# ut-amrl/vision_slam_frontend

Hardware: AMD Instinct MI355X
Metric: stereo frames/s (640x480, 2000 kp/frame) (higher is better)
Workload: dtype u8

## Files before the change

### include/vsf.h

```cpp
#ifndef VSF_H_
#define VSF_H_

#include <stddef.h>
#include <stdint.h>

#ifdef __cplusplus
extern "C" {
#endif

#define VSF_VERSION 2
#define VSF_DESC_BYTES 32
#define VSF_MAX_LEVELS 64

typedef enum {
  VSF_OK = 0,
  VSF_ERR_INVALID_ARG = 1,
  VSF_ERR_CAPACITY = 2,
  VSF_ERR_HIP = 3,
  VSF_ERR_UNSUPPORTED = 4,
  VSF_ERR_NO_DEVICE = 5
} vsf_status;

typedef struct {
  float x, y;
  float size;
  float angle;
  float response;
  int32_t octave;
  int32_t class_id;
} vsf_keypoint;

typedef struct {
  int32_t queryIdx, trainIdx, imgIdx;
  float distance;
} vsf_dmatch;

typedef struct {
  int32_t nfeatures;
  float scale_factor;
  int32_t nlevels;
  int32_t edge_threshold;
  int32_t first_level;
  int32_t wta_k;
  int32_t score_type;
  int32_t patch_size;
  int32_t fast_threshold;
  int32_t blur_sse2;
  int32_t fast_detector_threshold;
  int32_t fast_detector_nms;
  uint32_t ratio_num;
  uint32_t ratio_shift;
  int32_t width, height;
  int32_t max_images;
  int32_t max_keypoints;
  int32_t residual_order;
} vsf_params;

typedef struct vsf_ctx vsf_ctx;

vsf_status vsf_params_default(vsf_params* p, int width, int height, int max_images);
vsf_status vsf_params_set_ratio(vsf_params* p, float nn_match_ratio);

vsf_status vsf_create(const vsf_params* p, int device, vsf_ctx** out);
void vsf_destroy(vsf_ctx* ctx);
const char* vsf_status_string(vsf_status s);
int vsf_last_hip_error(const vsf_ctx* ctx);
vsf_status vsf_get_params(const vsf_ctx* ctx, vsf_params* out);
vsf_status vsf_set_stream(vsf_ctx* ctx, void* hip_stream);
vsf_status vsf_set_lanes(vsf_ctx* ctx, int lanes);
vsf_status vsf_set_pipeline(vsf_ctx* ctx, int on);
vsf_status vsf_set_input_event(vsf_ctx* ctx, void* hip_event);
vsf_status vsf_set_blur_overlap(vsf_ctx* ctx, int on);
vsf_status vsf_set_fast_resident(vsf_ctx* ctx, int waves);
vsf_status vsf_get_fast_resident(const vsf_ctx* ctx, int* waves);
vsf_status vsf_tune_fast_resident(vsf_ctx* ctx, const uint8_t* d_imgs, int n_images, size_t image_stride,
                                  size_t row_stride, vsf_keypoint* d_kp, uint8_t* d_desc, int32_t* d_counts,
                                  int samples, float* ms_grid, float* ms_resident);
typedef enum {
  VSF_OPT_FAST_BOTH_MAX = 0,
  VSF_OPT_SELECT_WIDE = 1,
  VSF_OPT_PYRAMID_FEW = 2,
  VSF_OPT_PYRAMID_CHAIN = 3,
  VSF_OPT_PYRAMID_ROWS = 4,
  VSF_OPT_SELECT_BIG_CLASS = 5,
  VSF_OPT_PIPE_AFTER_FAST = 6,
  VSF_OPT_PIPE_PRIORITY = 7,
  VSF_OPT_OBSERVE_THREAD = 8,
  VSF_OPT_PYRAMID_TAIL_MIN = 9,
  VSF_OPT_OBSERVE_COPY_THREAD = 10,
  VSF_OPT_COUNT = 11
} vsf_option;
vsf_status vsf_set_option(vsf_ctx* ctx, int option, int value);
vsf_status vsf_get_option(const vsf_ctx* ctx, int option, int* value);
vsf_status vsf_sync(vsf_ctx* ctx);
vsf_status vsf_reserve(vsf_ctx* ctx, int n_frames, int n_pairs);

vsf_status vsf_level_info(const vsf_ctx* ctx, int level, int* w, int* h, float* scale, int* nfeatures);

#define VSF_COMM_ID_BYTES 128
typedef struct vsf_comm vsf_comm;
vsf_status vsf_comm_unique_id(uint8_t* id);
vsf_status vsf_comm_create(vsf_ctx* ctx, const uint8_t* id, int rank, int world, vsf_comm** out);
void vsf_comm_destroy(vsf_comm* comm);
vsf_status vsf_comm_info(const vsf_comm* comm, int* rank, int* world, int* rccl_version);
vsf_status vsf_allgather_dev(vsf_ctx* ctx, vsf_comm* comm, const void* d_send, void* d_recv, size_t bytes_per_rank);
vsf_status vsf_gather_payload_dev(vsf_ctx* ctx, vsf_comm* comm, const uint8_t* d_send, size_t bytes, uint8_t* d_recv,
                                  size_t recv_stride, int root);


vsf_status vsf_extract(vsf_ctx* ctx, const uint8_t* img, int w, int h, size_t stride, vsf_keypoint* kp_out,
                       uint8_t* desc_out, int cap, int* n_out);
vsf_status vsf_extract_pair(vsf_ctx* ctx, const uint8_t* img0, const uint8_t* img1, int w, int h, size_t stride,
                            vsf_keypoint* kp0, uint8_t* desc0, int* n0, vsf_keypoint* kp1, uint8_t* desc1, int* n1,
                            int cap);
vsf_status vsf_fast_detect(vsf_ctx* ctx, const uint8_t* img, int w, int h, size_t stride, int threshold, int nms,
                           vsf_keypoint* kp_out, int cap, int* n_out);
vsf_status vsf_knn2_hamming(vsf_ctx* ctx, const uint8_t* q, int nq, const uint8_t* t, int nt, int32_t* idx2,
                            int32_t* dist2);
vsf_status vsf_get_matches(vsf_ctx* ctx, const uint8_t* q, int nq, const uint8_t* t, int nt, vsf_dmatch* out,
                           int cap, int* n_out);

vsf_status vsf_get_matches_multi(vsf_ctx* ctx, const uint8_t* const* q, const int* nq, int n_sets, const uint8_t* t,
                                 int nt, vsf_dmatch* out, int cap_per_set, int* n_out);


vsf_status vsf_extract_batch_dev(vsf_ctx* ctx, const uint8_t* d_imgs, int n_images, size_t image_stride,
                                 size_t row_stride, vsf_keypoint* d_kp, uint8_t* d_desc, int32_t* d_counts);
vsf_status vsf_match_batch_dev(vsf_ctx* ctx, const uint8_t* d_desc, const int32_t* d_counts, size_t set_stride,
                               const int32_t* d_q_set, const int32_t* d_t_set, int n_pairs, int32_t* d_idx2,
                               int32_t* d_dist2, vsf_dmatch* d_matches, int32_t* d_nmatches);
vsf_status vsf_stereo_batch_dev(vsf_ctx* ctx, const uint8_t* d_imgs, int n_frames, size_t image_stride,
                                size_t row_stride, vsf_keypoint* d_kp, uint8_t* d_desc, int32_t* d_counts,
                                vsf_dmatch* d_matches, int32_t* d_nmatches);


vsf_status vsf_remove_ambig_stereo_batch_dev(vsf_ctx* ctx, const vsf_keypoint* d_kp, const uint8_t* d_desc,
                                             const vsf_dmatch* d_matches, const int32_t* d_nmatches, int n_frames,
                                             const float* F, float thr_in, const float* d_thr_override,
                                             float* d_means, float* d_thr, vsf_keypoint* d_kp_out,
                                             uint8_t* d_desc_out, int32_t* d_counts_out);
vsf_status vsf_feature_matches_batch_dev(vsf_ctx* ctx, const uint8_t* d_desc, const int32_t* d_counts,
                                         size_t set_stride, const int32_t* d_q_set, const int32_t* d_t_set,
                                         int n_pairs, float best_percent, uint64_t* d_pairs, int32_t* d_npairs);

vsf_status vsf_stereo_residuals_batch_dev(vsf_ctx* ctx, const vsf_keypoint* d_kp, const vsf_dmatch* d_matches,
                                          const int32_t* d_nmatches, int n_frames, const float* F, float* d_means);
vsf_status vsf_stereo_thresholds_dev(vsf_ctx* ctx, const float* d_means, int n, float* d_thr_state, float* d_thr);
vsf_status vsf_stereo_filter_batch_dev(vsf_ctx* ctx, const vsf_keypoint* d_kp, const uint8_t* d_desc,
                                       const vsf_dmatch* d_matches, const int32_t* d_nmatches, int n_frames,
                                       const float* d_thr, vsf_keypoint* d_kp_out, uint8_t* d_desc_out,
                                       int32_t* d_counts_out);


typedef struct {
  float projection_left[12];
  float projection_right[12];
  float camera_matrix_left[9];
  float distortion_left[5];
  float fundamental[9];
  int32_t triangulate_rows;
} vsf_calibration;

typedef struct {
  uint32_t feature_idx_lo, feature_idx_hi;
  float pixel[2];
  float point3d[3];
} vsf_vision_feature;
typedef struct {
  uint64_t feature_idx_initial, feature_idx_current;
} vsf_feature_match;

vsf_status vsf_vision_features_batch_dev(vsf_ctx* ctx, const vsf_calibration* calib, const vsf_keypoint* d_kp,
                                         const uint8_t* d_desc, const int32_t* d_counts, int n_frames,
                                         vsf_vision_feature* d_features, int32_t* d_nfeatures, int32_t* d_npoints);

size_t vsf_packed_outputs_capacity(const vsf_ctx* ctx, int n_frames, int n_pairs);
vsf_status vsf_pack_outputs_dev(vsf_ctx* ctx, const vsf_vision_feature* d_features, const int32_t* d_nfeatures,
                                int n_frames, const uint64_t* d_pairs, const int32_t* d_npairs, int n_pairs,
                                uint8_t* d_payload, size_t payload_cap);


size_t vsf_observe_capacity(const vsf_ctx* ctx, int frame_life);
vsf_status vsf_observe_configure(vsf_ctx* ctx, int depth, int min_batch, int in_flight);
vsf_status vsf_observe_stereo(vsf_ctx* ctx, const uint8_t* left, const uint8_t* right, int w, int h, size_t stride,
                              const vsf_calibration* calib, float best_percent, int frame_life, uint8_t* out,
                              size_t cap, size_t* out_bytes);
vsf_status vsf_observe_submit(vsf_ctx* ctx, const uint8_t* left, const uint8_t* right, int w, int h, size_t stride,
                              const vsf_calibration* calib, float best_percent, int frame_life, int64_t* ticket);
vsf_status vsf_observe_collect(vsf_ctx* ctx, int64_t ticket, uint8_t* out, size_t cap, size_t* out_bytes);
vsf_status vsf_observe_collect_view(vsf_ctx* ctx, int64_t ticket, const uint8_t** out, size_t* out_bytes);
vsf_status vsf_observe_submit_compressed(vsf_ctx* ctx, const uint8_t* left, size_t left_bytes, const uint8_t* right,
                                         size_t right_bytes, int bayer, const vsf_calibration* calib, float best_percent,
                                         int frame_life, int64_t* ticket);
vsf_status vsf_observe_stereo_compressed(vsf_ctx* ctx, const uint8_t* left, size_t left_bytes, const uint8_t* right,
                                         size_t right_bytes, int bayer, const vsf_calibration* calib, float best_percent,
                                         int frame_life, uint8_t* out, size_t cap, size_t* out_bytes);
vsf_status vsf_observe_set_compressed_cap(vsf_ctx* ctx, size_t cap_per_image);
size_t vsf_observe_default_compressed_cap(int width, int height);
vsf_status vsf_compressed_image_size(const uint8_t* file, size_t nbytes, int* width, int* height);
vsf_status vsf_observe_poll(vsf_ctx* ctx, int64_t ticket, int* ready);
vsf_status vsf_observe_reset(vsf_ctx* ctx);
#define VSF_OBSERVE_MAX_STREAMS 64
vsf_status vsf_observe_set_streams(vsf_ctx* ctx, int n_streams);
vsf_status vsf_observe_submit_stream(vsf_ctx* ctx, int stream, const uint8_t* left, const uint8_t* right, int w, int h,
                                     size_t stride, const vsf_calibration* calib, float best_percent, int frame_life,
                                     int64_t* ticket);
vsf_status vsf_observe_submit_compressed_stream(vsf_ctx* ctx, int stream, const uint8_t* left, size_t left_bytes,
                                                const uint8_t* right, size_t right_bytes, int bayer,
                                                const vsf_calibration* calib, float best_percent, int frame_life,
                                                int64_t* ticket);
vsf_status vsf_observe_reset_stream(vsf_ctx* ctx, int stream);
vsf_status vsf_observe_stats(const vsf_ctx* ctx, int64_t* out, int n);
vsf_status vsf_observe_set_debug_images(vsf_ctx* ctx, int on);
vsf_status vsf_observe_debug_view(vsf_ctx* ctx, int64_t ticket, const uint8_t** stereo, const uint8_t** match);
vsf_status vsf_observe_set_debug_jpeg(vsf_ctx* ctx, int quality);
vsf_status vsf_observe_debug_jpeg_view(vsf_ctx* ctx, int64_t ticket, const uint8_t** stereo, size_t* stereo_bytes,
                                       const uint8_t** match, size_t* match_bytes);
vsf_status vsf_observe_set_debug_png(vsf_ctx* ctx, int on);
vsf_status vsf_observe_debug_png_view(vsf_ctx* ctx, int64_t ticket, const uint8_t** stereo, size_t* stereo_bytes,
                                      const uint8_t** match, size_t* match_bytes);

size_t vsf_observe_compressed_slot_bytes(size_t cap_per_image);
size_t vsf_observe_compressed_ring_bytes(int depth, size_t cap_per_image);
vsf_status vsf_observe_probe_compressed(const uint8_t* file, size_t nbytes, int width, int height, size_t cap_per_image,
                                        int force_serial, int* kind);

enum { VSF_DRAW_CIRCLE = 0, VSF_DRAW_LINE = 1 };
typedef struct {
  int32_t kind;
  int32_t x0, y0, x1, y1;
  uint8_t bgr[4];
} vsf_draw_op;
typedef struct {
  const uint8_t* src0;
  const uint8_t* src1;
  int32_t width, height;
  int64_t src_pitch;
  uint8_t* out;
  int64_t out_pitch;
  int32_t op_begin, op_count;
} vsf_draw_canvas;
vsf_status vsf_draw_canvases_dev(vsf_ctx* ctx, const vsf_draw_canvas* canvases, int n, const vsf_draw_op* d_ops, int n_ops);
vsf_status vsf_draw_canvases(vsf_ctx* ctx, const vsf_draw_canvas* canvases, int n, const vsf_draw_op* ops, int n_ops);

vsf_status vsf_jpeg_decode_gray_batch(vsf_ctx* ctx, const uint8_t* const* jpeg, const size_t* nbytes, int n_images,
                                      int width, int height, uint8_t* d_dst, size_t dst_image_stride,
                                      size_t dst_row_stride);

vsf_status vsf_png_decode_gray_batch(vsf_ctx* ctx, const uint8_t* const* png, const size_t* nbytes, int n_images,
                                     int width, int height, uint8_t* d_dst, size_t dst_image_stride,
                                     size_t dst_row_stride);

vsf_status vsf_imdecode_gray_batch(vsf_ctx* ctx, const uint8_t* const* files, const size_t* nbytes, int n_images,
                                   int width, int height, uint8_t* d_dst, size_t dst_image_stride,
                                   size_t dst_row_stride);

vsf_status vsf_bayer_bg_to_gray_batch_dev(vsf_ctx* ctx, const uint8_t* d_src, int n_images, int width, int height,
                                          size_t src_image_stride, size_t src_row_stride, uint8_t* d_dst,
                                          size_t dst_image_stride, size_t dst_row_stride);

size_t vsf_jpeg_encode_capacity(int width, int height, int channels);
vsf_status vsf_jpeg_encode_batch_dev(vsf_ctx* ctx, const uint8_t* d_src, int n_images, int width, int height, int channels,
                                     size_t src_image_stride, size_t src_row_stride, int quality, uint8_t* d_out,
                                     size_t out_stride, int32_t* d_out_bytes);
vsf_status vsf_jpeg_encode(vsf_ctx* ctx, const uint8_t* src, int n_images, int width, int height, int channels,
                           size_t src_image_stride, size_t src_row_stride, int quality, uint8_t* out, size_t out_stride,
                           int32_t* out_bytes);

size_t vsf_png_encode_capacity(int width, int height, int channels);
vsf_status vsf_png_encode_batch_dev(vsf_ctx* ctx, const uint8_t* d_src, int n_images, int width, int height, int channels,
                                    size_t src_image_stride, size_t src_row_stride, uint8_t* d_out, size_t out_stride,
                                    int32_t* d_out_bytes);
vsf_status vsf_png_encode(vsf_ctx* ctx, const uint8_t* src, int n_images, int width, int height, int channels,
                          size_t src_image_stride, size_t src_row_stride, uint8_t* out, size_t out_stride, int32_t* out_bytes);


vsf_status vsf_debug_png_encode_header(int width, int height, int channels, uint8_t* out, size_t cap, size_t* n_bytes);
vsf_status vsf_debug_png_encode_cpu(const uint8_t* src, int width, int height, int channels, size_t src_row_stride, uint8_t* out,
                                    size_t cap, size_t* n_bytes);

vsf_status vsf_debug_jpeg_encode_header(int width, int height, int channels, int quality, uint8_t* out, size_t cap,
                                        size_t* n_bytes);

vsf_status vsf_debug_inject_hip_error(vsf_ctx* ctx, int code);
vsf_status vsf_debug_level_image(vsf_ctx* ctx, int image, int level, int blurred, uint8_t* out, size_t ostride);
vsf_status vsf_debug_fast_candidates(vsf_ctx* ctx, int image, int level, vsf_keypoint* kp_out, int cap,
                                     int* n_out);
vsf_status vsf_debug_fast_work(const vsf_params* p, int orb, int nms, uint32_t* words, int cap, int* n_words, int* n_full,
                               int32_t* levels_out, int level_cap);
vsf_status vsf_debug_level_keypoints(vsf_ctx* ctx, int image, int level, vsf_keypoint* kp_out, int cap,
                                     int* n_out);
vsf_status vsf_debug_retain_best(vsf_ctx* ctx, uint32_t* key_bits, uint32_t* ids, int n, int n_points, int use_lds,
                                 int mode, int* n_out);
vsf_status vsf_debug_sort_trim(vsf_ctx* ctx, const vsf_dmatch* matches, int n_lists, int n, float best_percent,
                               int serial, uint64_t* pairs_out, int32_t* counts_out);

vsf_status vsf_debug_jpeg_serial(vsf_ctx* ctx, int on);

#define VSF_STAGE_COUNT 8
enum { VSF_STAGE_PYRAMID = 0, VSF_STAGE_FAST, VSF_STAGE_SELECT, VSF_STAGE_BLUR, VSF_STAGE_DESCRIBE, VSF_STAGE_KNN2,
       VSF_STAGE_RATIO, VSF_STAGE_TAIL  };
vsf_status vsf_profile_enable(vsf_ctx* ctx, int on);
vsf_status vsf_profile_read(vsf_ctx* ctx, double* ms_total, int64_t* launches, int reset);
const char* vsf_stage_name(int stage);

uint64_t vsf_algorithmic_bytes_per_image(const vsf_ctx* ctx);
uint64_t vsf_pyramid_pixels(const vsf_ctx* ctx);

#ifdef __cplusplus
}
#endif
#endif
```

### vision_slam_frontend_amd/capi.py

```python
from __future__ import annotations

import ctypes as C
from pathlib import Path

import numpy as np

_PKG = Path(__file__).resolve().parent
LIB_PATH = _PKG / "libvsf_hip.so"

KEYPOINT_DTYPE = np.dtype([("x", "<f4"), ("y", "<f4"), ("size", "<f4"), ("angle", "<f4"), ("response", "<f4"),
                           ("octave", "<i4"), ("class_id", "<i4")])
DMATCH_DTYPE = np.dtype([("queryIdx", "<i4"), ("trainIdx", "<i4"), ("imgIdx", "<i4"), ("distance", "<f4")])
VISION_FEATURE_DTYPE = np.dtype([("feature_idx", "<u8"), ("pixel", "<f4", (2,)), ("point3d", "<f4", (3,))])
FEATURE_MATCH_DTYPE = np.dtype([("feature_idx_initial", "<u8"), ("feature_idx_current", "<u8")])
assert VISION_FEATURE_DTYPE.itemsize == 28 and FEATURE_MATCH_DTYPE.itemsize == 16
DESC_BYTES = 32
PAYLOAD_MAGIC = 0x31465356

VSF_OK, VSF_ERR_INVALID_ARG, VSF_ERR_CAPACITY, VSF_ERR_HIP, VSF_ERR_UNSUPPORTED, VSF_ERR_NO_DEVICE = range(6)

EXPORTS = [
    "vsf_params_default", "vsf_params_set_ratio", "vsf_create", "vsf_destroy", "vsf_status_string",
    "vsf_last_hip_error", "vsf_get_params", "vsf_set_stream", "vsf_sync", "vsf_level_info", "vsf_extract",
    "vsf_fast_detect", "vsf_knn2_hamming", "vsf_get_matches", "vsf_extract_pair", "vsf_get_matches_multi", "vsf_extract_batch_dev", "vsf_match_batch_dev",
    "vsf_stereo_batch_dev", "vsf_set_lanes", "vsf_set_pipeline", "vsf_set_blur_overlap", "vsf_set_fast_resident", "vsf_get_fast_resident", "vsf_remove_ambig_stereo_batch_dev", "vsf_feature_matches_batch_dev", "vsf_bayer_bg_to_gray_batch_dev", "vsf_debug_level_image", "vsf_debug_fast_candidates", "vsf_debug_fast_work", "vsf_debug_level_keypoints",
    "vsf_algorithmic_bytes_per_image", "vsf_pyramid_pixels", "vsf_profile_enable", "vsf_profile_read",
    "vsf_stage_name", "vsf_debug_retain_best", "vsf_debug_sort_trim", "vsf_stereo_residuals_batch_dev", "vsf_stereo_thresholds_dev",
    "vsf_stereo_filter_batch_dev", "vsf_vision_features_batch_dev", "vsf_packed_outputs_capacity",
    "vsf_pack_outputs_dev", "vsf_observe_capacity", "vsf_observe_stereo", "vsf_observe_submit", "vsf_observe_collect", "vsf_observe_reset",
    "vsf_observe_configure", "vsf_observe_collect_view", "vsf_observe_stats", "vsf_observe_poll", "vsf_debug_jpeg_serial",
    "vsf_jpeg_decode_gray_batch", "vsf_png_decode_gray_batch", "vsf_imdecode_gray_batch", "vsf_tune_fast_resident", "vsf_set_option", "vsf_get_option", "vsf_debug_inject_hip_error", "vsf_comm_unique_id", "vsf_comm_create", "vsf_comm_destroy", "vsf_comm_info",
    "vsf_allgather_dev", "vsf_gather_payload_dev", "vsf_reserve", "vsf_set_input_event",
    "vsf_observe_set_debug_images", "vsf_observe_debug_view", "vsf_draw_canvases_dev", "vsf_draw_canvases",
    "vsf_observe_submit_compressed", "vsf_observe_stereo_compressed", "vsf_observe_set_compressed_cap",
    "vsf_observe_default_compressed_cap", "vsf_observe_compressed_slot_bytes", "vsf_observe_compressed_ring_bytes",
    "vsf_compressed_image_size", "vsf_observe_probe_compressed",
    "vsf_observe_set_debug_jpeg", "vsf_observe_debug_jpeg_view", "vsf_jpeg_encode_capacity", "vsf_jpeg_encode_batch_dev", "vsf_jpeg_encode", "vsf_debug_jpeg_encode_header",
    "vsf_png_encode_capacity", "vsf_png_encode_batch_dev", "vsf_png_encode", "vsf_debug_png_encode_header", "vsf_debug_png_encode_cpu", "vsf_observe_set_debug_png", "vsf_observe_debug_png_view",
    "vsf_observe_set_streams", "vsf_observe_submit_stream", "vsf_observe_submit_compressed_stream", "vsf_observe_reset_stream",
]
(OPT_FAST_BOTH_MAX, OPT_SELECT_WIDE, OPT_PYRAMID_FEW, OPT_PYRAMID_CHAIN, OPT_PYRAMID_ROWS, OPT_SELECT_BIG_CLASS,
 OPT_PIPE_AFTER_FAST, OPT_PIPE_PRIORITY, OPT_OBSERVE_THREAD, OPT_PYRAMID_TAIL_MIN, OPT_OBSERVE_COPY_THREAD) = range(11)
STAGE_COUNT = 8
OBSERVE_STATS = ("frames", "batches", "max_batch", "solo", "forced", "slot_waits", "depth", "bmax", "copy_ns", "launch_ns",
                 "wait_ns", "compressed", "ingest_commands", "compressed_bytes", "debug_jpeg_commands", "streams",
                 "multi_stream_batches")


class VsfParams(C.Structure):
    _fields_ = [("nfeatures", C.c_int32), ("scale_factor", C.c_float), ("nlevels", C.c_int32),
                ("edge_threshold", C.c_int32), ("first_level", C.c_int32), ("wta_k", C.c_int32),
                ("score_type", C.c_int32), ("patch_size", C.c_int32), ("fast_threshold", C.c_int32),
                ("blur_sse2", C.c_int32), ("fast_detector_threshold", C.c_int32), ("fast_detector_nms", C.c_int32),
                ("ratio_num", C.c_uint32), ("ratio_shift", C.c_uint32), ("width", C.c_int32), ("height", C.c_int32),
                ("max_images", C.c_int32), ("max_keypoints", C.c_int32), ("residual_order", C.c_int32)]


class VsfCalibration(C.Structure):
    _fields_ = [("projection_left", C.c_float * 12), ("projection_right", C.c_float * 12),
                ("camera_matrix_left", C.c_float * 9), ("distortion_left", C.c_float * 5),
                ("fundamental", C.c_float * 9), ("triangulate_rows", C.c_int32)]

    def set(self, name: str, values) -> "VsfCalibration":
        arr = getattr(self, name)
        v = np.ascontiguousarray(values, np.float32).reshape(-1)
        assert len(v) == len(arr), name
        for i, x in enumerate(v):
            arr[i] = float(x)
        return self

    def get(self, name: str) -> np.ndarray:
        return np.array(list(getattr(self, name)), np.float32)


DRAW_CIRCLE, DRAW_LINE = 0, 1
DRAW_OP_DTYPE = np.dtype([("kind", "<i4"), ("x0", "<i4"), ("y0", "<i4"), ("x1", "<i4"), ("y1", "<i4"), ("bgr", "u1", (4,))])
assert DRAW_OP_DTYPE.itemsize == 24


class VsfDrawCanvas(C.Structure):
    _fields_ = [("src0", C.c_void_p), ("src1", C.c_void_p), ("width", C.c_int32), ("height", C.c_int32),
                ("src_pitch", C.c_int64), ("out", C.c_void_p), ("out_pitch", C.c_int64), ("op_begin", C.c_int32),
                ("op_count", C.c_int32)]


class VsfError(RuntimeError):
    def __init__(self, status: int, where: str, hip: int = 0):
        self.status = status
        msg = "%s: %s" % (where, lib().vsf_status_string(status).decode())
        if status == VSF_ERR_HIP:
            msg += " (hipError %d)" % hip
        super().__init__(msg)


_lib = None


def jpeg_encode_capacity(width: int, height: int, channels: int) -> int:
    return int(lib().vsf_jpeg_encode_capacity(width, height, channels))


def jpeg_encode_header(width: int, height: int, channels: int, quality: int = 0) -> bytes:
    buf = np.zeros(640, np.uint8)
    n = C.c_size_t()
    st = lib().vsf_debug_jpeg_encode_header(width, height, channels, quality, buf.ctypes.data_as(C.c_void_p), 640, C.byref(n))
    if st != VSF_OK:
        raise VsfError(st, "vsf_debug_jpeg_encode_header")
    return buf[:n.value].tobytes()


def png_encode_capacity(width: int, height: int, channels: int) -> int:
    return int(lib().vsf_png_encode_capacity(width, height, channels))


def png_encode_header(width: int, height: int, channels: int) -> bytes:
    buf = np.zeros(64, np.uint8)
    n = C.c_size_t()
    st = lib().vsf_debug_png_encode_header(width, height, channels, buf.ctypes.data_as(C.c_void_p), 64, C.byref(n))
    if st != VSF_OK:
        raise VsfError(st, "vsf_debug_png_encode_header")
    return buf[:n.value].tobytes()


def png_encode_cpu(img) -> bytes:
    img = np.ascontiguousarray(img, dtype=np.uint8)
    h, w = img.shape[:2]
    ch = 1 if img.ndim == 2 else img.shape[2]
    cap = png_encode_capacity(w, h, ch)
    out = np.zeros(cap, np.uint8)
    n = C.c_size_t()
    st = lib().vsf_debug_png_encode_cpu(_p(img), w, h, ch, w * ch, _p(out), cap, C.byref(n))
    if st != VSF_OK:
        raise VsfError(st, "vsf_debug_png_encode_cpu")
    return out[:n.value].tobytes()


def lib() -> C.CDLL:
    global _lib
    if _lib is None:
        if not LIB_PATH.exists():
            raise ImportError("%s is missing: run `python -c 'import __graft_entry__ as g; g.build()'` "
                              "(hipcc --offload-arch=gfx950). The product has no CPU fallback." % LIB_PATH)
        L = C.CDLL(str(LIB_PATH))
        vp, i32, sz, pp = C.c_void_p, C.c_int, C.c_size_t, C.POINTER(VsfParams)
        ip = C.POINTER(C.c_int)
        L.vsf_params_default.argtypes = [pp, i32, i32, i32]
        L.vsf_params_set_ratio.argtypes = [pp, C.c_float]
        L.vsf_create.argtypes = [pp, i32, C.POINTER(vp)]
        L.vsf_destroy.argtypes = [vp]
        L.vsf_destroy.restype = None
        L.vsf_status_string.argtypes = [i32]
        L.vsf_status_string.restype = C.c_char_p
        L.vsf_last_hip_error.argtypes = [vp]
        L.vsf_get_params.argtypes = [vp, pp]
        L.vsf_set_stream.argtypes = [vp, vp]
        L.vsf_sync.argtypes = [vp]
        L.vsf_level_info.argtypes = [vp, i32, ip, ip, C.POINTER(C.c_float), ip]
        L.vsf_extract.argtypes = [vp, vp, i32, i32, sz, vp, vp, i32, ip]
        L.vsf_fast_detect.argtypes = [vp, vp, i32, i32, sz, i32, i32, vp, i32, ip]
        L.vsf_extract_pair.argtypes = [vp, vp, vp, i32, i32, sz, vp, vp, ip, vp, vp, ip, i32]
        L.vsf_get_matches_multi.argtypes = [vp, vp, vp, i32, vp, i32, vp, i32, vp]
        L.vsf_knn2_hamming.argtypes = [vp, vp, i32, vp, i32, vp, vp]
        L.vsf_get_matches.argtypes = [vp, vp, i32, vp, i32, vp, i32, ip]
        L.vsf_extract_batch_dev.argtypes = [vp, vp, i32, sz, sz, vp, vp, vp]
        L.vsf_match_batch_dev.argtypes = [vp, vp, vp, sz, vp, vp, i32, vp, vp, vp, vp]
        L.vsf_stereo_batch_dev.argtypes = [vp, vp, i32, sz, sz, vp, vp, vp, vp, vp]
        L.vsf_set_lanes.argtypes = [vp, i32]
        L.vsf_set_pipeline.argtypes = [vp, i32]
        L.vsf_set_input_event.argtypes = [vp, vp]
        L.vsf_reserve.argtypes = [vp, i32, i32]
        L.vsf_set_blur_overlap.argtypes = [vp, i32]
        L.vsf_set_fast_resident.argtypes = [vp, i32]
        L.vsf_get_fast_resident.argtypes = [vp, C.POINTER(C.c_int)]
        L.vsf_tune_fast_resident.argtypes = [vp, vp, i32, sz, sz, vp, vp, vp, i32, C.POINTER(C.c_float), C.POINTER(C.c_float)]
        L.vsf_set_option.argtypes = [vp, i32, i32]
        L.vsf_get_option.argtypes = [vp, i32, ip]
        L.vsf_debug_inject_hip_error.argtypes = [vp, i32]
        L.vsf_comm_unique_id.argtypes = [vp]
        L.vsf_comm_create.argtypes = [vp, vp, i32, i32, C.POINTER(vp)]
        L.vsf_comm_destroy.argtypes = [vp]
        L.vsf_comm_destroy.restype = None
        L.vsf_comm_info.argtypes = [vp, ip, ip, ip]
        L.vsf_allgather_dev.argtypes = [vp, vp, vp, vp, sz]
        L.vsf_gather_payload_dev.argtypes = [vp, vp, vp, sz, vp, sz, i32]
        L.vsf_remove_ambig_stereo_batch_dev.argtypes = [vp, vp, vp, vp, vp, i32, vp, C.c_float, vp, vp, vp, vp, vp, vp]
        L.vsf_feature_matches_batch_dev.argtypes = [vp, vp, vp, sz, vp, vp, i32, C.c_float, vp, vp]
        L.vsf_bayer_bg_to_gray_batch_dev.argtypes = [vp, vp, i32, i32, i32, sz, sz, vp, sz, sz]
        L.vsf_jpeg_encode_capacity.argtypes = [i32, i32, i32]
        L.vsf_jpeg_encode_capacity.restype = sz
        L.vsf_jpeg_encode_batch_dev.argtypes = [vp, vp, i32, i32, i32, i32, sz, sz, i32, vp, sz, vp]
        L.vsf_jpeg_encode.argtypes = [vp, vp, i32, i32, i32, i32, sz, sz, i32, vp, sz, vp]
        L.vsf_debug_jpeg_encode_header.argtypes = [i32, i32, i32, i32, vp, sz, C.POINTER(sz)]
        L.vsf_png_encode_capacity.argtypes = [i32, i32, i32]
        L.vsf_png_encode_capacity.restype = sz
        L.vsf_png_encode_batch_dev.argtypes = [vp, vp, i32, i32, i32, i32, sz, sz, vp, sz, vp]
        L.vsf_png_encode.argtypes = [vp, vp, i32, i32, i32, i32, sz, sz, vp, sz, vp]
        L.vsf_debug_png_encode_header.argtypes = [i32, i32, i32, vp, sz, C.POINTER(sz)]
        L.vsf_debug_png_encode_cpu.argtypes = [vp, i32, i32, i32, sz, vp, sz, C.POINTER(sz)]
        L.vsf_stereo_residuals_batch_dev.argtypes = [vp, vp, vp, vp, i32, vp, vp]
        L.vsf_stereo_thresholds_dev.argtypes = [vp, vp, i32, vp, vp]
        L.vsf_stereo_filter_batch_dev.argtypes = [vp, vp, vp, vp, vp, i32, vp, vp, vp, vp]
        L.vsf_vision_features_batch_dev.argtypes = [vp, C.POINTER(VsfCalibration), vp, vp, vp, i32, vp, vp, vp]
        L.vsf_packed_outputs_capacity.argtypes = [vp, i32, i32]
        L.vsf_packed_outputs_capacity.restype = sz
        L.vsf_pack_outputs_dev.argtypes = [vp, vp, vp, i32, vp, vp, i32, vp, sz]
        L.vsf_debug_sort_trim.argtypes = [vp, vp, i32, i32, C.c_float, i32, vp, vp]
        L.vsf_observe_capacity.argtypes = [vp, i32]
        L.vsf_observe_capacity.restype = sz
        L.vsf_observe_submit.argtypes = [vp, vp, vp, i32, i32, sz, C.POINTER(VsfCalibration), C.c_float, i32,
                                         C.POINTER(C.c_int64)]
        L.vsf_observe_collect.argtypes = [vp, C.c_int64, vp, sz, C.POINTER(sz)]
        L.vsf_observe_collect_view.argtypes = [vp, C.c_int64, C.POINTER(vp), C.POINTER(sz)]
        L.vsf_observe_configure.argtypes = [vp, i32, i32, i32]
        L.vsf_observe_stats.argtypes = [vp, vp, i32]
        L.vsf_observe_poll.argtypes = [vp, C.c_int64, C.POINTER(i32)]
        L.vsf_observe_stereo.argtypes = [vp, vp, vp, i32, i32, sz, C.POINTER(VsfCalibration), C.c_float, i32, vp, sz,
                                         C.POINTER(sz)]
        L.vsf_observe_reset.argtypes = [vp]
        L.vsf_observe_set_streams.argtypes = [vp, i32]
        L.vsf_observe_reset_stream.argtypes = [vp, i32]
        L.vsf_observe_submit_stream.argtypes = [vp, i32, vp, vp, i32, i32, sz, C.POINTER(VsfCalibration), C.c_float, i32,
                                                C.POINTER(C.c_int64)]
        L.vsf_observe_submit_compressed_stream.argtypes = [vp, i32, vp, sz, vp, sz, i32, C.POINTER(VsfCalibration), C.c_float,
                                                           i32, C.POINTER(C.c_int64)]
        L.vsf_observe_submit_compressed.argtypes = [vp, vp, sz, vp, sz, i32, C.POINTER(VsfCalibration), C.c_float, i32,
                                                    C.POINTER(C.c_int64)]
        L.vsf_observe_stereo_compressed.argtypes = [vp, vp, sz, vp, sz, i32, C.POINTER(VsfCalibration), C.c_float, i32, vp,
                                                    sz, C.POINTER(sz)]
        L.vsf_observe_set_compressed_cap.argtypes = [vp, sz]
        L.vsf_observe_default_compressed_cap.argtypes = [i32, i32]
        L.vsf_observe_default_compressed_cap.restype = sz
        L.vsf_observe_compressed_slot_bytes.argtypes = [sz]
        L.vsf_observe_compressed_slot_bytes.restype = sz
        L.vsf_observe_compressed_ring_bytes.argtypes = [i32, sz]
        L.vsf_observe_compressed_ring_bytes.restype = sz
        L.vsf_compressed_image_size.argtypes = [vp, sz, ip, ip]
        L.vsf_observe_probe_compressed.argtypes = [vp, sz, i32, i32, sz, i32, ip]
        L.vsf_observe_set_debug_images.argtypes = [vp, i32]
        L.vsf_observe_debug_view.argtypes = [vp, C.c_int64, C.POINTER(vp), C.POINTER(vp)]
        L.vsf_observe_set_debug_jpeg.argtypes = [vp, i32]
        L.vsf_observe_debug_jpeg_view.argtypes = [vp, C.c_int64, C.POINTER(vp), C.POINTER(sz), C.POINTER(vp), C.POINTER(sz)]
        L.vsf_observe_set_debug_png.argtypes = [vp, i32]
        L.vsf_observe_debug_png_view.argtypes = [vp, C.c_int64, C.POINTER(vp), C.POINTER(sz), C.POINTER(vp), C.POINTER(sz)]
        L.vsf_draw_canvases_dev.argtypes = [vp, C.POINTER(VsfDrawCanvas), i32, vp, i32]
        L.vsf_draw_canvases.argtypes = [vp, C.POINTER(VsfDrawCanvas), i32, vp, i32]
        L.vsf_jpeg_decode_gray_batch.argtypes = [vp, vp, vp, i32, i32, i32, vp, sz, sz]
        L.vsf_png_decode_gray_batch.argtypes = [vp, vp, vp, i32, i32, i32, vp, sz, sz]
        L.vsf_imdecode_gray_batch.argtypes = [vp, vp, vp, i32, i32, i32, vp, sz, sz]
        L.vsf_debug_level_image.argtypes = [vp, i32, i32, i32, vp, sz]
        L.vsf_debug_fast_candidates.argtypes = [vp, i32, i32, vp, i32, ip]
        L.vsf_debug_fast_work.argtypes = [vp, i32, i32, vp, i32, ip, ip, vp, i32]
        L.vsf_debug_level_keypoints.argtypes = [vp, i32, i32, vp, i32, ip]
        L.vsf_algorithmic_bytes_per_image.argtypes = [vp]
        L.vsf_algorithmic_bytes_per_image.restype = C.c_uint64
        L.vsf_pyramid_pixels.argtypes = [vp]
        L.vsf_pyramid_pixels.restype = C.c_uint64
        L.vsf_debug_retain_best.argtypes = [vp, vp, vp, i32, i32, i32, i32, ip]
        L.vsf_profile_enable.argtypes = [vp, i32]
        L.vsf_profile_read.argtypes = [vp, C.POINTER(C.c_double), C.POINTER(C.c_int64), i32]
        L.vsf_stage_name.argtypes = [i32]
        L.vsf_stage_name.restype = C.c_char_p
        _lib = L
    return _lib


def _p(a):
    return a.ctypes.data_as(C.c_void_p) if isinstance(a, np.ndarray) else C.c_void_p(int(a) if a else 0)


def default_params(width: int, height: int, max_images: int = 2, nfeatures: int = 10000, **over) -> VsfParams:
    p = VsfParams()
    st = lib().vsf_params_default(C.byref(p), width, height, max_images)
    if st != VSF_OK:
        raise VsfError(st, "vsf_params_default")
    p.nfeatures = nfeatures
    ratio = over.pop("nn_match_ratio", None)
    if ratio is not None:
        st = lib().vsf_params_set_ratio(C.byref(p), ratio)
        if st != VSF_OK:
            raise VsfError(st, "vsf_params_set_ratio")
    for k, v in over.items():
        if not hasattr(p, k):
            raise AttributeError(k)
        setattr(p, k, v)
    return p


class Context:

    def __init__(self, params: VsfParams, device: int = 0):
        self._h = C.c_void_p()
        st = lib().vsf_create(C.byref(params), device, C.byref(self._h))
        if st != VSF_OK:
            self._h = None
            raise VsfError(st, "vsf_create")
        self.params = VsfParams()
        lib().vsf_get_params(self._h, C.byref(self.params))
        self.device = device

    def close(self):
        if getattr(self, "_h", None):
            lib().vsf_destroy(self._h)
            self._h = None

    def __del__(self):
        try:
            self.close()
        except TypeError:
            pass

    def __enter__(self):
        return self

    def __exit__(self, *a):
        self.close()

    def _check(self, st: int, where: str, allow_capacity: bool = False):
        if st == VSF_OK or (allow_capacity and st == VSF_ERR_CAPACITY):
            return st
        raise VsfError(st, where, lib().vsf_last_hip_error(self._h))

    @property
    def nlevels(self) -> int:
        return self.params.nlevels

    def level_info(self, level: int):
        w, h, n, s = C.c_int(), C.c_int(), C.c_int(), C.c_float()
        self._check(lib().vsf_level_info(self._h, level, C.byref(w), C.byref(h), C.byref(s), C.byref(n)),
                    "vsf_level_info")
        return w.value, h.value, s.value, n.value

    def algorithmic_bytes_per_image(self) -> int:
        return int(lib().vsf_algorithmic_bytes_per_image(self._h))

    def pyramid_pixels(self) -> int:
        return int(lib().vsf_pyramid_pixels(self._h))

    def set_stream(self, hip_stream: int | None):
        self._check(lib().vsf_set_stream(self._h, C.c_void_p(hip_stream or 0)), "vsf_set_stream")

    def set_lanes(self, lanes: int):
        self._check(lib().vsf_set_lanes(self._h, lanes), "vsf_set_lanes")

    def set_blur_overlap(self, on: bool):
        self._check(lib().vsf_set_blur_overlap(self._h, int(on)), "vsf_set_blur_overlap")
# ... 470 lines not shown
```

### vision_slam_frontend_amd/csrc/k_fast.hip

```cpp
#include "vsf_gather.h"
#include <cstdlib>

#include "vsf_internal.h"

namespace {

typedef short v2s __attribute__((ext_vector_type(2)));
constexpr int SR = VSF_FAST_STRIP_ROWS;

struct FastArgs {
  const VsfLevel* levels;
  const uint32_t* units;
  int nwork_full;
  int nunits;
  const uint8_t* img0;
  size_t img0_stride;
  int img0_pitch;
  const uint8_t* pyr;
  uint32_t pyr_bytes;
  uint32_t* cand;
  uint32_t cand_entries;
  uint16_t* rowstart;
  int threshold;
  int nms;
};

__device__ __forceinline__ uint32_t wave_shr1(uint32_t v) {
  return (uint32_t)__builtin_amdgcn_update_dpp(0, (int)v, 0x138, 0xF, 0xF, true);
}
__device__ __forceinline__ uint32_t wave_shl1(uint32_t v) {
  return (uint32_t)__builtin_amdgcn_update_dpp(0, (int)v, 0x130, 0xF, 0xF, true);
}

template <class T>
__device__ __forceinline__ T uniform_copy(const T* p) {
  static_assert(sizeof(T) % 4 == 0, "dwords");
  T out;
  const uint32_t* src = reinterpret_cast<const uint32_t*>(p);
  uint32_t* dst = reinterpret_cast<uint32_t*>(&out);
#pragma unroll
  for (size_t i = 0; i < sizeof(T) / 4; i++) dst[i] = (uint32_t)__builtin_amdgcn_readfirstlane((int)src[i]);
  return out;
}

struct RowP {
  uint32_t d;
  v2s b1, b2, b3, b4, b5, b6, b7, b8;
};

__device__ __forceinline__ v2s as_v2s(uint32_t v) { return __builtin_bit_cast(v2s, v); }
__device__ __forceinline__ uint32_t as_u32(v2s v) { return __builtin_bit_cast(uint32_t, v); }

__device__ __forceinline__ void prep_row(RowP& r) {
  const uint32_t e = r.d & 0x00FF00FFu, o = (r.d >> 8) & 0x00FF00FFu;
  const uint32_t ep = wave_shr1(e), op = wave_shr1(o);
  const uint32_t en = wave_shl1(e), on = wave_shl1(o);
  r.b1 = as_v2s(op);
  r.b2 = as_v2s(__builtin_amdgcn_alignbit(e, ep, 16));
  r.b3 = as_v2s(__builtin_amdgcn_alignbit(o, op, 16));
  r.b4 = as_v2s(e);
  r.b5 = as_v2s(o);
  r.b6 = as_v2s(__builtin_amdgcn_alignbit(en, e, 16));
  r.b7 = as_v2s(__builtin_amdgcn_alignbit(on, o, 16));
  r.b8 = as_v2s(en);
}

__device__ __forceinline__ v2s vmin(v2s a, v2s b) { return __builtin_elementwise_min(a, b); }
__device__ __forceinline__ v2s vmax(v2s a, v2s b) { return __builtin_elementwise_max(a, b); }
__device__ __forceinline__ v2s vmin3(v2s a, v2s b, v2s c) {
  v2s r;
  asm("v_pk_minimum3_f16 %0, %1, %2, %3" : "=v"(r) : "v"(a), "v"(b), "v"(c));
  return r;
}
__device__ __forceinline__ v2s vmax3(v2s a, v2s b, v2s c) {
  v2s r;
  asm("v_pk_maximum3_f16 %0, %1, %2, %3" : "=v"(r) : "v"(a), "v"(b), "v"(c));
  return r;
}
__device__ __forceinline__ v2s vsubsat(v2s a, v2s b) {
  typedef unsigned short v2us __attribute__((ext_vector_type(2)));
  return __builtin_bit_cast(v2s, __builtin_elementwise_sub_sat(__builtin_bit_cast(v2us, a), __builtin_bit_cast(v2us, b)));
}

template <bool NMS>
__device__ __forceinline__ v2s score_from_circle(const v2s (&d)[16], v2s v, v2s toff) {
  v2s E[8], G[8], F[8], H[8];
#pragma unroll
  for (int j = 0; j < 8; j++) {
    E[j] = vmin(d[2 * j + 1], d[(2 * j + 2) & 15]);
    G[j] = vmax(d[2 * j + 1], d[(2 * j + 2) & 15]);
  }
#pragma unroll
  for (int j = 0; j < 8; j++) {
    F[j] = vmin(E[j], E[(j + 1) & 7]);
    H[j] = vmax(G[j], G[(j + 1) & 7]);
  }
  v2s ta[8], tb[8];
#pragma unroll
  for (int j = 0; j < 8; j++) {
    ta[j] = vmin3(F[j], F[(j + 2) & 7], vmax(d[2 * j], d[(2 * j + 9) & 15]));
    tb[j] = vmax3(H[j], H[(j + 2) & 7], vmin(d[2 * j], d[(2 * j + 9) & 15]));
  }
  const v2s A = vmax(vmax3(vmax3(ta[0], ta[1], ta[2]), vmax3(ta[3], ta[4], ta[5]), ta[6]), ta[7]);
  const v2s Bm = vmin(vmin3(vmin3(tb[0], tb[1], tb[2]), vmin3(tb[3], tb[4], tb[5]), tb[6]), tb[7]);
  const v2s sc = vsubsat(vmax(vsubsat(A, v), vsubsat(v, Bm)), toff);
  const v2s one = {1, 1};
  return NMS ? sc : vmin(sc, one);
}

template <bool NMS>
__device__ __forceinline__ v2s score_pair0(const RowP& R0, const RowP& R1, const RowP& R2, const RowP& R3, const RowP& R4,
                                           const RowP& R5, const RowP& R6, v2s toff) {
  const v2s d[16] = {R6.b4, R6.b5, R5.b6, R4.b7, R3.b7, R2.b7, R1.b6, R0.b5, R0.b4, R0.b3, R1.b2, R2.b1, R3.b1, R4.b1, R5.b2, R6.b3};
  return score_from_circle<NMS>(d, R3.b4, toff);
}
template <bool NMS>
__device__ __forceinline__ v2s score_pair1(const RowP& R0, const RowP& R1, const RowP& R2, const RowP& R3, const RowP& R4,
                                           const RowP& R5, const RowP& R6, v2s toff) {
  const v2s d[16] = {R6.b5, R6.b6, R5.b7, R4.b8, R3.b8, R2.b8, R1.b7, R0.b6, R0.b5, R0.b4, R1.b3, R2.b2, R3.b2, R4.b2, R5.b3, R6.b4};
  return score_from_circle<NMS>(d, R3.b5, toff);
}

struct ScoreRow {
  v2s s02, s13;
  v2s h3a, h3b;
  v2s h2a, h2b;
};

__device__ __forceinline__ ScoreRow make_score_row(v2s s02, v2s s13) {
  ScoreRow o;
  o.s02 = s02;
  o.s13 = s13;
  const v2s x = as_v2s(__builtin_amdgcn_alignbit(as_u32(s13), wave_shr1(as_u32(s13)), 16));
  const v2s y = as_v2s(__builtin_amdgcn_alignbit(wave_shl1(as_u32(s02)), as_u32(s02), 16));
  o.h2a = vmax(x, s13);
  o.h2b = vmax(s02, y);
  o.h3a = vmax3(x, s13, s02);
  o.h3b = vmax3(s02, y, s13);
  return o;
}

template <bool PACK, bool NMS>
__device__ __forceinline__ void fast_march_body(const FastArgs& a, int work, int image) {
  const int lane = threadIdx.x & 63;
  int level, band, strip, hl, nl, nrows0 = 0;
  bool valid = true, mixed = false, rim = false;
  VsfLevel L;
  if constexpr (PACK) {
    struct Item {
      uint32_t w[VSF_FAST_PACK_WORDS];
    };
    const Item P = uniform_copy(reinterpret_cast<const Item*>(a.units + a.nwork_full) + work);
    uint32_t w0 = P.w[4], w1 = P.w[5];
#pragma unroll
    for (int k = 1; k < VSF_FAST_PACK_SEGS; k++)
      if (k < (int)P.w[0] && lane >= (int)(P.w[5 + 2 * k] & 0xFFu)) w0 = P.w[4 + 2 * k], w1 = P.w[5 + 2 * k];
    nrows0 = (int)P.w[1];
    mixed = P.w[2] != 0u;
    rim = P.w[3] != 0u;
    level = (int)(w0 >> 24), band = (int)((w0 >> 16) & 0xFF), strip = (int)(w0 & 0x7FFF);
    hl = lane - (int)(w1 & 0xFFu);
    nl = (int)((w1 >> 8) & 0xFFu);
    valid = hl < nl;
    L = a.levels[level];
  } else {
    const uint32_t ud = uniform_copy(a.units + work);
    level = (int)(ud >> 24), band = (int)((ud >> 16) & 0xFF), strip = (int)(ud & 0x7FFF);
    L = uniform_copy(a.levels + level);
    hl = lane, nl = 64;
  }
  const int pitch = level == 0 ? a.img0_pitch : L.pitch, hrow = L.h;
  const uint8_t* src;
  uint32_t src_bytes;
  if constexpr (PACK) {
    const bool lvl0 = __builtin_amdgcn_readfirstlane(level) == 0;
    src = lvl0 ? a.img0 + (size_t)image * a.img0_stride : a.pyr + (size_t)image * a.pyr_bytes;
    src_bytes = lvl0 ? (uint32_t)(a.img0_pitch * __builtin_amdgcn_readfirstlane(hrow)) : a.pyr_bytes;
  } else {
    src = level == 0 ? a.img0 + (size_t)image * a.img0_stride : a.pyr + (size_t)image * a.pyr_bytes + L.offset;
    src_bytes = (uint32_t)(pitch * hrow);
  }
  const int t = a.threshold;
  const int offs = NMS ? max(t, 1) : t;
  const v2s toff = {(short)offs, (short)offs};
  const int bx0 = L.fast_a0 + VSF_FAST_BAND_COLS * band;
  const int c0 = bx0 - 4 + 4 * hl;
  const bool loadable = valid && c0 >= 0 && c0 + 3 < pitch;
  const int ys = L.y_lo + strip * SR;
  const int nrows = valid ? min(SR, L.y_hi - ys) : 0;
  if constexpr (!PACK) nrows0 = nrows;
  const int sx_lo = max(L.x_lo - 1, 3), sx_hi = min(L.x_hi + 1, L.w - 3);
  uint32_t sm02 = 0, sm13 = 0, em02 = 0, em13 = 0;
#pragma unroll
  for (int j = 0; j < 4; j++) {
    const int x = c0 + j;
    const uint32_t bit = 0xFFFFu << (16 * (j >> 1));
    const bool sc_ok = valid && ((hl >= 1 && hl <= nl - 2) || (hl == 0 && j == 3) || (hl == nl - 1 && j == 0)) &&
                       x >= sx_lo && x < sx_hi;
    const bool em_ok = valid && hl >= 1 && hl <= nl - 2 && x >= L.x_lo && x < L.x_hi && x < bx0 + VSF_FAST_BAND_COLS;
    if (j & 1) {
      if (sc_ok) sm13 |= bit;
      if (em_ok) em13 |= bit;
    } else {
      if (sc_ok) sm02 |= bit;
      if (em_ok) em02 |= bit;
    }
  }
  const int unit_local = strip * L.nbands + band;
  uint16_t* rs = a.rowstart + ((size_t)image * a.nunits + L.unit0 + unit_local) * VSF_FAST_RS_STRIDE;
  const int seg_cap = L.seg_cap;
  const __amdgpu_buffer_rsrc_t seg_rsrc =
      PACK ? __builtin_amdgcn_make_buffer_rsrc(a.cand + (size_t)image * a.cand_entries, 0, a.cand_entries * 4, 0x00020000)
           : __builtin_amdgcn_make_buffer_rsrc(a.cand + (size_t)image * a.cand_entries + L.cand_offset +
                                                   (size_t)unit_local * seg_cap,
                                               0, seg_cap * 4, 0x00020000);
  const uint32_t seg_off = PACK ? 4u * (L.cand_offset + (uint32_t)(unit_local * seg_cap)) : 0u;
  const __amdgpu_buffer_rsrc_t rs_rsrc = __builtin_amdgcn_make_buffer_rsrc(
      a.rowstart + (size_t)image * a.nunits * VSF_FAST_RS_STRIDE, 0, a.nunits * VSF_FAST_RS_STRIDE * 2, 0x00020000);
  const uint32_t rs_off = 2u * (uint32_t)((L.unit0 + unit_local) * VSF_FAST_RS_STRIDE);
  const bool rs_lane = PACK && valid && hl == 0;
  const int cfirst = lane - hl, cend = min(cfirst + nl, 64);
  const unsigned long long from_m = ~0ull << cfirst, cell_m = from_m & (cend >= 64 ? ~0ull : (1ull << cend) - 1ull);
  const uint32_t from_lo = (uint32_t)from_m, from_hi = (uint32_t)(from_m >> 32);
  const uint32_t cell_lo = (uint32_t)cell_m, cell_hi = (uint32_t)(cell_m >> 32);

  const __amdgpu_buffer_rsrc_t src_rsrc = __builtin_amdgcn_make_buffer_rsrc(const_cast<uint8_t*>(src), 0, src_bytes, 0x00020000);
  const uint32_t col_off = loadable ? (uint32_t)c0 : 0xFFFFFFF0u;
  const int qlo = 1 - ys, qhi = hrow - ys;
  const uint32_t rbase = loadable ? (level == 0 ? 0u : L.offset) + (uint32_t)(c0 + (ys - 1) * pitch) : 0x40000000u;
  auto load_row = [&](int q) -> uint32_t {
    if (PACK)
      return __builtin_amdgcn_raw_buffer_load_b32(src_rsrc, rbase + (uint32_t)__mul24(min(max(q, qlo), qhi), pitch), 0u,
                                                  0);
    const int yc = min(max(ys - 1 + q, 0), hrow - 1);
    return __builtin_amdgcn_raw_buffer_load_b32(src_rsrc, col_off, (uint32_t)(yc * pitch), 0);
  };

  const unsigned long long scorable = __builtin_amdgcn_ballot_w64((sm02 | sm13) != 0u);
  const v2s zero2 = {0, 0};
  ScoreRow S0 = make_score_row(zero2, zero2), S1 = S0, S2 = S0;
  int count = 0;
  uint32_t my_rs = 0;
  const uint32_t yx0 = ((uint32_t)ys << 12) + (uint32_t)c0 + ((uint32_t)(NMS ? offs - 1 : 0) << 24);
  auto below = [&](unsigned long long b, int acc) -> int {
    if (PACK)
      return (int)__builtin_amdgcn_mbcnt_hi((uint32_t)(b >> 32) & from_hi,
                                            __builtin_amdgcn_mbcnt_lo((uint32_t)b & from_lo, (uint32_t)acc));
    return (int)__builtin_amdgcn_mbcnt_hi((uint32_t)(b >> 32), __builtin_amdgcn_mbcnt_lo((uint32_t)b, (uint32_t)acc));
  };
  auto in_cell = [&](unsigned long long b) -> int {
    if (PACK) return __popc((uint32_t)b & cell_lo) + __popc((uint32_t)(b >> 32) & cell_hi);
    return __popcll(b);
  };

  auto step = [&](int q, const RowP& R0, const RowP& R1, const RowP& R2, const RowP& R3, const RowP& R4,
                  const RowP& R5, RowP& R6, const ScoreRow& S_up, const ScoreRow& S_mid, ScoreRow& S_dn) {
    prep_row(R6);
    v2s s02 = zero2, s13 = zero2;
    const int sy = ys - 1 + q;
    const bool row_ok = sy >= 3 && sy < hrow - 3;
    const uint32_t far = max(__builtin_amdgcn_sad_u8(R0.d, R3.d, 0u), __builtin_amdgcn_sad_u8(R6.d, R3.d, 0u));
    unsigned long long want = __builtin_amdgcn_ballot_w64(far > (uint32_t)t) & scorable;
    if (PACK) {
      if (rim) want &= __builtin_amdgcn_ballot_w64(row_ok);
    } else {
      want &= row_ok ? ~0ull : 0ull;
    }
    if (want != 0ull) {
      s02 = score_pair0<NMS>(R0, R1, R2, R3, R4, R5, R6, toff);
      s13 = score_pair1<NMS>(R0, R1, R2, R3, R4, R5, R6, toff);
      if (PACK && rim) {
        s02 = as_v2s(as_u32(s02) & (row_ok ? sm02 : 0u));
        s13 = as_v2s(as_u32(s13) & (row_ok ? sm13 : 0u));
      } else {
        s02 = as_v2s(as_u32(s02) & sm02);
        s13 = as_v2s(as_u32(s13) & sm13);
      }
    }
    S_dn = make_score_row(s02, s13);
    const int r = q - 2;
    if (r >= 0 && r < nrows0) {
      if (__any((as_u32(S_mid.s02) | as_u32(S_mid.s13)) != 0)) {
        uint32_t k02, k13;
        if (NMS) {
          const v2s nb02 = vmax3(S_up.h3a, S_dn.h3a, S_mid.h2a), nb13 = vmax3(S_up.h3b, S_dn.h3b, S_mid.h2b);
          k02 = as_u32((nb02 - S_mid.s02) >> 15) & as_u32(S_mid.s02) & em02;
          k13 = as_u32((nb13 - S_mid.s13) >> 15) & as_u32(S_mid.s13) & em13;
        } else {
          k02 = as_u32(S_mid.s02) & em02;
          k13 = as_u32(S_mid.s13) & em13;
        }
        if (PACK && mixed && r >= nrows) k02 = k13 = 0;
        const uint32_t yx = yx0 + ((uint32_t)r << 12);
        if (NMS) {
          const uint32_t kk = k02 | k13;
          const bool hasA = (kk & 0xFFFFu) != 0u, hasB = (kk >> 16) != 0u;
          const unsigned long long bA = __ballot(hasA), bB = __ballot(hasB);
          if ((bA | bB) != 0ull) {
            const int pos = below(bB, below(bA, count));
            const uint32_t eA = (kk << 24) + yx + ((k13 & 0xFFFFu) != 0u ? 1u : 0u);
            const uint32_t eB = ((kk & 0xFFFF0000u) << 8) + yx + 2u + ((k13 >> 16) != 0u ? 1u : 0u);
            const int posB = pos + (hasA ? 1 : 0);
            if (hasA && (!PACK || pos < seg_cap)) __builtin_amdgcn_raw_buffer_store_b32(eA, seg_rsrc, seg_off + 4u * (uint32_t)pos, 0, 0);
            if (hasB && (!PACK || posB < seg_cap)) __builtin_amdgcn_raw_buffer_store_b32(eB, seg_rsrc, seg_off + 4u * (uint32_t)posB, 0, 0);
            count += in_cell(bA) + in_cell(bB);
          }
        } else {
          const bool k0 = (k02 & 0xFFFFu) != 0, k1 = (k13 & 0xFFFFu) != 0, k2 = (k02 >> 16) != 0, k3 = (k13 >> 16) != 0;
          const unsigned long long b0 = __ballot(k0), b1 = __ballot(k1), b2 = __ballot(k2), b3 = __ballot(k3);
          if ((b0 | b1 | b2 | b3) != 0ull) {
            int pos = below(b3, below(b2, below(b1, below(b0, count))));
            if (k0) {
              if (!PACK || pos < seg_cap) __builtin_amdgcn_raw_buffer_store_b32(yx, seg_rsrc, seg_off + 4u * (uint32_t)pos, 0, 0);
              ++pos;
            }
            if (k1) {
              if (!PACK || pos < seg_cap) __builtin_amdgcn_raw_buffer_store_b32(yx + 1, seg_rsrc, seg_off + 4u * (uint32_t)pos, 0, 0);
              ++pos;
            }
            if (k2) {
              if (!PACK || pos < seg_cap) __builtin_amdgcn_raw_buffer_store_b32(yx + 2, seg_rsrc, seg_off + 4u * (uint32_t)pos, 0, 0);
              ++pos;
            }
            if (k3) {
              if (!PACK || pos < seg_cap) __builtin_amdgcn_raw_buffer_store_b32(yx + 3, seg_rsrc, seg_off + 4u * (uint32_t)pos, 0, 0);
            }
            count += in_cell(b0) + in_cell(b1) + in_cell(b2) + in_cell(b3);
          }
        }
      }
      if (r + 1 < SR) {
        if (PACK) {
          if (rs_lane)
            __builtin_amdgcn_raw_buffer_store_b16((unsigned short)min(count, seg_cap), rs_rsrc, rs_off, 2u * (uint32_t)(r + 1), 0);
        } else {
          asm("s_mov_b32 m0, %2\n\ts_nop 0\n\tv_writelane_b32 %0, %1, m0" : "+v"(my_rs) : "s"(min(count, seg_cap)), "s"(r + 1));
        }
      }
    }
  };

  RowP A0, A1, A2, A3, A4, A5, A6, A7, A8;
  A0.d = load_row(-3), A1.d = load_row(-2), A2.d = load_row(-1), A3.d = load_row(0), A4.d = load_row(1), A5.d = load_row(2),
  A6.d = load_row(3), A7.d = load_row(4);
  prep_row(A0), prep_row(A1), prep_row(A2), prep_row(A3), prep_row(A4), prep_row(A5);
  const int qe = nrows0 + 1;
#define VSF_FAST_STEP(j, r0, r1, r2, r3, r4, r5, r6, ld, su, sm, sd) \
  if (q + (j) > qe) break;                                             \
  ld.d = load_row(q + (j) + 5);                                        \
  step(q + (j), r0, r1, r2, r3, r4, r5, r6, su, sm, sd);
  for (int q = 0;; q += 9) {
    VSF_FAST_STEP(0, A0, A1, A2, A3, A4, A5, A6, A8, S0, S1, S2)
    VSF_FAST_STEP(1, A1, A2, A3, A4, A5, A6, A7, A0, S1, S2, S0)
    VSF_FAST_STEP(2, A2, A3, A4, A5, A6, A7, A8, A1, S2, S0, S1)
    VSF_FAST_STEP(3, A3, A4, A5, A6, A7, A8, A0, A2, S0, S1, S2)
    VSF_FAST_STEP(4, A4, A5, A6, A7, A8, A0, A1, A3, S1, S2, S0)
    VSF_FAST_STEP(5, A5, A6, A7, A8, A0, A1, A2, A4, S2, S0, S1)
    VSF_FAST_STEP(6, A6, A7, A8, A0, A1, A2, A3, A5, S0, S1, S2)
    VSF_FAST_STEP(7, A7, A8, A0, A1, A2, A3, A4, A6, S1, S2, S0)
    VSF_FAST_STEP(8, A8, A0, A1, A2, A3, A4, A5, A7, S2, S0, S1)
  }
#undef VSF_FAST_STEP
  if (PACK) {
    if (rs_lane) {
      rs[0] = 0;
      rs[SR] = (uint16_t)min(count, seg_cap);
    }
  } else {
    if (hl < SR) rs[hl] = (uint16_t)my_rs;
    if (hl == 0) rs[SR] = (uint16_t)min(count, seg_cap);
  }
}

template <bool PACK, bool NMS>
__global__ __launch_bounds__(256) void fast_march_kernel(FastArgs a, int nwork) {
  const int item = __builtin_amdgcn_readfirstlane(blockIdx.x * 4 + (threadIdx.x >> 6));
  if (item >= nwork) return;
  fast_march_body<PACK, NMS>(a, item, blockIdx.y);
}

template <bool NMS>
__global__ __launch_bounds__(256) void fast_march_both_kernel(FastArgs a, int nfull, int npack) {
  const int item = __builtin_amdgcn_readfirstlane(blockIdx.x * 4 + (threadIdx.x >> 6));
  if (item >= nfull + npack) return;
  if (item < nfull)
    fast_march_body<false, NMS>(a, item, blockIdx.y);
  else
    fast_march_body<true, NMS>(a, item - nfull, blockIdx.y);
}

template <bool PACK, bool NMS>
__global__ __launch_bounds__(1024) void fast_march_resident_kernel(FastArgs a, int nwork, int nimages, uint32_t* next_cell) {
  const int total = nwork * nimages;
  while (true) {
    uint32_t r;
    asm volatile(
        "s_mov_b64 s[34:35], exec\n\t"
        "s_mov_b64 exec, 1\n\t"
        "global_atomic_add %0, %1, %2, %3 sc0\n\t"
        "s_waitcnt vmcnt(0)\n\t"
        "s_mov_b64 exec, s[34:35]"
        : "=&v"(r)
        : "v"(0u), "v"(1u), "s"(next_cell)
        : "memory", "s34", "s35");
    const uint32_t u = (uint32_t)__builtin_amdgcn_readfirstlane((int)r);
    if (u >= (uint32_t)total) break;
    const int image = (int)u / nwork, cell = (int)u - image * nwork;
    fast_march_body<PACK, NMS>(a, cell, image);
  }
}

__global__ __launch_bounds__(256) void fast_emit_kernel(const VsfLevel* __restrict__ levels,
                                                        const uint32_t* __restrict__ cand, uint32_t cand_entries,
                                                        const uint16_t* __restrict__ rowstart, int nunits,
                                                        int max_keypoints, vsf_keypoint* __restrict__ out,
                                                        int32_t* __restrict__ counts, int32_t* __restrict__ status) {
  __shared__ int cellpre[2048 + 8];
  __shared__ __attribute__((aligned(4))) uint16_t rs_lds[64 * VSF_FAST_RS_STRIDE];
  __shared__ int lds4[4];
  const int image = blockIdx.x;
  const VsfLevel L = levels[0];
  const uint16_t* rs_img = rowstart + (size_t)image * nunits * VSF_FAST_RS_STRIDE;
  const uint32_t* cand_img = cand + (size_t)image * cand_entries;
  vsf_keypoint* o = out + (size_t)image * max_keypoints;
  const int n = vsf_gather_level<256>(L, cand_img, rs_img, cellpre, 2048, rs_lds, 64, lds4, [](int) {}, [&](int dst, uint32_t cd) {
    if (dst < max_keypoints) {
      vsf_keypoint kp;
      kp.x = (float)VSF_CAND_X(cd);
      kp.y = (float)VSF_CAND_Y(cd);
      kp.size = 7.f;
      kp.angle = -1.f;
      kp.response = (float)VSF_CAND_SCORE(cd);
      kp.octave = 0;
      kp.class_id = -1;
      o[dst] = kp;
    }
  });
  if (threadIdx.x == 0) {
    counts[image] = n;
    if (n > max_keypoints) atomicOr(status, 1);
  }
}

}

void vsf_launch_fast(const VsfDev& d, const VsfGeom& g, const VsfImages& im, int threshold, int nms, hipStream_t s,
                     int resident_waves_per_simd, int n_cus, uint32_t* d_cell_counters) {
  FastArgs a;
  a.levels = d.levels;
  a.units = d.units;
  a.nwork_full = g.nwork_full;
  a.nunits = g.nunits;
  a.img0 = im.base;
  a.img0_stride = im.image_stride;
  a.img0_pitch = (int)im.row_stride;
  a.pyr = d.pyr;
  a.pyr_bytes = g.pyr_bytes;
  a.cand = d.cand;
  a.cand_entries = g.cand_entries;
  a.rowstart = d.rowstart;
  a.threshold = threshold;
  a.nms = nms;
  if (resident_waves_per_simd > 0 && resident_waves_per_simd <= 4 && nms && d_cell_counters) {
    vsf_note(hipMemsetAsync(d_cell_counters, 0, 2 * sizeof(uint32_t), s));
    const dim3 block(256 * resident_waves_per_simd);
    if (g.nwork_full > 0)
      hipLaunchKernelGGL((fast_march_resident_kernel<false, true>), dim3(n_cus), block, 0, s, a, g.nwork_full, im.n,
                         d_cell_counters);
    if (g.nwork_pack > 0)
      hipLaunchKernelGGL((fast_march_resident_kernel<true, true>), dim3(n_cus), block, 0, s, a, g.nwork_pack, im.n,
                         d_cell_counters + 1);
    return;
  }
  const dim3 gf((g.nwork_full + 3) / 4, im.n), gp((g.nwork_pack + 3) / 4, im.n);
  const int both_max = d.tune ? d.tune->fast_both_max : 16;
  if (im.n <= both_max && g.nwork_full > 0 && g.nwork_pack > 0) {
    const dim3 gb((g.nwork_full + g.nwork_pack + 3) / 4, im.n);
    if (nms)
      hipLaunchKernelGGL((fast_march_both_kernel<true>), gb, dim3(256), 0, s, a, g.nwork_full, g.nwork_pack);
    else
      hipLaunchKernelGGL((fast_march_both_kernel<false>), gb, dim3(256), 0, s, a, g.nwork_full, g.nwork_pack);
    return;
  }
  if (nms) {
    if (g.nwork_full > 0) hipLaunchKernelGGL((fast_march_kernel<false, true>), gf, dim3(256), 0, s, a, g.nwork_full);
    if (g.nwork_pack > 0) hipLaunchKernelGGL((fast_march_kernel<true, true>), gp, dim3(256), 0, s, a, g.nwork_pack);
  } else {
    if (g.nwork_full > 0) hipLaunchKernelGGL((fast_march_kernel<false, false>), gf, dim3(256), 0, s, a, g.nwork_full);
    if (g.nwork_pack > 0) hipLaunchKernelGGL((fast_march_kernel<true, false>), gp, dim3(256), 0, s, a, g.nwork_pack);
  }
}

void vsf_launch_fast_emit(const VsfDev& d, const VsfGeom& g, int n_images, int max_keypoints, vsf_keypoint* d_kp,
                          int32_t* d_counts, hipStream_t s) {
  hipLaunchKernelGGL(fast_emit_kernel, dim3(n_images), dim3(256), 0, s, d.levels, d.cand, g.cand_entries, d.rowstart,
                     g.nunits, max_keypoints, d_kp, d_counts, d.status);
}
```

### vision_slam_frontend_amd/csrc/k_pyramid.hip

```cpp
#pragma clang fp contract(off)
#include <algorithm>
#include <cmath>
#include <cstdlib>
#include <type_traits>

#include "vsf_internal.h"

namespace {


typedef unsigned short v2u16 __attribute__((ext_vector_type(2)));
struct __attribute__((packed, aligned(1))) U8B {
  uint32_t lo, hi;
};

struct ResizeArgs {
  const uint8_t* src;
  size_t src_img_stride;
  int src_pitch, sw, sh;
  uint8_t* dst;
  size_t dst_img_stride;
  int dst_pitch, dw, dh;
  double scale_x, scale_y;
  int nstrips;
// ... 213 lines not shown
  }
  uint8_t* D = a.dst + (size_t)image * a.dst_img_stride;
  const int rlast = a.dh - last * R;
  const uint32_t d0 = (uint32_t)(sc * R) * (uint32_t)a.dst_pitch + (uint32_t)c.x4;
#pragma unroll
  for (int r = 0; r < R; r++) {
    const uint32_t wmr = (uint32_t)__builtin_amdgcn_ds_bpermute(slot + 4 * r, (int)wm);
    const uint32_t wor = (uint32_t)__builtin_amdgcn_ds_bpermute(slot + 4 * r, (int)wo);
    const bool step = (int)wor < 0;
    const H4 other = {step ? H[r + 2].a : H[r].a, step ? H[r + 2].b : H[r].b, step ? H[r + 2].c : H[r].c,
                      step ? H[r + 2].d : H[r].d};
    const uint32_t out = vblend(H[r + 1], other, wmr, wor);
    const uint32_t doff = d0 + (uint32_t)r * (uint32_t)a.dst_pitch;
    if (live && (r < rlast || strip < last)) {
      *reinterpret_cast<uint32_t*>(D + doff) = out;
      if (to_lds) st32(lcopy + doff, out);
    }
  }
}

template <int R>
__device__ __forceinline__ void resize_packed_unit(const ResizeArgs& a, int image, int j) {
  const VsfPackedLane at = packed_lane(a.pk, (uint32_t)j * 64u + (threadIdx.x & 63));
  const StripX c = strip_setup_at(a, a.pk.x0 + at.lane * 4);
  strip_packed<R>(a, c, image, at.strip, __builtin_amdgcn_readfirstlane(at.strip), a.src + (size_t)image * a.src_img_stride);
}

template <int R>
__global__ __launch_bounds__(256) __attribute__((amdgpu_waves_per_eu(8, 8))) void resize_strip_kernel(ResizeArgs a) {
  const int unit = __builtin_amdgcn_readfirstlane(blockIdx.x * 4 + (threadIdx.x >> 6));
  if (a.pk.waves > 0 && blockIdx.z == gridDim.z - 1) {
    if (unit < a.pk.waves) resize_packed_unit<R>(a, blockIdx.y, unit);
    return;
  }
  if (unit >= a.nstrips) return;
  resize_strip_unit<R>(a, blockIdx.y, unit, blockIdx.z);
}

struct PyramidArgs {
  const VsfLevel* levels;
  const uint8_t* img0;
  size_t img0_stride;
  int img0_pitch;
  uint8_t* pyr;
  uint32_t pyr_bytes;
  int l_begin, nlevels;
};

__host__ __device__ __forceinline__ ResizeArgs level_args(const VsfLevel& L, const VsfLevel& P, const PyramidArgs& p, int l) {
  ResizeArgs a;
  if (l >= 2) {
    a.src = p.pyr + P.offset;
    a.src_img_stride = (size_t)p.pyr_bytes;
    a.src_pitch = P.pitch;
  } else {
    a.src = p.img0;
    a.src_img_stride = p.img0_stride;
    a.src_pitch = p.img0_pitch;
  }
  a.sw = P.w;
  a.sh = P.h;
  a.dst = p.pyr + L.offset;
  a.dst_img_stride = (size_t)p.pyr_bytes;
  a.dst_pitch = L.pitch;
  a.dw = L.w;
  a.dh = L.h;
  a.scale_x = __builtin_bit_cast(double, ((unsigned long long)L.rscale_x[1] << 32) | L.rscale_x[0]);
  a.scale_y = __builtin_bit_cast(double, ((unsigned long long)L.rscale_y[1] << 32) | L.rscale_y[0]);
  a.nstrips = (L.h + 7) / 8;
  a.pk = VsfPackPlan{0, 0, 0, 0};
  return a;
}

constexpr int kTailLdsBytes = 61440;

__global__ __launch_bounds__(1024) void pyramid_image_kernel(PyramidArgs p) {
  __shared__ __attribute__((aligned(16))) uint8_t lvl[2][kTailLdsBytes];
  __shared__ uint32_t xs[2][kStripXWords][64];
  const int image = blockIdx.x;
  const int lane = threadIdx.x & 63;
  const int wave = __builtin_amdgcn_readfirstlane(threadIdx.x >> 6);
  auto level = [&](int l) {
    __builtin_assume(l >= 2);
    return level_args(p.levels[l], p.levels[l - 1], p, l);
  };
  auto publish = [&](int l) { stripx_store(xs[l & 1], lane, strip_setup(level(l), 0)); };
  if (wave == 0) publish(p.l_begin);
  __syncthreads();
  for (int l = p.l_begin; l < p.nlevels; l++) {
    const ResizeArgs a = level(l);
    const StripX c = stripx_load(xs[l & 1], lane, lane * 4, a.dw);
    const bool from_lds = l > p.l_begin;
    uint8_t* lcopy = (l + 1 < p.nlevels) ? lvl[(l - p.l_begin) & 1] : nullptr;
    const uint8_t* lsrc = lvl[(l - p.l_begin + 1) & 1];
    const uint8_t* gsrc = a.src + (size_t)image * a.src_img_stride;
    const VsfPackPlan pk = pack_plan(8, 0, a.dw, a.nstrips);
    if (pk.waves > 0) {
      for (int j = wave; j < pk.waves; j += 16) {
        const uint32_t g = (uint32_t)j * 64u + lane;
        VsfPackedLane at;
        at.strip = (int)__umulhi(g, pk.magic);
        at.lane = (int)g - at.strip * pk.lanes;
        const StripX cp = stripx_load(xs[l & 1], at.lane, at.lane * 4, a.dw);
        const int s_lo = __builtin_amdgcn_readfirstlane(at.strip);
        if (from_lds)
          strip_packed<8, true>(a, cp, image, at.strip, s_lo, lsrc, lcopy, lcopy != nullptr);
        else
          strip_packed<8>(a, cp, image, at.strip, s_lo, gsrc, lcopy, lcopy != nullptr);
      }
    } else {
      for (int strip = wave; strip < a.nstrips; strip += 16) {
        StripRows<8> rows;
        if (from_lds)
          strip_issue_from<8, true>(a, c, lsrc, strip * 8, rows);
        else
          strip_issue_from<8>(a, c, gsrc, strip * 8, rows);
        strip_finish<8>(a, c, image, strip * 8, a.dh, rows, lcopy, lcopy != nullptr);
      }
    }
    if (wave == 0 && l + 1 < p.nlevels) publish(l + 1);
    __syncthreads();
  }
}

constexpr int kSlabMaxLevels = 32;
constexpr int kSlabBands = 3;
constexpr size_t kSlabTapBytes = sizeof(uint32_t) * 2 * kSlabBands * kStripXWords * 64;
constexpr size_t kSlabFixedBytes = kSlabTapBytes + 2 * kSlabMaxLevels * sizeof(int) + (kSlabMaxLevels + 1) * sizeof(VsfLevel);

struct SlabArgs {
  PyramidArgs p;
  int la, lb;
  int nslabs;
  uint32_t cap;
  int32_t* status;
};

__global__ __launch_bounds__(1024) void pyramid_slab_kernel(SlabArgs q) {
  extern __shared__ __attribute__((aligned(16))) uint8_t smem[];
  const lds_u8p buf0 = (lds_u8p)smem, buf1 = buf0 + q.cap;
  uint32_t(*xs)[kSlabBands][kStripXWords][64] =
      reinterpret_cast<uint32_t(*)[kSlabBands][kStripXWords][64]>(smem + 2 * (size_t)q.cap);
  int* s_lo = reinterpret_cast<int*>(smem + 2 * (size_t)q.cap + kSlabTapBytes);
  int* s_hi = s_lo + kSlabMaxLevels;
  VsfLevel* s_lev = reinterpret_cast<VsfLevel*>(s_hi + kSlabMaxLevels);
  const int image = blockIdx.y, slab = blockIdx.x;
  const int lane = threadIdx.x & 63;
  const int wave = __builtin_amdgcn_readfirstlane(threadIdx.x >> 6);
  const int nl = q.lb - q.la;
  {
    const uint32_t* src = reinterpret_cast<const uint32_t*>(q.p.levels + (q.la - 1));
    uint32_t* dst = reinterpret_cast<uint32_t*>(s_lev);
    for (int i = threadIdx.x; i < (nl + 1) * (int)(sizeof(VsfLevel) / 4); i += 1024) dst[i] = src[i];
  }
  __syncthreads();
  auto level = [&](int l) { return level_args(s_lev[l - q.la + 1], s_lev[l - q.la], q.p, l); };
  if (threadIdx.x == 0) {
    const int hz = s_lev[nl].h;
    int lo = (int)((long)hz * slab / q.nslabs), hi = (int)((long)hz * (slab + 1) / q.nslabs);
    bool fits = true;
    s_lo[nl - 1] = lo;
    s_hi[nl - 1] = hi;
    for (int l = q.lb - 1; l > q.la; l--) {
      const ResizeArgs a = level(l);
      if (hi > lo) {
        const int f = resize_ytap32(min(lo, a.dh - 1), a.scale_y, a.sh).i0, g = resize_ytap32(min(hi - 1, a.dh - 1), a.scale_y, a.sh).i0;
        lo = f;
        hi = min(g + 1, a.sh - 1) + 1;
        fits = fits && (size_t)(hi - lo) * (size_t)a.src_pitch <= (size_t)q.cap;
      }
      s_lo[l - 1 - q.la] = lo;
      s_hi[l - 1 - q.la] = hi;
    }
    if (!fits) {
      atomicOr(q.status, 1);
      s_hi[nl - 1] = s_lo[nl - 1];
    }
  }
  auto publish = [&](int l) {
    const ResizeArgs a = level(l);
    const int band = 15 - wave;
    if (band < ((a.dw + 255) >> 8)) stripx_store(xs[l & 1][band], lane, strip_setup(a, band));
  };
  if (wave >= 16 - kSlabBands) publish(q.la);
  __syncthreads();
  if (s_hi[nl - 1] <= s_lo[nl - 1]) return;
  for (int l = q.la; l < q.lb; l++) {
    const ResizeArgs a = level(l);
    const int j = l - q.la;
    if (wave >= 16 - kSlabBands && l + 1 < q.lb) publish(l + 1);
    const int ylo = s_lo[j], yhi = s_hi[j];
    const int nb = (a.dw + 255) >> 8;
    const bool from_lds = j > 0;
    const bool to_lds = l + 1 < q.lb;
    const lds_u8p lcopy = ((j & 1) ? buf1 : buf0) - (uint32_t)ylo * (uint32_t)a.dst_pitch;
    const lds_cu8p lsrc = ((j & 1) ? buf0 : buf1) - (uint32_t)(from_lds ? s_lo[j - 1] : 0) * (uint32_t)a.src_pitch;
    const uint8_t* gsrc = a.src + (size_t)image * a.src_img_stride;
    auto run = [&](auto rows_tag) {
      constexpr int R = decltype(rows_tag)::value;
      const int nunits = ((yhi - ylo + R - 1) / R) * nb;
      for (int u = wave; u < nunits; u += 16) {
        const int st = u / nb, band = u - st * nb;
        const StripX c = stripx_load(xs[l & 1][band], lane, band * 256 + lane * 4, a.dw);
        const int ys = ylo + st * R;
        StripRows<R> rows;
        if (from_lds)
          strip_issue_from<R, true, lds_cu8p>(a, c, lsrc, ys, rows);
        else
          strip_issue_from<R>(a, c, gsrc, ys, rows);
        strip_finish<R, lds_u8p>(a, c, image, ys, yhi, rows, lcopy, to_lds);
      }
    };
    if (((yhi - ylo + 1) >> 1) * nb <= 16 - kSlabBands)
      run(std::integral_constant<int, 2>{});
    else if (((yhi - ylo + 3) >> 2) * nb <= 16 - kSlabBands)
      run(std::integral_constant<int, 4>{});
    else
      run(std::integral_constant<int, 8>{});
    __syncthreads();
  }
}

size_t slab_chain_bytes(const VsfLevel* lv, int la, int lb, int nslabs) {
  long rows = (lv[lb - 1].h + nslabs - 1) / nslabs + 1;
  size_t need = 0;
  for (int l = lb - 1; l > la; l--) {
    const double sy = 1. / ((double)lv[l].h / lv[l - 1].h);
    rows = std::min<long>((long)std::floor((double)rows * sy) + 4, lv[l - 1].h);
    need = std::max(need, (size_t)rows * (size_t)lv[l - 1].pitch);
  }
  return need;
}

PyramidArgs pyramid_args(const VsfDev& d, const VsfGeom& g, const VsfImages& im, int l_begin, int nlevels) {
  PyramidArgs p;
  p.levels = d.levels;
  p.img0 = im.base;
  p.img0_stride = im.image_stride;
  p.img0_pitch = (int)im.row_stride;
  p.pyr = d.pyr;
  p.pyr_bytes = g.pyr_bytes;
  p.l_begin = l_begin;
  p.nlevels = nlevels;
  return p;
}

bool launch_slab_chains(const VsfDev& d, const VsfGeom& g, const VsfLevel* h_levels, const VsfImages& im, hipStream_t s) {
  bool ok = true;
  for (int l = 1; l < g.nlevels; l++) ok = ok && h_levels[l].resize_any8 && h_levels[l].w <= 256 * kSlabBands;
  const int chain_env = d.tune ? d.tune->pyramid_chain : 8;
  const int lds_limit = d.tune ? d.tune->lds_limit : 160 * 1024;
  if (!(ok && chain_env > 0 && lds_limit >= 160 * 1024 - 2048)) return false;
  const size_t fixed = kSlabFixedBytes;
  const size_t budget = 144 * 1024;
  for (int la = 1; la < g.nlevels;) {
    int lb = std::min({la + chain_env, la + kSlabMaxLevels, g.nlevels});
    const int rows_env = d.tune ? std::max(1, d.tune->pyramid_rows) : 6;
    int nslabs = std::max(1, std::min(64, h_levels[lb - 1].h / rows_env));
    size_t need = slab_chain_bytes(h_levels, la, lb, nslabs);
    while (2 * need + fixed > budget && (nslabs < 64 || lb > la + 1)) {
      if (nslabs < 64)
        nslabs = std::min(64, nslabs * 2);
      else
        --lb;
      need = slab_chain_bytes(h_levels, la, lb, nslabs);
    }
    SlabArgs q;
    q.p = pyramid_args(d, g, im, la, lb);
    q.la = la;
    q.lb = lb;
    q.nslabs = nslabs;
    q.cap = (uint32_t)((need + 255) & ~(size_t)255);
    q.status = d.status;
    hipLaunchKernelGGL(pyramid_slab_kernel, dim3(nslabs, im.n), dim3(1024), 2 * (size_t)q.cap + fixed, s, q);
    la = lb;
  }
  return true;
}

int choose_l_tail(const VsfDev& d, const VsfGeom& g, const VsfLevel* h_levels, const VsfImages& im, const VsfSideStream* side,
                  bool few) {
  int l_tail = g.nlevels;
  if (side && (im.n >= 64 || few || (d.tune && d.tune->pyramid_tail_min > 0 && im.n >= d.tune->pyramid_tail_min))) {
    static int ncu = 0;
    if (ncu == 0) {
      int dev = 0;
      hipDeviceProp_t prop;
      if (hipGetDevice(&dev) == hipSuccess && hipGetDeviceProperties(&prop, dev) == hipSuccess) ncu = prop.multiProcessorCount;
      if (ncu <= 0) ncu = 256;
    }
    const int rounds = (im.n + ncu - 1) / ncu;
    const int tail_min = d.tune ? d.tune->pyramid_tail_min : 0;
    if (few || 4 * im.n >= 3 * rounds * ncu || (tail_min > 0 && im.n >= tail_min)) {
      while (l_tail > 2 && h_levels[l_tail - 1].w <= 256 && h_levels[l_tail - 1].resize_rows >= 8 &&
             h_levels[l_tail - 1].pitch * h_levels[l_tail - 1].h + 16 <= kTailLdsBytes)
        --l_tail;
      if (g.nlevels - l_tail < 4) l_tail = g.nlevels;
    }
  }
  return l_tail;
}

void launch_level_chains(const VsfDev& d, const VsfGeom& g, const VsfLevel* h_levels, const VsfImages& im, hipStream_t s,
                         const VsfSideStream* side, int l_tail) {
  const PyramidArgs p = pyramid_args(d, g, im, 1, l_tail);
  const int nchains = (side && side->n > 0 && im.n >= 2) ? 2 : 1;
  hipStream_t st[VSF_SIDE_STREAMS + 1] = {s};
  for (int c = 1; c < nchains; c++) st[c] = side->stream[c - 1];
  if (nchains > 1) {
    vsf_note(hipEventRecord(side->fork, s));
    for (int c = 1; c < nchains; c++) vsf_note(hipStreamWaitEvent(st[c], side->fork, 0));
  }
  for (int l = 1; l < l_tail; l++) {
    const VsfLevel& L = h_levels[l];
    for (int c = 0; c < nchains; c++) {
      const int i0 = (int)((long)im.n * c / nchains), n = (int)((long)im.n * (c + 1) / nchains) - i0;
      ResizeArgs a = level_args(L, h_levels[l - 1], p, l);
      a.src += (size_t)i0 * a.src_img_stride;
      a.dst += (size_t)i0 * a.dst_img_stride;
      const int nbands = (L.w + 255) / 256;
      const bool large = (long)L.w * L.h * n >= 4000000;
      if (L.resize_rows >= 8) {
        const int R = (large && L.resize_rows >= 16) ? 16 : 8;
        a.nstrips = (L.h + R - 1) / R;
        const int x0 = (L.w / 256) * 256;
        if (x0 < L.w) a.pk = pack_plan(R, x0, L.w, a.nstrips);
        const dim3 grid((a.nstrips + 3) / 4, n, nbands);
        if (R == 16)
          hipLaunchKernelGGL(resize_strip_kernel<16>, grid, dim3(256), 0, st[c], a);
        else
          hipLaunchKernelGGL(resize_strip_kernel<8>, grid, dim3(256), 0, st[c], a);
        continue;
      }
      const int rows = large ? 8 : 4;
      a.nstrips = (L.h + rows - 1) / rows;
      const dim3 grid((a.nstrips + 3) / 4, n, nbands);
      if (large)
        hipLaunchKernelGGL(resize_march_kernel<8>, grid, dim3(256), 0, st[c], a);
      else
        hipLaunchKernelGGL(resize_march_kernel<4>, grid, dim3(256), 0, st[c], a);
    }
  }
  for (int c = 1; c < nchains; c++) {
    vsf_note(hipEventRecord(side->join[c - 1], st[c]));
    vsf_note(hipStreamWaitEvent(s, side->join[c - 1], 0));
  }
}

}

hipError_t vsf_prepare_pyramid_kernels(int lds_limit) {
  if (lds_limit < 160 * 1024 - 2048) return hipSuccess;
  return hipFuncSetAttribute(reinterpret_cast<const void*>(pyramid_slab_kernel), hipFuncAttributeMaxDynamicSharedMemorySize,
                             160 * 1024 - 2048);
}

void vsf_launch_pyramid(const VsfDev& d, const VsfGeom& g, const VsfLevel* h_levels, const VsfImages& im,
                        hipStream_t s, const VsfSideStream* side) {
  const int few_max = d.tune ? d.tune->pyramid_few : 16;
  const bool few = side && im.n <= few_max;
  if (few && g.nlevels > 1 && launch_slab_chains(d, g, h_levels, im, s)) return;
  const int l_tail = choose_l_tail(d, g, h_levels, im, side, few);
  launch_level_chains(d, g, h_levels, im, s, side, l_tail);
  if (l_tail < g.nlevels)
    hipLaunchKernelGGL(pyramid_image_kernel, dim3(im.n), dim3(1024), 0, s, pyramid_args(d, g, im, l_tail, g.nlevels));
}
```

### vision_slam_frontend_amd/csrc/vsf_api.hip

```cpp
#include <algorithm>
#include <cfloat>
#include <climits>
#include <cmath>
#include <cstdio>
#include <cstring>
#include <new>
#include <vector>

#include "vsf_ctx.h"

using namespace vsfi;

thread_local int vsf_tls_hip_error = 0;

namespace vsfi {

vsf_status alloc_devset(vsf_ctx* ctx, const Geometry& G, DevSet* ds, bool orb, int n_images) {
  VSF_HIP(upload(ds->levels, G.levels));
  VSF_HIP(upload(ds->units, G.units));
  VSF_HIP(upload(ds->blur_mma_units, G.blur_mma_units));
  VSF_HIP(upload(ds->blur_mma_units_small, G.blur_mma_units_small));
  VSF_HIP(upload(ds->blur_tcol, G.blur_tcol));
  VSF_HIP(upload(ds->blur_tv, G.blur_tv));
  VSF_HIP(upload(ds->ic_table, build_ic_table()));
  const size_t n = (size_t)n_images;
  if (orb) {
    VSF_HIP(ds->pyr.alloc(n * G.g.pyr_bytes));
    VSF_HIP(ds->blur.alloc(n * G.g.pyr_bytes));
    VSF_HIP(ds->scratch.alloc(n * 6 * G.g.cand_entries * sizeof(uint32_t)));
    VSF_HIP(ds->lvlkp.alloc(n * G.g.lvlkp_entries * sizeof(VsfLevelKp)));
    VSF_HIP(ds->lvl_count.alloc(n * G.g.nlevels * sizeof(int32_t)));
    VSF_HIP(hipMemset(ds->lvl_count, 0, n * G.g.nlevels * sizeof(int32_t)));
  }
  VSF_HIP(ds->cand.alloc(n * G.g.cand_entries * sizeof(uint32_t)));
  const size_t rs_bytes = n * (size_t)std::max(G.g.nunits, 1) * VSF_FAST_RS_STRIDE * sizeof(uint16_t);
  VSF_HIP(ds->rowstart.alloc(rs_bytes));
  VSF_HIP(hipMemset(ds->rowstart, 0, rs_bytes));
  ds->d = VsfDev{ds->levels, ds->units,     ds->pyr,       ds->blur,        ds->cand, ds->rowstart, ds->scratch,
                 ds->lvlkp,  ds->ic_table,  ds->lvl_count, ctx->d_status,   0,        &ctx->tuning};
  ds->ready = true;
  return VSF_OK;
}

void free_retired(vsf_ctx* ctx) {
  ctx->retired.clear();
  ctx->retired_host.clear();
}

vsf_status ensure_match_buffers(vsf_ctx* ctx, int pairs, int rows) {
  if (pairs <= ctx->m_pairs && rows <= ctx->m_rows) return VSF_OK;
  pairs = std::max(pairs, ctx->m_pairs);
  rows = std::max(rows, ctx->m_rows);
  vsf_status st = grow_scratch(ctx, ctx->m_idx2, (size_t)pairs * rows * 2 * sizeof(int32_t));
  if (st == VSF_OK) st = grow_scratch(ctx, ctx->m_dist2, (size_t)pairs * rows * 2 * sizeof(int32_t));
  if (st != VSF_OK) return st;
  ctx->m_pairs = pairs;
  ctx->m_rows = rows;
  return VSF_OK;
}

vsf_status ensure_match_host_staging(vsf_ctx* ctx, int rows) {
  if (rows <= ctx->mh_rows) return VSF_OK;
  vsf_status st = grow_scratch(ctx, ctx->mh_desc, (size_t)2 * rows * VSF_DESC_BYTES);
  if (st == VSF_OK) st = grow_scratch(ctx, ctx->mh_matches, (size_t)rows * sizeof(vsf_dmatch));
  if (st != VSF_OK) return st;
  if (!ctx->mh_counts) VSF_HIP(ctx->mh_counts.alloc(2 * sizeof(int32_t)));
  if (!ctx->mh_nmatches) VSF_HIP(ctx->mh_nmatches.alloc(sizeof(int32_t)));
  ctx->mh_rows = rows;
  return VSF_OK;
}

vsf_status ensure_residual_buffers(vsf_ctx* ctx, int n_frames) {
  const size_t K = (size_t)ctx->p.max_keypoints;
  if (n_frames > ctx->f_frames) {
    vsf_status st = grow_scratch(ctx, ctx->f_residual, (size_t)n_frames * K * sizeof(float));
    if (st != VSF_OK) return st;
    ctx->f_frames = n_frames;
  }
  return VSF_OK;
}

vsf_status ensure_temporal_buffers(vsf_ctx* ctx, int n_pairs) {
  const size_t K = (size_t)ctx->p.max_keypoints;
  if (n_pairs <= ctx->t_pairs) return VSF_OK;
  vsf_status st = grow_scratch(ctx, ctx->t_matches, (size_t)n_pairs * K * sizeof(vsf_dmatch));
  if (st == VSF_OK) st = grow_scratch(ctx, ctx->t_nmatches, (size_t)n_pairs * sizeof(int32_t));
  if (st == VSF_OK) st = grow_scratch(ctx, ctx->t_sortkeys, (size_t)n_pairs * K * 8);
  if (st != VSF_OK) return st;
  ctx->t_pairs = n_pairs;
  return VSF_OK;
}

vsf_status ensure_vision_buffers(vsf_ctx* ctx, int n_frames) {
  const size_t K = (size_t)ctx->p.max_keypoints;
  if (n_frames <= ctx->v_frames) return VSF_OK;
  vsf_status st = grow_scratch(ctx, ctx->v_pairs, (size_t)n_frames * K * 2 * sizeof(uint64_t));
  if (st == VSF_OK) st = grow_scratch(ctx, ctx->v_npairs, (size_t)n_frames * sizeof(int32_t));
  if (st == VSF_OK) st = grow_scratch(ctx, ctx->v_sets, (size_t)2 * n_frames * sizeof(int32_t));
  if (st != VSF_OK) return st;
  vsf_launch_fill_stereo_sets(ctx->v_sets, n_frames, ctx->stream);
  ctx->v_frames = n_frames;
  return VSF_OK;
}

vsf_status ensure_pack_buffers(vsf_ctx* ctx, int n) {
  if (n <= ctx->pk_entries) return VSF_OK;
  vsf_status st = grow_scratch(ctx, ctx->pk_offsets, (size_t)n * sizeof(uint32_t));
  if (st != VSF_OK) return st;
  ctx->pk_entries = n;
  return VSF_OK;
}

vsf_status reserve_scratch(vsf_ctx* ctx, int n_frames, int n_pairs) {
  const int pairs = std::max(n_frames, n_pairs);
  vsf_status st = ensure_match_buffers(ctx, pairs, ctx->p.max_keypoints);
  if (st == VSF_OK) st = ensure_residual_buffers(ctx, n_frames);
  if (st == VSF_OK) st = ensure_temporal_buffers(ctx, pairs);
  if (st == VSF_OK) st = ensure_vision_buffers(ctx, n_frames);
  if (st == VSF_OK) st = ensure_pack_buffers(ctx, n_frames + n_pairs);
  return st;
}

vsf_status check_status_word(vsf_ctx* ctx) {
  VSF_HIP(hipMemcpyAsync(ctx->h_status, ctx->d_status, sizeof(int32_t), hipMemcpyDeviceToHost, ctx->stream));
  VSF_HIP(hipMemsetAsync(ctx->d_status, 0, sizeof(int32_t), ctx->stream));
  VSF_HIP(hipStreamSynchronize(ctx->stream));
  VSF_STICKY();
  if (*ctx->h_status & 2) return VSF_ERR_INVALID_ARG;
  return (*ctx->h_status & 1) ? VSF_ERR_CAPACITY : VSF_OK;
}

vsf_status validate_images(const vsf_ctx* ctx, const uint8_t* d_imgs, int n, size_t image_stride, size_t row_stride) {
  if (!d_imgs || n < 1 || n > ctx->p.max_images) return VSF_ERR_INVALID_ARG;
  if (((uintptr_t)d_imgs & 15) || (image_stride & 15) || (row_stride & 15)) return VSF_ERR_INVALID_ARG;
  if (row_stride < (size_t)ctx->p.width || image_stride < row_stride * (size_t)ctx->p.height) return VSF_ERR_INVALID_ARG;
  return VSF_OK;
}

void prof_fold(vsf_ctx* ctx) {
  for (size_t i = 0; i < ctx->ev_used; i++) {
    float ms = 0.f;
    if (hipEventElapsedTime(&ms, ctx->ev_pool[2 * i], ctx->ev_pool[2 * i + 1]) == hipSuccess) {
      ctx->prof_ms[ctx->ev_stage[i]] += ms;
      ctx->prof_launches[ctx->ev_stage[i]] += ctx->ev_launches[i];
    }
  }
  ctx->ev_used = 0;
}

void sync_all_streams(vsf_ctx* ctx) {
  if (ctx->stream) vsf_note(hipStreamSynchronize(ctx->stream));
  if (ctx->own_stream && ctx->own_stream != ctx->stream) vsf_note(hipStreamSynchronize(ctx->own_stream));
  if (ctx->aux_stream) vsf_note(hipStreamSynchronize(ctx->aux_stream));
  if (ctx->pipe_stream) vsf_note(hipStreamSynchronize(ctx->pipe_stream));
  if (ctx->blur_stream) vsf_note(hipStreamSynchronize(ctx->blur_stream));
  for (int i = 1; i < ctx->side.n; i++)
    if (ctx->side.stream[i]) vsf_note(hipStreamSynchronize(ctx->side.stream[i]));
  if (ctx->ob.copy_stream) vsf_note(hipStreamSynchronize(ctx->ob.copy_stream));
  if (ctx->ob.tail_stream) vsf_note(hipStreamSynchronize(ctx->ob.tail_stream));
}

VsfDev shifted(const VsfDev& d, const VsfGeom& g, int i0) {
  VsfDev o = d;
  const size_t i = (size_t)i0;
  if (o.pyr) o.pyr += i * g.pyr_bytes;
  if (o.blur) o.blur += i * g.pyr_bytes;
  o.cand += i * g.cand_entries;
  o.rowstart += i * (size_t)g.nunits * VSF_FAST_RS_STRIDE;
  if (o.scratch) o.scratch += i * 6 * g.cand_entries;
  if (o.lvlkp) o.lvlkp += i * g.lvlkp_entries;
  if (o.lvl_count) o.lvl_count += i * g.nlevels;
  return o;
}

void extract_on(vsf_ctx* ctx, hipStream_t st, const VsfImages& im_all, int i0, int n, vsf_keypoint* d_kp,
                uint8_t* d_desc, int32_t* d_counts, bool inputs_complete, const VsfSideStream* own_side, int32_t* status,
                int status_stride) {
  const VsfGeom& g = ctx->orb.g;
  VsfDev d = shifted(ctx->dorb.d, g, i0);
  if (status) {
    d.status = status;
    d.status_stride = status_stride;
  }
  VsfImages im = im_all;
  im.base += (size_t)i0 * im.image_stride;
  im.n = n;
  const size_t K = (size_t)ctx->p.max_keypoints;
  const bool pipe = ctx->pipeline && inputs_complete && ctx->lanes == 1 && st == ctx->stream && i0 == 0;
  if (pipe) {
    const int buf = ctx->pyr_flip;
    d.pyr = buf ? ctx->pyr_alt : ctx->dorb.d.pyr;
    hipStream_t ps = ctx->pipe_stream ? ctx->pipe_stream : ctx->aux_stream;
    if (ctx->pyr_free_valid[buf]) vsf_note(hipStreamWaitEvent(ps, ctx->ev_pyr_free[buf], 0));
    if (ctx->fast_done_valid && ctx->tuning.pipe_after_fast) vsf_note(hipStreamWaitEvent(ps, ctx->ev_fast_done, 0));
    if (ctx->ingest_done_valid) vsf_note(hipStreamWaitEvent(ps, ctx->ev_ingest_done, 0));
    if (ctx->input_event) vsf_note(hipStreamWaitEvent(ps, ctx->input_event, 0));
    {
      StageTimer t(ctx, ps, VSF_STAGE_PYRAMID, g.nlevels - 1);
      vsf_launch_pyramid(d, g, ctx->orb.levels.data(), im, ps, nullptr);
    }
    vsf_note(hipEventRecord(ctx->ev_pyr_done, ps));
    vsf_note(hipStreamWaitEvent(st, ctx->ev_pyr_done, 0));
  } else {
    StageTimer t(ctx, st, VSF_STAGE_PYRAMID, g.nlevels - 1);
    vsf_launch_pyramid(d, g, ctx->orb.levels.data(), im, st, own_side ? own_side : (ctx->lanes == 1 ? &ctx->side : nullptr));
  }
  ctx->last_pyr = d.pyr - (size_t)i0 * g.pyr_bytes;
  const bool beside_ok = ctx->blur_overlap && im.n >= 32 && ctx->blur_stream;
  int resident = 0;
  if (beside_ok && ctx->lanes == 1 && st == ctx->stream && i0 == 0 && !own_side) {
    if (ctx->fast_force >= 0)
      resident = ctx->fast_force;
    else if (ctx->fast_resident >= 0)
      resident = ctx->fast_resident;
    else if (ctx->fast_tune.n == im.n && ctx->fast_tune.choice > 0)
      resident = ctx->fast_tune.choice;
  }
  const bool blur_beside = beside_ok;
  auto launch_blur = [&](hipStream_t bs) {
    StageTimer t(ctx, bs, VSF_STAGE_BLUR, 1);
    if (im.n >= 32)
      vsf_launch_blur_mma(d, g, im, ctx->dorb.blur_mma_units, (int)ctx->orb.blur_mma_units.size(), ctx->dorb.blur_tcol,
                          ctx->dorb.blur_tv, ctx->orb.blur_bias, bs);
    else
      vsf_launch_blur_mma(d, g, im, ctx->dorb.blur_mma_units_small, (int)ctx->orb.blur_mma_units_small.size(),
                          ctx->dorb.blur_tcol, ctx->dorb.blur_tv, ctx->orb.blur_bias, bs);
  };
  auto fork_blur = [&]() {
    vsf_note(hipEventRecord(ctx->ev_blur_fork, st));
    vsf_note(hipStreamWaitEvent(ctx->blur_stream, ctx->ev_blur_fork, 0));
    launch_blur(ctx->blur_stream);
    vsf_note(hipEventRecord(ctx->ev_blur_done, ctx->blur_stream));
  };
  if (blur_beside) fork_blur();
  {
    StageTimer t(ctx, st, VSF_STAGE_FAST, 1);
    vsf_launch_fast(d, g, im, ctx->p.fast_threshold, 1, st, blur_beside ? resident : 0, ctx->n_cus, ctx->fast_cells);
  }
  if (pipe) {
    vsf_note(hipEventRecord(ctx->ev_fast_done, st));
    ctx->fast_done_valid = true;
  }
  {
    StageTimer t(ctx, st, VSF_STAGE_SELECT, 1);
    vsf_launch_select(d, g, ctx->orb.levels.data(), im, st);
  }
  if (blur_beside)
    vsf_note(hipStreamWaitEvent(st, ctx->ev_blur_done, 0));
  else
    launch_blur(st);
  {
    StageTimer t(ctx, st, VSF_STAGE_DESCRIBE, 1);
    vsf_launch_describe(d, g, im, ctx->p.max_keypoints, d_kp + i0 * K, d_desc + i0 * K * VSF_DESC_BYTES, d_counts + i0,
                        st);
  }
  if (pipe) {
    const int buf = ctx->pyr_flip;
    vsf_note(hipEventRecord(ctx->ev_pyr_free[buf], st));
    ctx->pyr_free_valid[buf] = true;
    ctx->pyr_flip ^= 1;
  }
}

void match_on(vsf_ctx* ctx, hipStream_t st, const uint8_t* d_desc, const int32_t* d_counts, size_t set_stride,
              const int32_t* d_q_set, const int32_t* d_t_set, int p0, int n, int32_t* d_idx2, int32_t* d_dist2,
              vsf_dmatch* d_matches, int32_t* d_nmatches, int32_t* status) {
  const int rows = ctx->p.max_keypoints;
  const size_t R = (size_t)rows;
  const uint8_t* desc = d_desc;
  const int32_t* counts = d_counts;
  if (!d_q_set) {
    desc += (size_t)(2 * p0) * set_stride;
    counts += 2 * p0;
  }
  int32_t* idx2 = d_idx2 + (size_t)p0 * R * 2;
  int32_t* dist2 = d_dist2 + (size_t)p0 * R * 2;
  {
    StageTimer t(ctx, st, VSF_STAGE_KNN2, 1);
    vsf_launch_knn2(desc, counts, set_stride, d_q_set ? d_q_set + p0 : nullptr, d_t_set ? d_t_set + p0 : nullptr, n,
                    rows, idx2, dist2, st);
  }
  {
    StageTimer t(ctx, st, VSF_STAGE_RATIO, 1);
    vsf_launch_ratio_compact(counts, d_q_set ? d_q_set + p0 : nullptr, d_t_set ? d_t_set + p0 : nullptr, n, rows, idx2,
                             dist2, ctx->p.ratio_num, ctx->p.ratio_shift, d_matches + (size_t)p0 * R, d_nmatches + p0,
                             status ? status : ctx->d_status, st);
  }
}

vsf_status fork_lane(vsf_ctx* ctx) {
  VSF_HIP(hipEventRecord(ctx->ev_fork, ctx->stream));
  VSF_HIP(hipStreamWaitEvent(ctx->aux_stream, ctx->ev_fork, 0));
  return VSF_OK;
}
vsf_status join_lane(vsf_ctx* ctx) {
  VSF_HIP(hipEventRecord(ctx->ev_join, ctx->aux_stream));
  VSF_HIP(hipStreamWaitEvent(ctx->stream, ctx->ev_join, 0));
  return VSF_OK;
}

vsf_status extract_async(vsf_ctx* ctx, const VsfImages& im, vsf_keypoint* d_kp, uint8_t* d_desc, int32_t* d_counts,
                         bool inputs_complete) {
  vsf_status st = run_chunked(ctx, im.n, [&](hipStream_t s, int i0, int n) {
    extract_on(ctx, s, im, i0, n, d_kp, d_desc, d_counts, inputs_complete);
  });
  if (st != VSF_OK) return st;
  ctx->last_images = im;
  ctx->last_valid = true;
  VSF_STICKY();
  return VSF_OK;
}

vsf_status ensure_pipeline_buffers(vsf_ctx* ctx) {
  if (ctx->pyr_alt) return VSF_OK;
  VSF_HIP(ctx->pyr_alt.alloc((size_t)ctx->p.max_images * ctx->orb.g.pyr_bytes));
  VSF_HIP(ctx->ev_pyr_done.alloc(hipEventDisableTiming));
  VSF_HIP(ctx->ev_fast_done.alloc(hipEventDisableTiming));
  for (Event& e : ctx->ev_pyr_free) VSF_HIP(e.alloc(hipEventDisableTiming));
  return VSF_OK;
}

}

hipStream_t vsf_ctx_stream(const vsf_ctx* ctx) { return ctx->stream; }
int vsf_ctx_device(const vsf_ctx* ctx) { return ctx->device; }
void vsf_ctx_set_last_error(vsf_ctx* ctx, int code) { ctx->last_hip = code; }
void vsf_ctx_absorb_noted_error(vsf_ctx* ctx) {
  if (ctx->pending_hip == 0) ctx->pending_hip = vsf_tls_hip_error;
  vsf_tls_hip_error = 0;
}

extern "C" {

vsf_status vsf_params_default(vsf_params* p, int width, int height, int max_images) {
  if (!p) return VSF_ERR_INVALID_ARG;
  std::memset(p, 0, sizeof(*p));
  p->nfeatures = 10000;
  p->scale_factor = 1.04f;
  p->nlevels = 50;
  p->edge_threshold = 31;
  p->first_level = 0;
  p->wta_k = 2;
  p->score_type = 0;
  p->patch_size = 31;
  p->fast_threshold = 20;
  p->blur_sse2 = 1;
  p->residual_order = 0;
  p->fast_detector_threshold = 10;
  p->fast_detector_nms = 1;
  p->width = width;
  p->height = height;
  p->max_images = max_images;
  p->max_keypoints = 0;
  return vsf_params_set_ratio(p, 0.6f);
}

vsf_status vsf_params_set_ratio(vsf_params* p, float nn_match_ratio) {
  if (!p || !(nn_match_ratio > 0.f) || !(nn_match_ratio < 256.f)) return VSF_ERR_INVALID_ARG;
  double r = (double)nn_match_ratio;
  uint32_t shift = 0;
  while (r != std::floor(r) && shift < 31) {
    r *= 2.0;
    ++shift;
  }
  if (r != std::floor(r) || r >= 4294967296.0) return VSF_ERR_INVALID_ARG;
  p->ratio_num = (uint32_t)r;
  p->ratio_shift = shift;
  return VSF_OK;
}

const char* vsf_status_string(vsf_status s) {
  switch (s) {
    case VSF_OK: return "ok";
    case VSF_ERR_INVALID_ARG: return "invalid argument";
    case VSF_ERR_CAPACITY: return "capacity exceeded (results truncated)";
    case VSF_ERR_HIP: return "HIP runtime error";
    case VSF_ERR_UNSUPPORTED: return "unsupported parameter combination";
    case VSF_ERR_NO_DEVICE: return "no usable GPU";
  }
  return "unknown";
}

vsf_status vsf_create(const vsf_params* p, int device, vsf_ctx** out) {
  if (!p || !out) return VSF_ERR_INVALID_ARG;
  *out = nullptr;
  if (p->first_level != 0 || p->wta_k != 2 || p->score_type != 0 || p->patch_size != 31) return VSF_ERR_UNSUPPORTED;
  if (p->nlevels < 1 || p->nlevels > VSF_MAX_LEVELS || p->width < 16 || p->height < 16 || p->max_images < 1 ||
      p->nfeatures < 0 || p->edge_threshold < 0 || !(p->scale_factor > 1.0f))
    return VSF_ERR_INVALID_ARG;
  if (p->edge_threshold < 22) return VSF_ERR_UNSUPPORTED;
  {
    const std::vector<int> um = orb_umax(31);
    static const int expect[16] = {15, 15, 15, 15, 14, 14, 14, 13, 13, 12, 11, 10, 9, 8, 6, 3};
    for (int i = 0; i < 16; i++)
      if (um[i] != expect[i]) return VSF_ERR_UNSUPPORTED;
  }
  int ndev = 0;
  if (hipGetDeviceCount(&ndev) != hipSuccess || ndev < 1 || device < 0 || device >= ndev) return VSF_ERR_NO_DEVICE;
  vsf_ctx* ctx = new (std::nothrow) vsf_ctx();
  if (!ctx) return VSF_ERR_INVALID_ARG;
  ctx->p = *p;
  if (ctx->p.max_keypoints <= 0) ctx->p.max_keypoints = ctx->p.nfeatures + 256;
  ctx->device = device;
  auto fail = [&](vsf_status s) {
    vsf_destroy(ctx);
    return s;
  };
  if (hipSetDevice(device) != hipSuccess) return fail(VSF_ERR_NO_DEVICE);
  {
    int cus = 0;
    if (hipDeviceGetAttribute(&cus, hipDeviceAttributeMultiprocessorCount, device) == hipSuccess && cus > 0) ctx->n_cus = cus;
  }
  if (!build_geometry(ctx->p, true, true, &ctx->orb)) return fail(VSF_ERR_INVALID_ARG);
  if (ctx->own_stream.alloc(hipStreamNonBlocking) != hipSuccess) return fail(VSF_ERR_HIP);
  ctx->stream = ctx->own_stream;
  vsf_ctx::SideOwner& so = ctx->side_own;
  if (ctx->aux_stream.alloc(hipStreamNonBlocking) != hipSuccess ||
      ctx->ev_fork.alloc(hipEventDisableTiming) != hipSuccess ||
      ctx->ev_join.alloc(hipEventDisableTiming) != hipSuccess ||
      so.fork.alloc(hipEventDisableTiming) != hipSuccess)
    return fail(VSF_ERR_HIP);
  ctx->side.fork = so.fork;
  if (ctx->blur_stream.alloc(hipStreamNonBlocking) != hipSuccess ||
      ctx->ev_blur_fork.alloc(hipEventDisableTiming) != hipSuccess ||
      ctx->ev_blur_done.alloc(hipEventDisableTiming) != hipSuccess)
    return fail(VSF_ERR_HIP);
  for (int i = 0; i < VSF_SIDE_STREAMS; i++) {
    if (i > 0 && so.stream[i].alloc(hipStreamNonBlocking) != hipSuccess) return fail(VSF_ERR_HIP);
    if (so.join[i].alloc(hipEventDisableTiming) != hipSuccess) return fail(VSF_ERR_HIP);
    ctx->side.stream[i] = i > 0 ? so.stream[i].get() : ctx->aux_stream.get();
    ctx->side.join[i] = so.join[i];
    ctx->side.n = i + 1;
  }
  if (ctx->d_status.alloc(4 * sizeof(int32_t)) != hipSuccess) return fail(VSF_ERR_HIP);
  if (hipMemset(ctx->d_status, 0, 4 * sizeof(int32_t)) != hipSuccess) return fail(VSF_ERR_HIP);
  {
    int per_block = 0, per_cu = 0;
    if (hipDeviceGetAttribute(&per_block, hipDeviceAttributeMaxSharedMemoryPerBlock, device) != hipSuccess) per_block = 0;
    if (hipDeviceGetAttribute(&per_cu, hipDeviceAttributeMaxSharedMemoryPerMultiprocessor, device) != hipSuccess) per_cu = 0;
    int limit = std::min(std::max(std::max(per_block, per_cu), 64 * 1024), 160 * 1024);
    if (vsf_prepare_sort_kernels(limit) != hipSuccess) {
      (void)hipGetLastError();
      limit = 64 * 1024;
    }
    ctx->tuning.lds_limit = limit;
    if (vsf_prepare_pyramid_kernels(limit) != hipSuccess) {
      (void)hipGetLastError();
      ctx->tuning.pyramid_chain = 0;
    }
    if (vsf_prepare_jpeg_kernels(limit) != hipSuccess) {
      (void)hipGetLastError();
      ctx->tuning.jpeg_serial = 1;
    }
  }
  if (ctx->fast_cells.alloc(2 * sizeof(uint32_t)) != hipSuccess) return fail(VSF_ERR_HIP);
  if (ctx->h_status.alloc(sizeof(int32_t), hipHostMallocDefault) != hipSuccess) return fail(VSF_ERR_HIP);
  vsf_status st = alloc_devset(ctx, ctx->orb, &ctx->dorb, true, ctx->p.max_images);
  if (st != VSF_OK) return fail(st);
  ctx->st_img_pitch = (size_t)align_up(ctx->p.width, 64);
  ctx->st_img_stride = ctx->st_img_pitch * (size_t)ctx->p.height;
  const size_t n = (size_t)ctx->p.max_images, K = (size_t)ctx->p.max_keypoints;
  if (ctx->st_img.alloc(n * ctx->st_img_stride) != hipSuccess ||
      ctx->st_kp.alloc(n * K * sizeof(vsf_keypoint)) != hipSuccess ||
      ctx->st_desc.alloc(n * K * VSF_DESC_BYTES) != hipSuccess ||
      ctx->st_counts.alloc(n * sizeof(int32_t)) != hipSuccess)
    return fail(VSF_ERR_HIP);
  if (reserve_scratch(ctx, std::max(1, ctx->p.max_images / 2), std::max(1, ctx->p.max_images / 2)) != VSF_OK)
    return fail(VSF_ERR_HIP);
  if (hipDeviceSynchronize() != hipSuccess) return fail(VSF_ERR_HIP);
  *out = ctx;
  return VSF_OK;
}

void vsf_destroy(vsf_ctx* ctx) {
  if (!ctx) return;
  hipSetDevice(ctx->device);
  stop_observe_threads(ctx);
  sync_all_streams(ctx);
  vsf_tls_hip_error = 0;
  delete ctx;
}

int vsf_last_hip_error(const vsf_ctx* ctx) { return ctx ? ctx->last_hip : 0; }

vsf_status vsf_get_params(const vsf_ctx* ctx, vsf_params* out) {
  if (!ctx || !out) return VSF_ERR_INVALID_ARG;
  *out = ctx->p;
  return VSF_OK;
}

vsf_status vsf_set_stream(vsf_ctx* ctx, void* hip_stream) {
  VsfErrorScope scope_(ctx);
  if (!ctx) return VSF_ERR_INVALID_ARG;
  VSF_HIP(hipStreamSynchronize(ctx->stream));
  prof_fold(ctx);
  ctx->stream = hip_stream ? (hipStream_t)hip_stream : ctx->own_stream;
  return VSF_OK;
}

vsf_status vsf_set_lanes(vsf_ctx* ctx, int lanes) {
  VsfErrorScope scope_(ctx);
  if (!ctx || lanes < 1 || lanes > 2) return VSF_ERR_INVALID_ARG;
  VSF_HIP(hipStreamSynchronize(ctx->stream));
  ctx->lanes = lanes;
  return VSF_OK;
}

vsf_status vsf_set_blur_overlap(vsf_ctx* ctx, int on) {
  VsfErrorScope scope_(ctx);
  if (!ctx) return VSF_ERR_INVALID_ARG;
  VSF_HIP(hipStreamSynchronize(ctx->stream));
  ctx->blur_overlap = on ? 1 : 0;
  return VSF_OK;
}

vsf_status vsf_set_fast_resident(vsf_ctx* ctx, int waves) {
  VsfErrorScope scope_(ctx);
  if (!ctx || waves < -1 || waves == 1 || waves > 4) return VSF_ERR_INVALID_ARG;
  VSF_HIP(hipStreamSynchronize(ctx->stream));
  ctx->fast_resident = waves;
  return VSF_OK;
}

vsf_status vsf_get_fast_resident(const vsf_ctx* ctx, int* waves) {
  if (!ctx || !waves) return VSF_ERR_INVALID_ARG;
  *waves = ctx->fast_resident >= 0 ? ctx->fast_resident : std::max(ctx->fast_tune.choice, 0);
  return VSF_OK;
}

vsf_status vsf_set_option(vsf_ctx* ctx, int option, int value) {
  VsfErrorScope scope_(ctx);
  if (!ctx || option < 0 || option >= VSF_OPT_COUNT) return VSF_ERR_INVALID_ARG;
  VSF_HIP(hipStreamSynchronize(ctx->stream));
  VsfTuning& t = ctx->tuning;
  switch (option) {
    case VSF_OPT_FAST_BOTH_MAX:
      if (value < 0) return VSF_ERR_INVALID_ARG;
      t.fast_both_max = value;
      break;
    case VSF_OPT_SELECT_WIDE: t.select_wide = value != 0; break;
    case VSF_OPT_SELECT_BIG_CLASS: t.select_big_class = value != 0; break;
    case VSF_OPT_PIPE_AFTER_FAST: t.pipe_after_fast = value != 0; break;
    case VSF_OPT_OBSERVE_THREAD: t.observe_thread = value != 0; break;
    case VSF_OPT_OBSERVE_COPY_THREAD: t.observe_copy_thread = value != 0; break;
    case VSF_OPT_PIPE_PRIORITY:
      if (value < -1 || value > 1) return VSF_ERR_INVALID_ARG;
      t.pipe_priority = value;
      break;
    case VSF_OPT_PYRAMID_FEW:
      if (value < 0) return VSF_ERR_INVALID_ARG;
      t.pyramid_few = value;
      break;
    case VSF_OPT_PYRAMID_CHAIN:
      if (value < 0 || value > 64) return VSF_ERR_INVALID_ARG;
      if (value > 0 && t.lds_limit < 160 * 1024 - 2048) return VSF_ERR_UNSUPPORTED;
      t.pyramid_chain = value;
      break;
    case VSF_OPT_PYRAMID_ROWS:
      if (value < 1) return VSF_ERR_INVALID_ARG;
      t.pyramid_rows = value;
      break;
    case VSF_OPT_PYRAMID_TAIL_MIN:
      if (value < 0) return VSF_ERR_INVALID_ARG;
      t.pyramid_tail_min = value;
      break;
    default: return VSF_ERR_INVALID_ARG;
  }
  return VSF_OK;
}

vsf_status vsf_get_option(const vsf_ctx* ctx, int option, int* value) {
  if (!ctx || !value) return VSF_ERR_INVALID_ARG;
  const VsfTuning& t = ctx->tuning;
  switch (option) {
    case VSF_OPT_FAST_BOTH_MAX: *value = t.fast_both_max; break;
    case VSF_OPT_SELECT_WIDE: *value = t.select_wide; break;
    case VSF_OPT_SELECT_BIG_CLASS: *value = t.select_big_class; break;
    case VSF_OPT_PIPE_AFTER_FAST: *value = t.pipe_after_fast; break;
    case VSF_OPT_OBSERVE_THREAD: *value = t.observe_thread; break;
    case VSF_OPT_OBSERVE_COPY_THREAD: *value = t.observe_copy_thread; break;
    case VSF_OPT_PIPE_PRIORITY: *value = t.pipe_priority; break;
    case VSF_OPT_PYRAMID_FEW: *value = t.pyramid_few; break;
    case VSF_OPT_PYRAMID_CHAIN: *value = t.pyramid_chain; break;
    case VSF_OPT_PYRAMID_ROWS: *value = t.pyramid_rows; break;
    case VSF_OPT_PYRAMID_TAIL_MIN: *value = t.pyramid_tail_min; break;
    default: return VSF_ERR_INVALID_ARG;
  }
  return VSF_OK;
}

vsf_status vsf_set_pipeline(vsf_ctx* ctx, int on) {
  VsfErrorScope scope_(ctx);
  if (!ctx) return VSF_ERR_INVALID_ARG;
  VSF_HIP(hipSetDevice(ctx->device));
  VSF_HIP(hipStreamSynchronize(ctx->stream));
  VSF_HIP(hipStreamSynchronize(ctx->aux_stream));
  if (ctx->pipe_stream) VSF_HIP(hipStreamSynchronize(ctx->pipe_stream));
  if (on && ctx->tuning.pipe_priority != ctx->pipe_stream_priority) {
    ctx->pipe_stream.reset();
    ctx->pipe_stream_priority = 0;
    if (ctx->tuning.pipe_priority != 0) {
      int least = 0, greatest = 0;
      VSF_HIP(hipDeviceGetStreamPriorityRange(&least, &greatest));
      VSF_HIP(ctx->pipe_stream.alloc(hipStreamNonBlocking, ctx->tuning.pipe_priority > 0 ? least : greatest));
      ctx->pipe_stream_priority = ctx->tuning.pipe_priority;
    }
  }
  if (on) {
    const vsf_status st = ensure_pipeline_buffers(ctx);
    if (st != VSF_OK) return st;
  }
  ctx->pipeline = on != 0;
  ctx->pyr_free_valid[0] = ctx->pyr_free_valid[1] = false;
  ctx->fast_done_valid = false;
  return VSF_OK;
}

vsf_status vsf_sync(vsf_ctx* ctx) {
  VsfErrorScope scope_(ctx);
  if (!ctx) return VSF_ERR_INVALID_ARG;
  const vsf_status st = check_status_word(ctx);
  if (!ctx->retired.empty() || !ctx->retired_host.empty()) {
    VSF_HIP(hipSetDevice(ctx->device));
    sync_all_streams(ctx);
    free_retired(ctx);
  }
  return st;
}

vsf_status vsf_set_input_event(vsf_ctx* ctx, void* hip_event) {
  VsfErrorScope scope_(ctx);
  if (!ctx) return VSF_ERR_INVALID_ARG;
  ctx->input_event = static_cast<hipEvent_t>(hip_event);
  return VSF_OK;
}

vsf_status vsf_reserve(vsf_ctx* ctx, int n_frames, int n_pairs) {
  VsfErrorScope scope_(ctx);
  if (!ctx || n_frames < 1 || n_pairs < 0) return VSF_ERR_INVALID_ARG;
  VSF_HIP(hipSetDevice(ctx->device));
  sync_all_streams(ctx);
  free_retired(ctx);
  vsf_status st = reserve_scratch(ctx, n_frames, n_pairs);
  if (st != VSF_OK) return st;
  sync_all_streams(ctx);
  free_retired(ctx);
  VSF_STICKY();
  return VSF_OK;
}

vsf_status vsf_level_info(const vsf_ctx* ctx, int level, int* w, int* h, float* scale, int* nfeatures) {
  if (!ctx || level < 0 || level >= ctx->orb.g.nlevels) return VSF_ERR_INVALID_ARG;
  const VsfLevel& L = ctx->orb.levels[level];
  if (w) *w = L.w;
  if (h) *h = L.h;
  if (scale) *scale = L.scale;
  if (nfeatures) *nfeatures = L.nfeatures;
  return VSF_OK;
}

uint64_t vsf_pyramid_pixels(const vsf_ctx* ctx) { return ctx ? ctx->orb.g.pyramid_pixels : 0; }

uint64_t vsf_algorithmic_bytes_per_image(const vsf_ctx* ctx) {
  if (!ctx) return 0;
  const auto& Ls = ctx->orb.levels;
  uint64_t P = 0, rd = 0, wr = 0;
  for (size_t l = 0; l < Ls.size(); l++) {
    const uint64_t px = (uint64_t)Ls[l].w * Ls[l].h;
    P += px;
    if (l + 1 < Ls.size()) rd += px;
    if (l >= 1) wr += px;
  }
  return rd + wr + P + 2 * P + (uint64_t)ctx->p.nfeatures * (sizeof(vsf_keypoint) + VSF_DESC_BYTES);
}

}
```

### vision_slam_frontend_amd/csrc/vsf_ctx.h

```cpp
#ifndef VSF_CTX_H_
#define VSF_CTX_H_

#include <cstddef>
#include <cstdint>
#include <memory>
#include <vector>

#include "vsf_internal.h"
#include "vsf_observe_plan.h"
#include "vsf_observe_queue.h"

namespace vsfi {

inline int align_up(int v, int a) { return (v + a - 1) / a * a; }

struct Geometry {
  VsfGeom g{};
  std::vector<VsfLevel> levels;
  std::vector<uint32_t> units;
  std::vector<VsfTap> xt, yt;
  std::vector<uint32_t> blur_mma_units, blur_mma_units_small;
  std::vector<uint4> blur_tcol, blur_tv;
  int blur_bias = 0;
};

struct DevSet {
  VsfDev d{};
  vsfi::DevBuf<VsfLevel> levels;
  vsfi::DevBuf<uint32_t> units;
  vsfi::DevBuf<uint32_t> blur_mma_units;
  vsfi::DevBuf<uint32_t> blur_mma_units_small;
  vsfi::DevBuf<uint4> blur_tcol;
  vsfi::DevBuf<uint4> blur_tv;
  vsfi::DevBuf<uint2> ic_table;
  vsfi::DevBuf<uint8_t> pyr, blur;
  vsfi::DevBuf<uint32_t> scratch, cand;
  vsfi::DevBuf<VsfLevelKp> lvlkp;
  vsfi::DevBuf<int32_t> lvl_count;
  vsfi::DevBuf<uint16_t> rowstart;
  bool ready = false;
};

bool build_geometry(const vsf_params& p, bool orb, bool nms, Geometry* out);
void gaussian_taps(int k[4]);
std::vector<uint2> build_ic_table();
std::vector<int> orb_umax(int patch_size);

}

struct vsf_ctx {
  vsf_params p{};
  int device = 0;
  int n_cus = 256;
  vsfi::Stream own_stream;
  hipStream_t stream = nullptr;
  vsfi::Stream aux_stream;
  vsfi::Event ev_fork, ev_join;
  vsfi::Stream blur_stream;
  vsfi::Event ev_blur_fork, ev_blur_done;
  struct SideOwner {
    vsfi::Stream stream[VSF_SIDE_STREAMS];
    vsfi::Event fork, join[VSF_SIDE_STREAMS];
  } side_own;
  VsfSideStream side{};
  bool pipeline = false;
  vsfi::Stream pipe_stream;
  int pipe_stream_priority = 0;
  int pyr_flip = 0;
  vsfi::Event ev_pyr_done, ev_pyr_free[2], ev_fast_done;
  bool pyr_free_valid[2] = {false, false}, fast_done_valid = false;
  vsfi::Event ev_ingest_done;
  bool ingest_done_valid = false;
  hipEvent_t input_event = nullptr;
  const uint8_t* last_pyr = nullptr;
  int lanes = 1;
  int blur_overlap = 1;
  int fast_resident = -1;
  int fast_force = -1;
  VsfTuning tuning;
  int last_hip = 0;
  int pending_hip = 0;
  static constexpr int kObserveBatchSlots = 4;
  struct ObserveBatchMeta;
  struct ObserveBatch {
    vsfi::DevBuf<uint8_t> d_img;
    vsfi::DevBuf<vsf_keypoint> kp_raw;
    vsfi::DevBuf<uint8_t> desc_raw;
    vsfi::DevBuf<int32_t> counts_raw;
    vsfi::DevBuf<vsf_dmatch> matches;
    vsfi::DevBuf<int32_t> nmatches;
    vsfi::DevBuf<int32_t> status;
    vsfi::PinnedBuf<ObserveBatchMeta> h_meta;
    VsfStaging blob;
    vsfi::Event ev_uploaded, ev_extracted, ev_done;
    bool used = false;
    hipStream_t done_stream = nullptr;
  };
  struct ObserveFrame {
    vsf_calibration calib;
    float best_percent = 0.f;
    int batch = -1;
    uint8_t kind[2] = {0, 0};
    uint32_t nbytes[2] = {0, 0};
    bool bayer = false;
    int stream = 0;
    int64_t k = 0;
  };
  struct ObserveStream {
    int64_t frames = 0;
    int64_t last_ticket = -1;
    int uncollected = 0;
  };
  struct DebugForm {
    int kind = VSF_FILE_NONE;
    int quality = 0;
    bool operator==(const DebugForm& o) const { return kind == o.kind && quality == o.quality; }
  };
  struct Observe {
    vsfi::Stream copy_stream, tail_stream;
    std::unique_ptr<vsfi::ObserveQueue> queue;
    std::unique_ptr<vsfi::ObserveCopyHelper> copy_helper;
    bool ready = false;
    int frame_life = 0;
    bool debug = false;
    vsfi::DevBuf<uint8_t> dbg_canvas;
    vsfi::DevBuf<uint64_t> dbg_win;
    vsfi::DevBuf<vsf_draw_op> dbg_ops;
    vsfi::DevBuf<void> dbg_table;
    vsfi::DevBuf<vsf_keypoint> dbg_prev_kp;
    vsfi::DevBuf<int64_t> dbg_ints;
    size_t dbg_stride = 0;
    vsfi::PinnedBuf<uint8_t> h_dbg;
    vsfi::PinnedBuf<uint32_t> h_col;
    int64_t col_ring = 0, col_generated = 0, col_retired = 0;
    struct DebugFiles {
      DebugForm form;
      size_t off[2] = {0, 0}, cap[2] = {0, 0}, slot = 0;
      vsfi::DevBuf<uint8_t> d_slots;
      vsfi::DevBuf<int32_t> d_bytes;
      vsfi::DevBuf<uint8_t> d_scratch;
      vsfi::PinnedBuf<uint8_t> h_ring;
    } files;
    int depth = 0;
    int bmax = 0;
    int n_streams = 1;
    int ring = 0;
    int max_pairs = 0;
    vsfi::DevBuf<uint8_t> sets;
    vsfi::DevBuf<int32_t> set_counts;
    vsfi::DevBuf<float> residual;
    vsfi::DevBuf<float> floats;
    vsfi::DevBuf<vsf_keypoint> kpf;
    vsfi::DevBuf<int32_t> ints;
    vsfi::DevBuf<int32_t> ex_idx2, ex_dist2;
    vsfi::DevBuf<int32_t> t_idx2, t_dist2;
    vsfi::DevBuf<vsf_dmatch> t_matches;
    vsfi::DevBuf<int32_t> t_nmatches;
    vsfi::DevBuf<void> t_sortkeys;
    vsfi::DevBuf<uint64_t> pairs;
    vsfi::DevBuf<int32_t> npairs;
    vsfi::DevBuf<vsf_vision_feature> features;
    vsfi::PinnedBuf<uint8_t> h_img;
    vsfi::PinnedBuf<uint8_t> h_out;
    vsfi::PinnedBuf<uint8_t> h_cmp;
    size_t cmp_cap = 0, cmp_slot = 0;
    vsfi::DevBuf<uint8_t> d_bayer;
    VsfDecodeScratch ing_scratch;
    size_t out_cap = 0, out_stride = 0;
    ObserveBatch batch[kObserveBatchSlots];
    std::vector<ObserveFrame> frames;
    std::vector<ObserveStream> streams;
    std::vector<vsfi::ObservePlanIn> plan_in;
    vsfi::ObservePlan plan;
    int last_batch = -1;
    int64_t stat_copy_ns = 0, stat_wait_ns = 0;
  } ob;
  int ob_depth = 0, ob_min_batch = 0, ob_in_flight = 2;
  int ob_streams = 1;
  bool ob_debug = false;
  DebugForm ob_debug_form;
  size_t ob_cmp_cap = 0;
  vsfi::DevBuf<uint8_t> pyr_alt;
  vsfi::Geometry orb, fast;
  vsfi::DevSet dorb, dfast;
  vsfi::DevBuf<int32_t> d_status;
  vsfi::DevBuf<uint32_t> fast_cells;
  struct FastTune {
    int n = 0, choice = -1;
    vsfi::Event ev[2];
  } fast_tune;
  vsfi::PinnedBuf<int32_t> h_status;
  vsfi::DevBuf<uint8_t> st_img;
  size_t st_img_pitch = 0, st_img_stride = 0;
  vsfi::DevBuf<vsf_keypoint> st_kp;
  vsfi::DevBuf<uint8_t> st_desc;
  vsfi::DevBuf<int32_t> st_counts;
  vsfi::DevBuf<int32_t> m_idx2;
  vsfi::DevBuf<int32_t> m_dist2;
  int m_pairs = 0, m_rows = 0;
  vsfi::DevBuf<float> f_residual;
  int f_frames = 0;
  vsfi::DevBuf<vsf_dmatch> t_matches;
  vsfi::DevBuf<int32_t> t_nmatches;
  vsfi::DevBuf<void> t_sortkeys;
  int t_pairs = 0;
  vsfi::DevBuf<uint64_t> v_pairs;
  vsfi::DevBuf<int32_t> v_npairs;
  vsfi::DevBuf<int32_t> v_sets;
  int v_frames = 0;
  vsfi::DevBuf<uint32_t> pk_offsets;
  int pk_entries = 0;
  std::vector<vsfi::DevBuf<void>> retired;
  std::vector<vsfi::PinnedBuf<void>> retired_host;
  vsfi::DevBuf<uint64_t> dr_win;
  size_t dr_win_cap = 0;
  vsfi::DevBuf<void> dr_canv;
  int dr_canv_cap = 0;
  std::vector<uint8_t> dr_canv_host;
  vsfi::Event dr_uploaded;
  vsfi::DevBuf<uint8_t> dr_buf;
  size_t dr_buf_cap = 0;
  VsfStaging ingest_stage[2];
  int ingest_flip = 0;
  VsfDecodeScratch ingest_scratch;
  VsfEncodeScratch encode;
  vsfi::DevBuf<uint8_t> mh_desc;
  vsfi::DevBuf<int32_t> mh_counts;
  vsfi::DevBuf<vsf_dmatch> mh_matches;
  vsfi::DevBuf<int32_t> mh_nmatches;
  int mh_rows = 0;
  vsfi::DevBuf<uint8_t> mm_desc;
  vsfi::DevBuf<int32_t> mm_counts;
  vsfi::DevBuf<vsf_dmatch> mm_matches;
  vsfi::DevBuf<int32_t> mm_nmatches;
  int mm_sets = 0, mm_rows = 0;
  VsfImages last_images{};
  bool last_valid = false;
  bool fast_nms = true;
  bool prof_on = false;
  std::vector<vsfi::Event> ev_pool;
  std::vector<int> ev_stage;
  std::vector<int> ev_launches;
  size_t ev_used = 0;
  double prof_ms[VSF_STAGE_COUNT] = {0};
  int64_t prof_launches[VSF_STAGE_COUNT] = {0};
};

#define VSF_HIP(call)                     \
  do {                                    \
    hipError_t e_ = (call);               \
    if (e_ != hipSuccess) {               \
      ctx->last_hip = (int)e_;            \
      return VSF_ERR_HIP;                 \
    }                                     \
  } while (0)
#define VSF_STICKY()                                               \
  do {                                                             \
    hipError_t e_ = hipGetLastError();                             \
    if (e_ == hipSuccess) e_ = (hipError_t)vsf_tls_hip_error;      \
    if (e_ == hipSuccess) e_ = (hipError_t)ctx->pending_hip;       \
    vsf_tls_hip_error = 0;                                         \
    ctx->pending_hip = 0;                                          \
    if (e_ != hipSuccess) {                                        \
      ctx->last_hip = (int)e_;                                     \
      return VSF_ERR_HIP;                                          \
    }                                                              \
  } while (0)

namespace vsfi {

template <class T>
hipError_t upload(DevBuf<T>& dst, const std::vector<T>& v) {
  hipError_t e = dst.alloc(v.size() * sizeof(T));
  if (e != hipSuccess) return e;
  return hipMemcpy(dst, v.data(), v.size() * sizeof(T), hipMemcpyHostToDevice);
}

vsf_status alloc_devset(vsf_ctx* ctx, const Geometry& G, DevSet* ds, bool orb, int n_images);

template <class T>
vsf_status grow_scratch(vsf_ctx* ctx, DevBuf<T>& buf, size_t bytes) {
  DevBuf<T> fresh;
  VSF_HIP(fresh.alloc(std::max<size_t>(bytes, 16)));
  if (buf) ctx->retired.emplace_back(buf.release());
  buf = std::move(fresh);
  return VSF_OK;
}
void free_retired(vsf_ctx* ctx);
vsf_status decode_runs(vsf_ctx* ctx, const uint8_t* const* files, const size_t* nbytes, const uint8_t* kinds, int n, int width,
                       int height, VsfStaging& stage, VsfDecodeScratch& scratch, uint8_t* d_dst, size_t dst_image_stride,
                       int dst_pitch, int32_t* d_status, int status_stride, hipStream_t s, int* n_runs = nullptr);
vsf_status ensure_match_buffers(vsf_ctx* ctx, int pairs, int rows);
vsf_status ensure_match_host_staging(vsf_ctx* ctx, int rows);
vsf_status ensure_residual_buffers(vsf_ctx* ctx, int n_frames);
vsf_status ensure_temporal_buffers(vsf_ctx* ctx, int n_pairs);
vsf_status ensure_vision_buffers(vsf_ctx* ctx, int n_frames);
vsf_status ensure_pack_buffers(vsf_ctx* ctx, int n);
vsf_status reserve_scratch(vsf_ctx* ctx, int n_frames, int n_pairs);
vsf_status ensure_pipeline_buffers(vsf_ctx* ctx);
void free_observe(vsf_ctx* ctx);
void stop_observe_threads(vsf_ctx* ctx);

vsf_status check_status_word(vsf_ctx* ctx);
vsf_status validate_images(const vsf_ctx* ctx, const uint8_t* d_imgs, int n, size_t image_stride, size_t row_stride);
void prof_fold(vsf_ctx* ctx);
void sync_all_streams(vsf_ctx* ctx);

struct StageTimer {
  vsf_ctx* ctx;
  size_t slot = 0;
  bool on;
  hipStream_t st;
  StageTimer(vsf_ctx* c, hipStream_t stream, int stage, int launches) : ctx(c), on(c->prof_on), st(stream) {
    if (!on) return;
    if (ctx->ev_used >= 2048) {
      sync_all_streams(ctx);
      prof_fold(ctx);
    }
    slot = ctx->ev_used++;
    while (ctx->ev_pool.size() < 2 * (slot + 1)) {
      ctx->ev_pool.emplace_back();
      vsf_note(ctx->ev_pool.back().alloc(hipEventDefault));
    }
    if (ctx->ev_stage.size() <= slot) {
      ctx->ev_stage.resize(slot + 1);
      ctx->ev_launches.resize(slot + 1);
    }
    ctx->ev_stage[slot] = stage;
    ctx->ev_launches[slot] = launches;
    vsf_note(hipEventRecord(ctx->ev_pool[2 * slot], st));
  }
  ~StageTimer() {
    if (on) vsf_note(hipEventRecord(ctx->ev_pool[2 * slot + 1], st));
  }
};

VsfDev shifted(const VsfDev& d, const VsfGeom& g, int i0);

struct InputEventScope {
  vsf_ctx* ctx;
  explicit InputEventScope(vsf_ctx* c) : ctx(c) {}
  void wait() {
    if (ctx->input_event) vsf_note(hipStreamWaitEvent(ctx->stream, ctx->input_event, 0));
  }
  ~InputEventScope() { ctx->input_event = nullptr; }
};

void extract_on(vsf_ctx* ctx, hipStream_t st, const VsfImages& im_all, int i0, int n, vsf_keypoint* d_kp, uint8_t* d_desc,
                int32_t* d_counts, bool inputs_complete = false, const VsfSideStream* own_side = nullptr,
                int32_t* status = nullptr, int status_stride = 0);
void match_on(vsf_ctx* ctx, hipStream_t st, const uint8_t* d_desc, const int32_t* d_counts, size_t set_stride,
              const int32_t* d_q_set, const int32_t* d_t_set, int p0, int n, int32_t* d_idx2, int32_t* d_dist2,
              vsf_dmatch* d_matches, int32_t* d_nmatches, int32_t* status = nullptr);
vsf_status fork_lane(vsf_ctx* ctx);
vsf_status join_lane(vsf_ctx* ctx);

template <class Body>
vsf_status run_chunked(vsf_ctx* ctx, int units, Body body) {
  if (ctx->lanes < 2 || units < 2) {
    body(ctx->stream, 0, units);
    return VSF_OK;
  }
  vsf_status st = fork_lane(ctx);
  if (st != VSF_OK) return st;
  const int n0 = (units + 1) / 2;
  body(ctx->stream, 0, n0);
  body(ctx->aux_stream, n0, units - n0);
  return join_lane(ctx);
}

vsf_status extract_async(vsf_ctx* ctx, const VsfImages& im, vsf_keypoint* d_kp, uint8_t* d_desc, int32_t* d_counts,
                         bool inputs_complete = false);

}

#endif
```

### vision_slam_frontend_amd/csrc/vsf_geometry.hip

```cpp
#include <algorithm>
#include <cfloat>
#include <climits>
#include <cmath>
#include <cstdio>
#include <cstring>
#include <new>
#include <vector>

#include "vsf_ctx.h"

using namespace vsfi;

namespace {

inline int cvRoundD(double v) { return (int)std::nearbyint(v); }
inline int cvRoundF(float v) { return (int)std::nearbyintf(v); }
inline int cvFloorD(double v) {
  const int i = cvRoundD(v);
  return i - ((float)(v - i) < 0);
}
inline int cvCeilD(double v) {
  const int i = cvRoundD(v);
  return i + ((float)(i - v) < 0);
}

}

namespace vsfi {

void build_taps(int sw, int sh, int dw, int dh, std::vector<VsfTap>* xt, std::vector<VsfTap>* yt) {
  const double scale_x = 1. / ((double)dw / sw), scale_y = 1. / ((double)dh / sh);
  for (int dx = 0; dx < dw; dx++) xt->push_back(resize_xtap(dx, scale_x, sw));
  while (xt->size() % 4) xt->push_back(VsfTap{0, 0, 0, 0});
  for (int dy = 0; dy < dh; dy++) yt->push_back(resize_ytap(dy, scale_y, sh));
}

std::vector<int> orb_umax(int patch_size) {
  const int half = patch_size / 2;
  std::vector<int> umax(half + 2, 0);
  int v, v0;
  const int vmax = cvFloorD(half * std::sqrt(2.f) / 2 + 1);
  const int vmin = cvCeilD(half * std::sqrt(2.f) / 2);
  for (v = 0; v <= vmax; ++v) umax[v] = cvRoundD(std::sqrt((double)half * half - v * v));
  for (v = half, v0 = 0; v >= vmin; --v) {
    while (umax[v0] == umax[v0 + 1]) ++v0;
    umax[v] = v0;
    ++v0;
  }
  return umax;
}

inline int reflect101_host(int p, int len) {
  if (p < 0) p = -p;
  if (p >= len) p = 2 * len - 2 - p;
  return p < 0 ? 0 : (p >= len ? len - 1 : p);
}

uint16_t f16_bits_of_small_int(int v) {
  if (v == 0) return 0;
  int e = 0;
  while ((v >> (e + 1)) != 0) e++;
  const int mant = e <= 10 ? (v << (10 - e)) & 0x3FF : (v >> (e - 10)) & 0x3FF;
  return (uint16_t)(((e + 15) << 10) | mant);
}

void build_blur_mma_tables(Geometry* G) {
  int k4[4];
  gaussian_taps(k4);
  const int k[7] = {k4[0], k4[1], k4[2], k4[3], k4[2], k4[1], k4[0]};
  G->blur_bias = 128 * (k[0] + k[1] + k[2] + k[3] + k[4] + k[5] + k[6]);
  G->blur_tcol.clear();
  G->blur_mma_units.clear();
  G->blur_mma_units_small.clear();
  for (size_t l = 0; l < G->levels.size(); l++) {
    VsfLevel& L = G->levels[l];
    L.blur_tcol = (uint32_t)(G->blur_tcol.size() / 64);
    const int nbands = (L.w + 63) / 64, npairs = (nbands + 1) / 2;
    for (int b = 0; b < 2 * npairs; b++)
      for (int op = 0; op < 4; op++) {
        const int tile = 2 * b + (op >> 1);
        const int first = 32 * tile - 16 + 32 * (op & 1);
        for (int lane = 0; lane < 64; lane++) {
          const int n = lane & 31, h = lane >> 5, x = 32 * tile + n;
          int8_t wgt[16] = {0};
          if (x < L.w)
            for (int j = 0; j < 7; j++) {
              const int c = reflect101_host(x + j - 3, L.w) - (first + 16 * h);
              if (c >= 0 && c < 16) wgt[c] = (int8_t)(wgt[c] + k[j]);
            }
          uint4 v;
          memcpy(&v, wgt, 16);
          G->blur_tcol.push_back(v);
        }
      }
    const int nsteps = (L.h + VSF_BLUR_MMA_ROWS - 1) / VSF_BLUR_MMA_ROWS, ndsteps = (nsteps + 1) / 2;
    for (int pass = 0; pass < 2; pass++) {
      const int per_unit = pass == 0 ? VSF_BLUR_MMA_STEPS : VSF_BLUR_MMA_STEPS_SMALL;
      std::vector<uint32_t>& units = pass == 0 ? G->blur_mma_units : G->blur_mma_units_small;
      const int nstrips = (ndsteps + per_unit - 1) / per_unit;
      for (int st = 0; st < nstrips; st++) {
        const int s0 = (int)((long long)ndsteps * st / nstrips), s1 = (int)((long long)ndsteps * (st + 1) / nstrips);
        for (int b = 0; b < npairs; b++)
          units.push_back(((uint32_t)l << 24) | ((uint32_t)b << 16) | ((uint32_t)s0 << 8) | (uint32_t)(s1 - s0));
      }
    }
  }
  G->blur_tv.clear();
  for (int op = 0; op < 4; op++)
    for (int lane = 0; lane < 64; lane++) {
      const int n = lane & 31, h = lane >> 5, s = op & 1;
      uint16_t e[8];
      for (int j = 0; j < 8; j++) {
        const int row = 16 * s + 8 * (j >> 2) + 4 * h + (j & 3), d = row - n;
        const int tap = (n < VSF_BLUR_MMA_ROWS && d >= 0 && d < 7) ? k[d] : 0;
        e[j] = f16_bits_of_small_int(op >= 2 ? tap * 256 : tap);
      }
      uint4 v;
      memcpy(&v, e, 16);
      G->blur_tv.push_back(v);
    }
}

bool build_geometry(const vsf_params& p, bool orb, bool nms, Geometry* out) {
  Geometry& G = *out;
  const int nlevels = orb ? p.nlevels : 1;
  const int border = orb ? std::max(p.edge_threshold, 3) : 3;
  G.levels.assign(nlevels, VsfLevel{});
  G.g.nlevels = nlevels;
  G.g.width = p.width;
  G.g.height = p.height;
  const double scale_factor = (double)p.scale_factor;
  std::vector<int> nfeat(nlevels, 0);
  if (orb) {
    const float factor = (float)(1.0 / scale_factor);
    float nd = p.nfeatures * (1 - factor) / (1 - (float)std::pow((double)factor, (double)nlevels));
    int sum = 0;
    for (int l = 0; l < nlevels - 1; l++) {
      nfeat[l] = cvRoundF(nd);
      sum += nfeat[l];
      nd *= factor;
    }
    nfeat[nlevels - 1] = std::max(p.nfeatures - sum, 0);
  }
  uint32_t offset = 0;
  uint64_t pixels = 0;
  int max_w = 0;
  for (int l = 0; l < nlevels; l++) {
    VsfLevel& L = G.levels[l];
    L.scale = orb ? (float)std::pow(scale_factor, (double)(l - p.first_level)) : 1.f;
    L.w = cvRoundF(p.width / L.scale);
    L.h = cvRoundF(p.height / L.scale);
    if (L.w < 8 || L.h < 1 || L.w > 4095 || L.h > 4095) return false;
    L.pitch = align_up(L.w, 64);
    L.offset = offset;
    offset += (uint32_t)align_up(L.pitch * align_up(L.h, 8), 256);
    L.nfeatures = nfeat[l];
    pixels += (uint64_t)L.w * L.h;
    max_w = std::max(max_w, L.w);
    if (L.w <= 2 * border || L.h <= 2 * border) {
      L.x_lo = L.x_hi = L.y_lo = L.y_hi = border;
    } else {
      L.x_lo = border;
      L.x_hi = L.w - border;
      L.y_lo = border;
      L.y_hi = L.h - border;
    }
    L.blur_vec_end = p.blur_sse2 ? (L.w - L.w % 4) : 0;
  }
  G.g.pyr_bytes = offset;
  G.g.pyramid_pixels = pixels;
  uint32_t cand = 0;
  int kp_off = 0, ncells = 0;
  struct Narrow {
    int rows, lanes, level, band, strip;
  };
  std::vector<Narrow> narrow;
  for (int l = 0; l < nlevels; l++) {
    VsfLevel& L = G.levels[l];
    const int vw = L.x_hi - L.x_lo, vh = L.y_hi - L.y_lo;
    L.fast_a0 = L.x_lo & ~3;
    L.nbands = vw > 0 ? (L.x_hi - L.fast_a0 + VSF_FAST_BAND_COLS - 1) / VSF_FAST_BAND_COLS : 0;
    L.nstrips = vh > 0 && vw > 0 ? (vh + VSF_FAST_STRIP_ROWS - 1) / VSF_FAST_STRIP_ROWS : 0;
    if (L.nbands > 255 || L.nstrips > 32767) return false;
    L.unit0 = ncells;
    ncells += L.nstrips * L.nbands;
    for (int s = 0; s < L.nstrips; s++)
      for (int b = 0; b < L.nbands; b++) {
        const int bx0 = L.fast_a0 + VSF_FAST_BAND_COLS * b;
        const int lanes = (std::min(L.x_hi, bx0 + VSF_FAST_BAND_COLS) - bx0 + 3) / 4 + 2;
        const int rows = std::min(VSF_FAST_STRIP_ROWS, L.y_hi - (L.y_lo + VSF_FAST_STRIP_ROWS * s));
        if (lanes < 64)
          narrow.push_back(Narrow{rows, lanes, l, b, s});
        else
          G.units.push_back(((uint32_t)l << 24) | ((uint32_t)b << 16) | (uint32_t)s);
      }
    const int bw = std::min(VSF_FAST_BAND_COLS, std::max(vw, 1)), bh = std::min(VSF_FAST_STRIP_ROWS, std::max(vh, 1));
    L.seg_cap = nms ? ((bw + 1) / 2) * ((bh + 1) / 2) : bw * bh;
    L.seg_cap = std::max(L.seg_cap, 1);
    L.cand_offset = cand;
    cand += (uint32_t)L.seg_cap * (uint32_t)(L.nstrips * L.nbands);
    L.kp_offset = kp_off;
    L.kp_cap = 2 * L.nfeatures + 64;
    kp_off += L.kp_cap;
  }
  G.g.cand_entries = std::max(cand, 1u);
  G.g.nunits = ncells;
  std::stable_sort(narrow.begin(), narrow.end(), [](const Narrow& a, const Narrow& b) {
    if (a.rows != b.rows) return a.rows > b.rows;
    if (a.lanes != b.lanes) return a.lanes > b.lanes;
    if (a.level != b.level) return a.level < b.level;
    if (a.strip != b.strip) return a.strip < b.strip;
    return a.band < b.band;
  });
  struct Bin {
    int lanes;
    std::vector<int> cells;
  };
  std::vector<Bin> bins;
  for (int i = 0; i < (int)narrow.size(); i++) {
    const Narrow& c = narrow[i];
    size_t k = 0;
    for (; k < bins.size(); k++) {
      const Bin& B = bins[k];
      if (B.lanes + c.lanes <= 64 && (int)B.cells.size() < VSF_FAST_PACK_SEGS &&
          (narrow[B.cells[0]].level == 0) == (c.level == 0))
        break;
    }
    if (k == bins.size()) bins.push_back(Bin{0, {}});
    bins[k].lanes += c.lanes;
    bins[k].cells.push_back(i);
  }
  std::vector<uint32_t> packs;
  for (const Bin& B : bins) {
    const Narrow& c0 = narrow[B.cells[0]];
    if (B.cells.size() == 1) {
      G.units.push_back(((uint32_t)c0.level << 24) | ((uint32_t)c0.band << 16) | (uint32_t)c0.strip);
      continue;
    }
    uint32_t w[VSF_FAST_PACK_WORDS] = {0};
    int first = 0, mixed = 0, rim = 0;
    w[0] = (uint32_t)B.cells.size();
    w[1] = (uint32_t)c0.rows;
    for (size_t j = 0; j < B.cells.size(); j++) {
      const Narrow& c = narrow[B.cells[j]];
      const VsfLevel& L = G.levels[c.level];
      mixed |= c.rows != c0.rows;
      rim |= L.y_lo - 1 < 3 || L.y_hi >= L.h - 3;
      w[4 + 2 * j] = ((uint32_t)c.level << 24) | ((uint32_t)c.band << 16) | (uint32_t)c.strip;
      w[5 + 2 * j] = (uint32_t)first | ((uint32_t)c.lanes << 8) | ((uint32_t)c.rows << 16);
      first += c.lanes;
    }
    w[2] = (uint32_t)mixed;
    w[3] = (uint32_t)rim;
    packs.insert(packs.end(), w, w + VSF_FAST_PACK_WORDS);
  }
  G.g.nwork_full = (int)G.units.size();
  G.g.nwork_pack = (int)(packs.size() / VSF_FAST_PACK_WORDS);
  G.units.insert(G.units.end(), packs.begin(), packs.end());
  if (G.units.empty()) G.units.push_back(0);
  G.g.lvlkp_entries = std::max(kp_off, 1);
  if (orb) {
    for (int l = 1; l < nlevels; l++) {
      VsfLevel& L = G.levels[l];
      const VsfLevel& P = G.levels[l - 1];
      L.xtab = (uint32_t)G.xt.size();
      L.ytab = (uint32_t)G.yt.size();
      build_taps(P.w, P.h, L.w, L.h, &G.xt, &G.yt);
      {
        const double sx = 1. / ((double)L.w / P.w), sy = 1. / ((double)L.h / P.h);
        memcpy(L.rscale_x, &sx, 8);
        memcpy(L.rscale_y, &sy, 8);
      }
      if (P.w < 8) return false;
      for (int x4 = 0; x4 < L.w; x4 += 4) {
        const int base = std::min((int)G.xt[L.xtab + x4].i0, P.w - 8);
        for (int j = 0; j < 4 && x4 + j < L.w; j++) {
          const VsfTap& t = G.xt[L.xtab + x4 + j];
          if (t.i0 < base || t.i1 - base > 7) return false;
        }
      }
      L.resize_rows = 0;
      for (int R : {16, 8, 4}) {
        bool ok = true;
        for (int ys = 0; ys < L.h && ok; ys += R) {
          const int f = G.yt[L.ytab + ys].i0;
          for (int r = 0; r < R && ys + r < L.h && ok; r++) {
            const VsfTap& t = G.yt[L.ytab + ys + r];
            const int dlt = (int)t.i0 - f - r;
            ok = (dlt == 0 || dlt == 1) && (int)t.i1 == std::min((int)t.i0 + 1, P.h - 1);
          }
        }
        if (ok) {
          L.resize_rows = R;
          break;
        }
      }
      L.resize_any8 = 1;
      for (int ys = 0; ys < L.h && L.resize_any8; ys++) {
        const int f = G.yt[L.ytab + ys].i0;
        for (int r = 0; r < 8 && ys + r < L.h && L.resize_any8; r++) {
          const VsfTap& t = G.yt[L.ytab + ys + r];
          const int dlt = (int)t.i0 - f - r;
          if (!((dlt == 0 || dlt == 1) && (int)t.i1 == std::min((int)t.i0 + 1, P.h - 1))) L.resize_any8 = 0;
        }
      }
    }
  }
  if (G.xt.empty()) G.xt.push_back(VsfTap{0, 0, 0, 0});
  if (G.yt.empty()) G.yt.push_back(VsfTap{0, 0, 0, 0});
  if (orb) {
    int k4[4];
    gaussian_taps(k4);
    const int ksum = 2 * (k4[0] + k4[1] + k4[2]) + k4[3];
    if (ksum > 257 || k4[3] > 127 || G.levels[0].w > 64 * 255 || G.levels[0].h > VSF_BLUR_MMA_ROWS * 255) return false;
    build_blur_mma_tables(&G);
  }
  if (G.blur_mma_units.empty()) G.blur_mma_units.push_back(0);
  if (G.blur_mma_units_small.empty()) G.blur_mma_units_small.push_back(0);
  if (G.blur_tcol.empty()) G.blur_tcol.push_back(make_uint4(0, 0, 0, 0));
  if (G.blur_tv.empty()) G.blur_tv.push_back(make_uint4(0, 0, 0, 0));
  return true;
}

std::vector<uint2> build_ic_table() {
  const std::vector<int> um = orb_umax(31);
  std::vector<uint2> t(4 * VSF_IC_ITEMS, make_uint2(0, 0));
  for (int s = 0; s < 4; s++)
    for (int item = 0; item < 31 * 9; item++) {
      const int r = item / 9, j = item % 9, v = r - 15, d = um[std::abs(v)];
      uint32_t wx = 0, wm = 0;
      for (int b = 0; b < 4; b++) {
        const int u = 4 * j + b - s - 15;
        if (std::abs(u) <= d) {
          wx |= (uint32_t)(u + 16) << (8 * b);
          wm |= 1u << (8 * b);
        }
      }
      t[(size_t)s * VSF_IC_ITEMS + item] = make_uint2(wx, wm);
    }
  return t;
}

void gaussian_taps(int k[4]) {
  const int n = 7;
  const double sigma = 2.0, scale2x = -0.5 / (sigma * sigma);
  float cf[7];
  double sum = 0;
  for (int i = 0; i < n; i++) {
    const double x = i - (n - 1) * 0.5;
    cf[i] = (float)std::exp(scale2x * x * x);
    sum += cf[i];
  }
  sum = 1. / sum;
  for (int i = 0; i < 4; i++) k[i] = cvRoundD((double)(float)(cf[i] * sum) * 256.0);
}

}
```

### vision_slam_frontend_amd/csrc/vsf_internal.h

```cpp
#ifndef VSF_INTERNAL_H_
#define VSF_INTERNAL_H_

#include <hip/hip_runtime.h>
#include <stdint.h>

#include <vector>

#include "../../include/vsf.h"
#include "vsf_own.h"
#include "vsf_resize.h"

#define VSF_FAST_BAND_COLS 248
#define VSF_FAST_PACK_SEGS 8
#define VSF_FAST_PACK_WORDS (4 + 2 * VSF_FAST_PACK_SEGS)
#define VSF_FAST_STRIP_ROWS 32
#define VSF_FAST_RS_STRIDE (VSF_FAST_STRIP_ROWS + 2)
#define VSF_BLUR_MMA_ROWS 26
#define VSF_BLUR_MMA_STEPS 16
#define VSF_BLUR_MMA_STEPS_SMALL 2
#define VSF_BLUR_TILE_OFFSET(pitch, x, y) \
  ((uint32_t)((y) >> 2) * (uint32_t)((pitch) * 4) + ((uint32_t)((x) >> 5) << 7) + ((uint32_t)((y) & 3) << 5) + (uint32_t)((x) & 31))
#define VSF_SORT_LDS_ROWS 4096
#define VSF_IC_ITEMS 320

struct VsfLevel {
  int32_t w, h;
  int32_t pitch;
  uint32_t offset;
  float scale;
  int32_t nfeatures;
  int32_t x_lo, x_hi;
  int32_t y_lo, y_hi;
  int32_t fast_a0;
  int32_t nbands, nstrips;
  int32_t unit0;
  uint32_t cand_offset;
  int32_t seg_cap;
  int32_t kp_offset;
  int32_t kp_cap;
  int32_t blur_vec_end;
  uint32_t xtab, ytab;
  int32_t resize_rows;
  int32_t resize_any8;
  uint32_t rscale_x[2], rscale_y[2];
  uint32_t blur_tcol;
};

#define VSF_CAND_PACK(x, y, s) (((uint32_t)(s) << 24) | ((uint32_t)(y) << 12) | (uint32_t)(x))
#define VSF_CAND_X(c) ((int)((c)&0xFFFu))
#define VSF_CAND_Y(c) ((int)(((c) >> 12) & 0xFFFu))
#define VSF_CAND_SCORE(c) ((int)((c) >> 24))

struct VsfLevelKp {
  uint32_t xy;
  float response;
  float angle;
  float ca, sb;
};

struct VsfGeom {
  int nlevels;
  int width, height;
  uint32_t pyr_bytes;
  uint32_t cand_entries;
  int nunits;
  int nwork_full, nwork_pack;
  int lvlkp_entries;
  uint64_t pyramid_pixels;
};

struct VsfTuning {
  int fast_both_max = 16;
  int select_wide = 1;
  int pipe_priority = 0;
  int pipe_after_fast = 1;
  int select_big_class = 1;
  int jpeg_serial = 0;
  int pyramid_few = 16;
  int pyramid_chain = 8;
  int pyramid_rows = 6;
  int pyramid_tail_min = 0;
  int observe_copy_thread = 1;
  int observe_thread = 0;
  int lds_limit = 0;
};

extern thread_local int vsf_tls_hip_error;
inline void vsf_note(hipError_t e) {
  if (e != hipSuccess && vsf_tls_hip_error == 0) vsf_tls_hip_error = (int)e;
}
hipStream_t vsf_ctx_stream(const vsf_ctx* ctx);
int vsf_ctx_device(const vsf_ctx* ctx);
void vsf_ctx_set_last_error(vsf_ctx* ctx, int code);
constexpr int VSF_RCCL_ERROR_BASE = 10000;
void vsf_ctx_absorb_noted_error(vsf_ctx* ctx);
void vsf_ctx_enter(vsf_ctx* ctx);
struct VsfErrorScope {
  vsf_ctx* ctx;
  explicit VsfErrorScope(vsf_ctx* c, bool enter = true) : ctx(c) {
    if (ctx && enter) vsf_ctx_enter(ctx);
  }
  ~VsfErrorScope() {
    if (ctx && vsf_tls_hip_error != 0) vsf_ctx_absorb_noted_error(ctx);
  }
  VsfErrorScope(const VsfErrorScope&) = delete;
  VsfErrorScope& operator=(const VsfErrorScope&) = delete;
};
hipError_t vsf_prepare_sort_kernels(int lds_limit);
hipError_t vsf_prepare_pyramid_kernels(int lds_limit);
hipError_t vsf_prepare_jpeg_kernels(int lds_limit);

struct VsfDev {
  const VsfLevel* levels;
  const uint32_t* units;
  uint8_t* pyr;
  uint8_t* blur;
  uint32_t* cand;
  uint16_t* rowstart;
  uint32_t* scratch;
  VsfLevelKp* lvlkp;
  const uint2* ic_table;
  int32_t* lvl_count;
  int32_t* status;
  int status_stride;
  const VsfTuning* tune;
};

struct VsfImages {
  const uint8_t* base;
  size_t image_stride;
  size_t row_stride;
  int n;
};

#define VSF_SIDE_STREAMS 1
struct VsfSideStream {
  hipStream_t stream[VSF_SIDE_STREAMS];
  hipEvent_t fork, join[VSF_SIDE_STREAMS];
  int n;
};
void vsf_launch_bayer_bg_gray(const uint8_t* d_src, int n, int w, int h, size_t src_image_stride, int src_pitch,
                              uint8_t* d_dst, size_t dst_image_stride, int dst_pitch, hipStream_t s);
void vsf_launch_pyramid(const VsfDev& d, const VsfGeom& g, const VsfLevel* h_levels, const VsfImages& im,
                        hipStream_t s, const VsfSideStream* side);
void vsf_launch_fast(const VsfDev& d, const VsfGeom& g, const VsfImages& im, int threshold, int nms, hipStream_t s,
                     int resident_waves_per_simd = 0, int n_cus = 0, uint32_t* d_cell_counters = nullptr);
void vsf_launch_select(const VsfDev& d, const VsfGeom& g, const VsfLevel* h_levels, const VsfImages& im,
                       hipStream_t s);
void vsf_launch_retain_best_test(uint2* d_data, uint32_t* d_tables, int n, int n_points, int use_lds, int mode,
                                 int* d_out_n, hipStream_t s);
void vsf_launch_blur_mma(const VsfDev& d, const VsfGeom& g, const VsfImages& im, const uint32_t* d_units, int nunits,
                         const uint4* d_tcol, const uint4* d_tv, int bias, hipStream_t s);
void vsf_launch_describe(const VsfDev& d, const VsfGeom& g, const VsfImages& im, int max_keypoints,
                         vsf_keypoint* d_kp, uint8_t* d_desc, int32_t* d_counts, hipStream_t s);
void vsf_launch_fast_emit(const VsfDev& d, const VsfGeom& g, int n_images, int max_keypoints, vsf_keypoint* d_kp,
                          int32_t* d_counts, hipStream_t s);
void vsf_launch_knn2(const uint8_t* d_desc, const int32_t* d_counts, size_t set_stride, const int32_t* d_q_set,
                     const int32_t* d_t_set, int n_pairs, int max_rows, int32_t* d_idx2, int32_t* d_dist2,
                     hipStream_t s, int rows_hint = 0);
void vsf_launch_ratio_compact(const int32_t* d_counts, const int32_t* d_q_set, const int32_t* d_t_set, int n_pairs,
                              int max_rows, const int32_t* d_idx2, const int32_t* d_dist2, uint32_t ratio_num,
                              uint32_t ratio_shift, vsf_dmatch* d_matches, int32_t* d_nmatches, int32_t* d_status,
                              hipStream_t s);

struct VsfF9 {
  float v[9];
};
void vsf_launch_stereo_filter(const vsf_keypoint* d_kp, const uint8_t* d_desc, const vsf_dmatch* d_matches,
                              const int32_t* d_nmatches, int n_frames, int max_rows, const float* d_F, const float* h_F,
                              int order, const float* d_thr_override, float thr_in, float* d_residual, float* d_mean, float* d_thr,
                              vsf_keypoint* d_kp_out, uint8_t* d_desc_out, int32_t* d_counts_out, hipStream_t s);
void vsf_launch_stereo_residuals(const vsf_keypoint* d_kp, const vsf_dmatch* d_matches, const int32_t* d_nmatches,
                                 int n_frames, int max_rows, const float* d_F, const float* h_F, int order, float* d_residual,
                                 float* d_mean, hipStream_t s);
void vsf_launch_stereo_filter_only(const vsf_keypoint* d_kp, const uint8_t* d_desc, const vsf_dmatch* d_matches,
                                   const int32_t* d_nmatches, int n_frames, int max_rows, const float* d_residual,
                                   const float* d_thr, vsf_keypoint* d_kp_out, uint8_t* d_desc_out,
                                   int32_t* d_counts_out, hipStream_t s, const int32_t* d_out_sets = nullptr,
                                   int32_t* d_set_counts = nullptr);
bool vsf_launch_stereo_one_frame(const vsf_keypoint* d_kp, const uint8_t* d_desc, const vsf_dmatch* d_matches,
                                 const int32_t* d_nmatches, int max_rows, const float* h_F, int order, float* d_mean,
                                 float* d_thr, float* d_thr_state, vsf_keypoint* d_kp_out, uint8_t* d_desc_out,
                                 int32_t* d_counts_out, const int32_t* d_out_sets, int32_t* d_set_counts, hipStream_t s);
void vsf_launch_stereo_thresholds(const float* d_means, int n, float* d_state, float* d_thr, hipStream_t s);
void vsf_launch_fill_stereo_sets(int32_t* d_sets, int n_frames, hipStream_t s);
void vsf_launch_vision_features(const vsf_keypoint* d_kp, const int32_t* d_counts, const uint64_t* d_pairs,
                                const int32_t* d_npairs, int n_frames, int max_rows, const vsf_calibration& c,
                                vsf_vision_feature* d_out, int32_t* d_nfeatures, int32_t* d_npoints, hipStream_t s);
void vsf_launch_pack_outputs(const vsf_vision_feature* d_features, const int32_t* d_nfeatures, int n_frames,
                             const uint64_t* d_pairs, const int32_t* d_npairs, int n_pairs, int max_rows,
                             uint8_t* d_payload, uint32_t cap_bytes, uint32_t* d_offsets, int32_t* d_status,
                             hipStream_t s);
void vsf_launch_sort_trim(const vsf_dmatch* d_matches, const int32_t* d_nmatches, int n_pairs, int max_rows,
                          float best_percent, const float* d_best_percent_of, void* d_scratch, uint64_t* d_pairs,
                          int32_t* d_npairs, hipStream_t s, bool force_serial = false, int lds_limit = 160 * 1024);
#define VSF_OBSERVE_MAX_PAIRS 64
struct VsfObserveFrame {
  int32_t left_set;
  int32_t n_past;
  int32_t tp0;
  int32_t out_slot;
};
struct VsfObserveParam {
  int32_t stream;
  int32_t calib;
  float best_percent;
  int32_t prev, tail;
};
void vsf_launch_stereo_residuals_table(const vsf_keypoint* d_kp, const vsf_dmatch* d_matches, const int32_t* d_nmatches,
                                       int n_frames, int max_rows, const VsfObserveParam* d_par, const vsf_calibration* d_calibs,
                                       int order, float* d_residual, float* d_mean, hipStream_t s);
void vsf_launch_stereo_thresholds_streams(const float* d_means, int n, const VsfObserveParam* d_par, float* d_state,
                                          float* d_thr, hipStream_t s);
void vsf_launch_vision_features_table(const vsf_keypoint* d_kp, const int32_t* d_counts, const uint64_t* d_pairs,
                                      const int32_t* d_npairs, int n_frames, int max_rows, const VsfObserveParam* d_par,
                                      const vsf_calibration* d_calibs, vsf_vision_feature* d_out, int32_t* d_nfeatures,
                                      int32_t* d_npoints, hipStream_t s);
struct VsfObserveArgs {
  int n_frames, max_rows;
  const int32_t* counts_raw;
  const int32_t* nmatches;
  const int32_t* counts_f;
  const int32_t* npoints;
  const float* means;
  const float* thr;
  const vsf_vision_feature* features;
  const vsf_keypoint* kp_f;
  const uint8_t* desc_sets;
  const uint64_t* pairs;
  const int32_t* npairs;
  int32_t* status;
  const VsfObserveFrame* frames;
  uint8_t* out;
  size_t out_stride;
  uint32_t out_cap;
};
void vsf_launch_observe_pack(const VsfObserveArgs& a, int max_pairs_per_frame, hipStream_t s);
struct VsfObserveDebugArgs {
  int n_frames, max_rows, width, height;
  const uint8_t* images;
  size_t image_stride, image_pitch;
  const vsf_keypoint* kp_f;
  const int32_t* counts_f;
  const uint64_t* pairs;
  const int32_t* npairs;
  const VsfObserveFrame* frames;
  vsf_keypoint* prev_kp;
  int32_t* prev_n;
  const uint32_t* colours;
  int64_t colour_ring;
  int64_t* colour_cursor;
  vsf_draw_op* ops;
  void* canvases;
  uint8_t* canvas;
  size_t canvas_stride;
  uint64_t* winners;
  uint8_t* out;
  size_t out_stride;
};
void vsf_launch_observe_debug(const VsfObserveDebugArgs& a, hipStream_t s);

#ifdef __cplusplus
#include <vector>
struct VsfJpegPlan {
  size_t off_images = 0, off_index = 0, off_tables = 0, off_scans = 0, off_prog_huff = 0, off_stream = 0, total = 0;
  std::vector<uint8_t> head;
  std::vector<size_t> scan_begin;
  std::vector<uint32_t> stream_off, stream_len;
  int n_par = 0;
  int n_prog = 0;
  int n_prog_huff = 0;
  int max_luma_blocks = 0;
  int max_slots = 1;
};
vsf_status vsf_jpeg_plan(const uint8_t* const* jpeg, const size_t* nbytes, int n, int width, int height, bool force_serial,
                         VsfJpegPlan* plan);
void vsf_jpeg_fill(const VsfJpegPlan& plan, const uint8_t* const* jpeg, int n, uint8_t* dst);
#endif
#ifdef __cplusplus
struct VsfPngPlan {
  size_t off_images = 0, off_pieces = 0, off_tables = 0, off_stream = 0, total = 0;
  std::vector<uint8_t> head;
  std::vector<uint32_t> piece_first, piece_off, piece_len;
  std::vector<uint32_t> stream_off, stream_len;
  size_t filtered_stride = 0;
  bool any_rgb = false;
  bool any_general = false;
};
vsf_status vsf_png_plan(const uint8_t* const* png, const size_t* nbytes, int n, int width, int height, VsfPngPlan* plan);
void vsf_png_fill(const VsfPngPlan& plan, const uint8_t* const* png, int n, uint8_t* dst);
#endif
struct VsfDecodeScratch {
  vsfi::DevBuf<uint8_t> clean;
  vsfi::DevBuf<int16_t> coef;
  vsfi::DevBuf<int32_t> flags;
  vsfi::DevBuf<uint8_t> filtered;
  vsfi::DevBuf<int32_t> file_status;
  size_t clean_cap = 0, coef_cap = 0, flags_cap = 0, filtered_cap = 0, file_status_cap = 0;
  size_t bytes() const { return clean_cap + coef_cap + flags_cap + filtered_cap + file_status_cap; }
};
struct VsfDecodeNeed {
  size_t clean = 0, coef = 0, flags = 0, filtered = 0, file_status = 0;
};
struct VsfStaging {
  vsfi::PinnedBuf<uint8_t> h;
  vsfi::DevBuf<uint8_t> d;
  size_t cap = 0;
  vsfi::Event uploaded;
};
VsfDecodeNeed vsf_jpeg_scratch_need(const VsfJpegPlan& plan);
VsfDecodeNeed vsf_png_scratch_need(const VsfPngPlan& plan, int n);
void vsf_launch_jpeg_decode(const uint8_t* d_blob, const VsfJpegPlan& plan, int n, int width, int height,
                            const VsfDecodeScratch& scratch, uint8_t* d_dst, size_t dst_image_stride, int dst_pitch,
                            int32_t* d_status, int status_stride, bool prog_serial, hipStream_t s);
void vsf_launch_png_decode(const uint8_t* d_blob, const VsfPngPlan& plan, int n, int width, int height,
                           const VsfDecodeScratch& scratch, uint8_t* d_dst, size_t dst_image_stride, int dst_pitch,
                           int32_t* d_status, int status_stride, hipStream_t s);

enum { VSF_FILE_NONE = 0, VSF_FILE_JPEG = 1, VSF_FILE_PNG = 2 };
int vsf_file_kind(const uint8_t* file, size_t nbytes);
int vsf_run_end(const uint8_t* kinds, int n, int i0);
struct VsfDecodeRun {
  int i0 = 0, n = 0, kind = VSF_FILE_NONE;
  size_t off = 0;
  VsfJpegPlan jp;
  VsfPngPlan pp;
};
struct VsfDecodeRuns {
  std::vector<VsfDecodeRun> runs;
  size_t total = 0;
};
vsf_status vsf_plan_runs(const uint8_t* const* files, const size_t* nbytes, const uint8_t* kinds, int n, int width, int height,
                         bool force_serial, VsfDecodeRuns* out);
void vsf_fill_runs(const VsfDecodeRuns& plan, const uint8_t* const* files, uint8_t* dst);
struct VsfEncodeJob {
  int kind = VSF_FILE_NONE;
  int n = 0, width = 0, height = 0, channels = 0;
  size_t src_image_stride = 0, src_row_stride = 0;
  int quality = 0;
  size_t out_stride = 0;
  size_t out_cap = 0;
  size_t cap() const { return out_cap == 0 || out_cap > out_stride ? out_stride : out_cap; }
};
int vsf_jpeg_enc_launches();
size_t vsf_jpeg_enc_scratch_need(const VsfEncodeJob& job);
void vsf_jpeg_enc_launch(const VsfEncodeJob& job, const uint8_t* d_src, void* d_scratch, uint8_t* d_out, int32_t* d_out_bytes,
                         int32_t* d_status, hipStream_t s);
int vsf_png_enc_launches();
size_t vsf_png_enc_scratch_need(const VsfEncodeJob& job);
void vsf_png_enc_launch(const VsfEncodeJob& job, const uint8_t* d_src, void* d_scratch, uint8_t* d_out, int32_t* d_out_bytes,
                        int32_t* d_status, hipStream_t s);
inline size_t vsf_encode_capacity(int kind, int w, int h, int ch) {
  return kind == VSF_FILE_PNG ? vsf_png_encode_capacity(w, h, ch) : vsf_jpeg_encode_capacity(w, h, ch);
}
inline int vsf_encode_launches(int kind) { return kind == VSF_FILE_PNG ? vsf_png_enc_launches() : vsf_jpeg_enc_launches(); }
inline size_t vsf_encode_scratch_need(const VsfEncodeJob& j) { return j.kind == VSF_FILE_PNG ? vsf_png_enc_scratch_need(j) : vsf_jpeg_enc_scratch_need(j); }
inline void vsf_launch_encode(const VsfEncodeJob& j, const uint8_t* d_src, void* d_scratch, uint8_t* d_out, int32_t* d_out_bytes,
                              int32_t* d_status, hipStream_t s) {
  (j.kind == VSF_FILE_PNG ? vsf_png_enc_launch : vsf_jpeg_enc_launch)(j, d_src, d_scratch, d_out, d_out_bytes, d_status, s);
}
struct VsfEncodeScratch {
  vsfi::DevBuf<uint8_t> scratch;
  vsfi::DevBuf<uint8_t> staging;
  size_t scratch_cap = 0, staging_cap = 0;
};
void vsf_launch_files_home(const uint8_t* d_files, size_t file_stride, const int32_t* d_bytes, int n, uint8_t* h_ring,
                           size_t slot_stride, size_t file_off, int which, int slot0, int depth, const VsfObserveFrame* frames,
                           const uint8_t* results, size_t result_stride, hipStream_t s);
void vsf_launch_ingest_finish(uint8_t* d_img, size_t image_stride, int pitch, int rows, const int32_t* d_status, int n,
                              hipStream_t s);

#endif
```

Baseline: 43180.

## Start FAST on early pyramid levels on a side stream while pyramid finishes

Splits FAST detection into an early part covering the full cells of the first pyramid levels and a late part for the rest. A hook in the pyramid level chain fires once the chosen level is built and launches the early part on the blur stream. This overlaps FAST with the remaining pyramid construction. A second, double-buffered candidate and rowstart buffer with free events keeps consecutive pipelined frames from clobbering each other. The cost is extra memory, more events and cross-stream dependencies, and a smaller late FAST launch.

```diff
diff --git a/include/vsf.h b/include/vsf.h
--- a/include/vsf.h
+++ b/include/vsf.h
@@ -88,7 +88,9 @@
   VSF_OPT_OBSERVE_THREAD = 8,
   VSF_OPT_PYRAMID_TAIL_MIN = 9,
   VSF_OPT_OBSERVE_COPY_THREAD = 10,
-  VSF_OPT_COUNT = 11
+  VSF_OPT_FAST_EARLY_LEVELS = 11,
+  VSF_OPT_FAST_EARLY_FORM = 12,
+  VSF_OPT_COUNT = 13
 } vsf_option;
 vsf_status vsf_set_option(vsf_ctx* ctx, int option, int value);
 vsf_status vsf_get_option(const vsf_ctx* ctx, int option, int* value);
diff --git a/vision_slam_frontend_amd/capi.py b/vision_slam_frontend_amd/capi.py
--- a/vision_slam_frontend_amd/capi.py
+++ b/vision_slam_frontend_amd/capi.py
@@ -40,7 +40,8 @@
     "vsf_observe_set_streams", "vsf_observe_submit_stream", "vsf_observe_submit_compressed_stream", "vsf_observe_reset_stream",
 ]
 (OPT_FAST_BOTH_MAX, OPT_SELECT_WIDE, OPT_PYRAMID_FEW, OPT_PYRAMID_CHAIN, OPT_PYRAMID_ROWS, OPT_SELECT_BIG_CLASS,
- OPT_PIPE_AFTER_FAST, OPT_PIPE_PRIORITY, OPT_OBSERVE_THREAD, OPT_PYRAMID_TAIL_MIN, OPT_OBSERVE_COPY_THREAD) = range(11)
+ OPT_PIPE_AFTER_FAST, OPT_PIPE_PRIORITY, OPT_OBSERVE_THREAD, OPT_PYRAMID_TAIL_MIN, OPT_OBSERVE_COPY_THREAD,
+ OPT_FAST_EARLY_LEVELS, OPT_FAST_EARLY_FORM) = range(13)
 STAGE_COUNT = 8
 OBSERVE_STATS = ("frames", "batches", "max_batch", "solo", "forced", "slot_waits", "depth", "bmax", "copy_ns", "launch_ns",
                  "wait_ns", "compressed", "ingest_commands", "compressed_bytes", "debug_jpeg_commands", "streams",
diff --git a/vision_slam_frontend_amd/csrc/k_fast.hip b/vision_slam_frontend_amd/csrc/k_fast.hip
--- a/vision_slam_frontend_amd/csrc/k_fast.hip
+++ b/vision_slam_frontend_amd/csrc/k_fast.hip
@@ -1,4 +1,5 @@
 #include "vsf_gather.h"
+#include <algorithm>
 #include <cstdlib>
 
 #include "vsf_internal.h"
@@ -373,24 +374,25 @@
 }
 
 template <bool PACK, bool NMS>
-__global__ __launch_bounds__(256) void fast_march_kernel(FastArgs a, int nwork) {
+__global__ __launch_bounds__(256) void fast_march_kernel(FastArgs a, int first, int nwork) {
   const int item = __builtin_amdgcn_readfirstlane(blockIdx.x * 4 + (threadIdx.x >> 6));
   if (item >= nwork) return;
-  fast_march_body<PACK, NMS>(a, item, blockIdx.y);
+  fast_march_body<PACK, NMS>(a, first + item, blockIdx.y);
 }
 
 template <bool NMS>
-__global__ __launch_bounds__(256) void fast_march_both_kernel(FastArgs a, int nfull, int npack) {
+__global__ __launch_bounds__(256) void fast_march_both_kernel(FastArgs a, int first, int nfull, int npack) {
   const int item = __builtin_amdgcn_readfirstlane(blockIdx.x * 4 + (threadIdx.x >> 6));
   if (item >= nfull + npack) return;
   if (item < nfull)
-    fast_march_body<false, NMS>(a, item, blockIdx.y);
+    fast_march_body<false, NMS>(a, first + item, blockIdx.y);
   else
     fast_march_body<true, NMS>(a, item - nfull, blockIdx.y);
 }
 
 template <bool PACK, bool NMS>
-__global__ __launch_bounds__(1024) void fast_march_resident_kernel(FastArgs a, int nwork, int nimages, uint32_t* next_cell) {
+__global__ __launch_bounds__(1024) void fast_march_resident_kernel(FastArgs a, int first, int nwork, int nimages,
+                                                                  uint32_t* next_cell) {
   const int total = nwork * nimages;
   while (true) {
     uint32_t r;
@@ -406,7 +408,7 @@
     const uint32_t u = (uint32_t)__builtin_amdgcn_readfirstlane((int)r);
     if (u >= (uint32_t)total) break;
     const int image = (int)u / nwork, cell = (int)u - image * nwork;
-    fast_march_body<PACK, NMS>(a, cell, image);
+    fast_march_body<PACK, NMS>(a, first + cell, image);
   }
 }
 
@@ -445,7 +447,11 @@
 }
 
 void vsf_launch_fast(const VsfDev& d, const VsfGeom& g, const VsfImages& im, int threshold, int nms, hipStream_t s,
-                     int resident_waves_per_simd, int n_cus, uint32_t* d_cell_counters) {
+                     int resident_waves_per_simd, int n_cus, uint32_t* d_cell_counters, int part, int n_early) {
+  n_early = std::min(std::max(n_early, 0), g.nwork_full);
+  const int f0 = part == VSF_FAST_LATE ? n_early : 0;
+  const int nf = part == VSF_FAST_EARLY ? n_early : g.nwork_full - f0;
+  const int np = part == VSF_FAST_EARLY ? 0 : g.nwork_pack;
   FastArgs a;
   a.levels = d.levels;
   a.units = d.units;
@@ -462,32 +468,31 @@
   a.threshold = threshold;
   a.nms = nms;
   if (resident_waves_per_simd > 0 && resident_waves_per_simd <= 4 && nms && d_cell_counters) {
-    vsf_note(hipMemsetAsync(d_cell_counters, 0, 2 * sizeof(uint32_t), s));
+    uint32_t* cnt = part == VSF_FAST_EARLY ? d_cell_counters + 2 : d_cell_counters;
+    vsf_note(hipMemsetAsync(cnt, 0, (part == VSF_FAST_EARLY ? 1 : 2) * sizeof(uint32_t), s));
     const dim3 block(256 * resident_waves_per_simd);
-    if (g.nwork_full > 0)
-      hipLaunchKernelGGL((fast_march_resident_kernel<false, true>), dim3(n_cus), block, 0, s, a, g.nwork_full, im.n,
-                         d_cell_counters);
-    if (g.nwork_pack > 0)
-      hipLaunchKernelGGL((fast_march_resident_kernel<true, true>), dim3(n_cus), block, 0, s, a, g.nwork_pack, im.n,
-                         d_cell_counters + 1);
+    if (nf > 0)
+      hipLaunchKernelGGL((fast_march_resident_kernel<false, true>), dim3(n_cus), block, 0, s, a, f0, nf, im.n, cnt);
+    if (np > 0)
+      hipLaunchKernelGGL((fast_march_resident_kernel<true, true>), dim3(n_cus), block, 0, s, a, 0, np, im.n, cnt + 1);
     return;
   }
-  const dim3 gf((g.nwork_full + 3) / 4, im.n), gp((g.nwork_pack + 3) / 4, im.n);
+  const dim3 gf((nf + 3) / 4, im.n), gp((np + 3) / 4, im.n);
   const int both_max = d.tune ? d.tune->fast_both_max : 16;
-  if (im.n <= both_max && g.nwork_full > 0 && g.nwork_pack > 0) {
-    const dim3 gb((g.nwork_full + g.nwork_pack + 3) / 4, im.n);
+  if (im.n <= both_max && nf > 0 && np > 0) {
+    const dim3 gb((nf + np + 3) / 4, im.n);
     if (nms)
-      hipLaunchKernelGGL((fast_march_both_kernel<true>), gb, dim3(256), 0, s, a, g.nwork_full, g.nwork_pack);
+      hipLaunchKernelGGL((fast_march_both_kernel<true>), gb, dim3(256), 0, s, a, f0, nf, np);
     else
-      hipLaunchKernelGGL((fast_march_both_kernel<false>), gb, dim3(256), 0, s, a, g.nwork_full, g.nwork_pack);
+      hipLaunchKernelGGL((fast_march_both_kernel<false>), gb, dim3(256), 0, s, a, f0, nf, np);
     return;
   }
   if (nms) {
-    if (g.nwork_full > 0) hipLaunchKernelGGL((fast_march_kernel<false, true>), gf, dim3(256), 0, s, a, g.nwork_full);
-    if (g.nwork_pack > 0) hipLaunchKernelGGL((fast_march_kernel<true, true>), gp, dim3(256), 0, s, a, g.nwork_pack);
+    if (nf > 0) hipLaunchKernelGGL((fast_march_kernel<false, true>), gf, dim3(256), 0, s, a, f0, nf);
+    if (np > 0) hipLaunchKernelGGL((fast_march_kernel<true, true>), gp, dim3(256), 0, s, a, 0, np);
   } else {
-    if (g.nwork_full > 0) hipLaunchKernelGGL((fast_march_kernel<false, false>), gf, dim3(256), 0, s, a, g.nwork_full);
-    if (g.nwork_pack > 0) hipLaunchKernelGGL((fast_march_kernel<true, false>), gp, dim3(256), 0, s, a, g.nwork_pack);
+    if (nf > 0) hipLaunchKernelGGL((fast_march_kernel<false, false>), gf, dim3(256), 0, s, a, f0, nf);
+    if (np > 0) hipLaunchKernelGGL((fast_march_kernel<true, false>), gp, dim3(256), 0, s, a, 0, np);
   }
 }
 
diff --git a/vision_slam_frontend_amd/csrc/k_pyramid.hip b/vision_slam_frontend_amd/csrc/k_pyramid.hip
--- a/vision_slam_frontend_amd/csrc/k_pyramid.hip
+++ b/vision_slam_frontend_amd/csrc/k_pyramid.hip
@@ -539,9 +539,11 @@
 }
 
 void launch_level_chains(const VsfDev& d, const VsfGeom& g, const VsfLevel* h_levels, const VsfImages& im, hipStream_t s,
-                         const VsfSideStream* side, int l_tail) {
+                         const VsfSideStream* side, int l_tail, const VsfPyramidHook* hook) {
   const PyramidArgs p = pyramid_args(d, g, im, 1, l_tail);
   const int nchains = (side && side->n > 0 && im.n >= 2) ? 2 : 1;
+  if (nchains > 1) hook = nullptr;
+  if (hook && hook->level <= 0) hook->fn(hook->arg, s);
   hipStream_t st[VSF_SIDE_STREAMS + 1] = {s};
   for (int c = 1; c < nchains; c++) st[c] = side->stream[c - 1];
   if (nchains > 1) {
@@ -577,6 +579,7 @@
       else
         hipLaunchKernelGGL(resize_march_kernel<4>, grid, dim3(256), 0, st[c], a);
     }
+    if (hook && hook->level == l) hook->fn(hook->arg, s);
   }
   for (int c = 1; c < nchains; c++) {
     vsf_note(hipEventRecord(side->join[c - 1], st[c]));
@@ -593,12 +596,12 @@
 }
 
 void vsf_launch_pyramid(const VsfDev& d, const VsfGeom& g, const VsfLevel* h_levels, const VsfImages& im,
-                        hipStream_t s, const VsfSideStream* side) {
+                        hipStream_t s, const VsfSideStream* side, const VsfPyramidHook* hook) {
   const int few_max = d.tune ? d.tune->pyramid_few : 16;
   const bool few = side && im.n <= few_max;
   if (few && g.nlevels > 1 && launch_slab_chains(d, g, h_levels, im, s)) return;
   const int l_tail = choose_l_tail(d, g, h_levels, im, side, few);
-  launch_level_chains(d, g, h_levels, im, s, side, l_tail);
+  launch_level_chains(d, g, h_levels, im, s, side, l_tail, hook);
   if (l_tail < g.nlevels)
     hipLaunchKernelGGL(pyramid_image_kernel, dim3(im.n), dim3(1024), 0, s, pyramid_args(d, g, im, l_tail, g.nlevels));
 }
diff --git a/vision_slam_frontend_amd/csrc/vsf_api.hip b/vision_slam_frontend_amd/csrc/vsf_api.hip
--- a/vision_slam_frontend_amd/csrc/vsf_api.hip
+++ b/vision_slam_frontend_amd/csrc/vsf_api.hip
@@ -177,6 +177,16 @@
                 uint8_t* d_desc, int32_t* d_counts, bool inputs_complete, const VsfSideStream* own_side, int32_t* status,
                 int status_stride) {
   const VsfGeom& g = ctx->orb.g;
+  const bool pipe = ctx->pipeline && inputs_complete && ctx->lanes == 1 && st == ctx->stream && i0 == 0;
+  const int early_levels = pipe && ctx->cand_alt && ctx->blur_stream && ctx->fast_force < 0
+                               ? std::min(ctx->tuning.fast_early_levels, g.fast_split_levels)
+                               : 0;
+  const int n_early = early_levels > 0 ? vsf_fast_n_early(ctx->orb.levels.data(), g.nlevels, early_levels) : 0;
+  if (n_early > 0) {
+    ctx->cand_flip ^= 1;
+    ctx->dorb.d.cand = ctx->cand_flip ? ctx->cand_alt.get() : ctx->dorb.cand.get();
+    ctx->dorb.d.rowstart = ctx->cand_flip ? ctx->rowstart_alt.get() : ctx->dorb.rowstart.get();
+  }
   VsfDev d = shifted(ctx->dorb.d, g, i0);
   if (status) {
     d.status = status;
@@ -186,7 +196,6 @@
   im.base += (size_t)i0 * im.image_stride;
   im.n = n;
   const size_t K = (size_t)ctx->p.max_keypoints;
-  const bool pipe = ctx->pipeline && inputs_complete && ctx->lanes == 1 && st == ctx->stream && i0 == 0;
   if (pipe) {
     const int buf = ctx->pyr_flip;
     d.pyr = buf ? ctx->pyr_alt : ctx->dorb.d.pyr;
@@ -195,10 +204,36 @@
     if (ctx->fast_done_valid && ctx->tuning.pipe_after_fast) vsf_note(hipStreamWaitEvent(ps, ctx->ev_fast_done, 0));
     if (ctx->ingest_done_valid) vsf_note(hipStreamWaitEvent(ps, ctx->ev_ingest_done, 0));
     if (ctx->input_event) vsf_note(hipStreamWaitEvent(ps, ctx->input_event, 0));
+    struct Early {
+      vsf_ctx* ctx;
+      const VsfDev* d;
+      const VsfImages* im;
+      int n_early;
+      bool fired;
+    } early{ctx, &d, &im, n_early, false};
+    const VsfPyramidHook hook{early_levels - 1,
+                              [](void* arg, hipStream_t chain) {
+                                Early& e = *static_cast<Early*>(arg);
+                                vsf_ctx* c = e.ctx;
+                                hipStream_t es = c->blur_stream;
+                                e.fired = true;
+                                vsf_note(hipEventRecord(c->ev_early_go, chain));
+                                vsf_note(hipStreamWaitEvent(es, c->ev_early_go, 0));
+                                if (c->cand_free_valid[c->cand_flip])
+                                  vsf_note(hipStreamWaitEvent(es, c->ev_cand_free[c->cand_flip], 0));
+                                {
+                                  StageTimer t(c, es, VSF_STAGE_FAST, 0);
+                                  vsf_launch_fast(*e.d, c->orb.g, *e.im, c->p.fast_threshold, 1, es, c->tuning.fast_early_form,
+                                                  c->n_cus, c->fast_cells, VSF_FAST_EARLY, e.n_early);
+                                }
+                                vsf_note(hipEventRecord(c->ev_early_done, es));
+                              },
+                              &early};
     {
       StageTimer t(ctx, ps, VSF_STAGE_PYRAMID, g.nlevels - 1);
-      vsf_launch_pyramid(d, g, ctx->orb.levels.data(), im, ps, nullptr);
+      vsf_launch_pyramid(d, g, ctx->orb.levels.data(), im, ps, nullptr, n_early > 0 ? &hook : nullptr);
     }
+    if (n_early > 0 && !early.fired) hook.fn(&early, ps);
     vsf_note(hipEventRecord(ctx->ev_pyr_done, ps));
     vsf_note(hipStreamWaitEvent(st, ctx->ev_pyr_done, 0));
   } else {
@@ -233,9 +268,11 @@
     vsf_note(hipEventRecord(ctx->ev_blur_done, ctx->blur_stream));
   };
   if (blur_beside) fork_blur();
+  if (n_early > 0) vsf_note(hipStreamWaitEvent(st, ctx->ev_early_done, 0));
   {
     StageTimer t(ctx, st, VSF_STAGE_FAST, 1);
-    vsf_launch_fast(d, g, im, ctx->p.fast_threshold, 1, st, blur_beside ? resident : 0, ctx->n_cus, ctx->fast_cells);
+    vsf_launch_fast(d, g, im, ctx->p.fast_threshold, 1, st, blur_beside ? resident : 0, ctx->n_cus, ctx->fast_cells,
+                    n_early > 0 ? VSF_FAST_LATE : VSF_FAST_ALL, n_early);
   }
   if (pipe) {
     vsf_note(hipEventRecord(ctx->ev_fast_done, st));
@@ -244,6 +281,10 @@
   {
     StageTimer t(ctx, st, VSF_STAGE_SELECT, 1);
     vsf_launch_select(d, g, ctx->orb.levels.data(), im, st);
+  }
+  if (pipe && ctx->cand_alt) {
+    vsf_note(hipEventRecord(ctx->ev_cand_free[ctx->cand_flip], st));
+    ctx->cand_free_valid[ctx->cand_flip] = true;
   }
   if (blur_beside)
     vsf_note(hipStreamWaitEvent(st, ctx->ev_blur_done, 0));
@@ -314,6 +355,16 @@
 vsf_status ensure_pipeline_buffers(vsf_ctx* ctx) {
   if (ctx->pyr_alt) return VSF_OK;
   VSF_HIP(ctx->pyr_alt.alloc((size_t)ctx->p.max_images * ctx->orb.g.pyr_bytes));
+  {
+    const size_t n = (size_t)ctx->p.max_images;
+    const size_t rs_bytes = n * (size_t)std::max(ctx->orb.g.nunits, 1) * VSF_FAST_RS_STRIDE * sizeof(uint16_t);
+    VSF_HIP(ctx->cand_alt.alloc(n * ctx->orb.g.cand_entries * sizeof(uint32_t)));
+    VSF_HIP(ctx->rowstart_alt.alloc(rs_bytes));
+    VSF_HIP(hipMemset(ctx->rowstart_alt, 0, rs_bytes));
+    for (Event& e : ctx->ev_cand_free) VSF_HIP(e.alloc(hipEventDisableTiming));
+    VSF_HIP(ctx->ev_early_go.alloc(hipEventDisableTiming));
+    VSF_HIP(ctx->ev_early_done.alloc(hipEventDisableTiming));
+  }
   VSF_HIP(ctx->ev_pyr_done.alloc(hipEventDisableTiming));
   VSF_HIP(ctx->ev_fast_done.alloc(hipEventDisableTiming));
   for (Event& e : ctx->ev_pyr_free) VSF_HIP(e.alloc(hipEventDisableTiming));
@@ -453,7 +504,7 @@
       ctx->tuning.jpeg_serial = 1;
     }
   }
-  if (ctx->fast_cells.alloc(2 * sizeof(uint32_t)) != hipSuccess) return fail(VSF_ERR_HIP);
+  if (ctx->fast_cells.alloc(3 * sizeof(uint32_t)) != hipSuccess) return fail(VSF_ERR_HIP);
   if (ctx->h_status.alloc(sizeof(int32_t), hipHostMallocDefault) != hipSuccess) return fail(VSF_ERR_HIP);
   vsf_status st = alloc_devset(ctx, ctx->orb, &ctx->dorb, true, ctx->p.max_images);
   if (st != VSF_OK) return fail(st);
@@ -541,6 +592,14 @@
     case VSF_OPT_SELECT_WIDE: t.select_wide = value != 0; break;
     case VSF_OPT_SELECT_BIG_CLASS: t.select_big_class = value != 0; break;
     case VSF_OPT_PIPE_AFTER_FAST: t.pipe_after_fast = value != 0; break;
+    case VSF_OPT_FAST_EARLY_LEVELS:
+      if (value < 0 || value > VSF_MAX_LEVELS) return VSF_ERR_INVALID_ARG;
+      t.fast_early_levels = value;
+      break;
+    case VSF_OPT_FAST_EARLY_FORM:
+      if (value < 0 || value > 3) return VSF_ERR_INVALID_ARG;
+      t.fast_early_form = value;
+      break;
     case VSF_OPT_OBSERVE_THREAD: t.observe_thread = value != 0; break;
     case VSF_OPT_OBSERVE_COPY_THREAD: t.observe_copy_thread = value != 0; break;
     case VSF_OPT_PIPE_PRIORITY:
@@ -577,6 +636,8 @@
     case VSF_OPT_SELECT_WIDE: *value = t.select_wide; break;
     case VSF_OPT_SELECT_BIG_CLASS: *value = t.select_big_class; break;
     case VSF_OPT_PIPE_AFTER_FAST: *value = t.pipe_after_fast; break;
+    case VSF_OPT_FAST_EARLY_LEVELS: *value = t.fast_early_levels; break;
+    case VSF_OPT_FAST_EARLY_FORM: *value = t.fast_early_form; break;
     case VSF_OPT_OBSERVE_THREAD: *value = t.observe_thread; break;
     case VSF_OPT_OBSERVE_COPY_THREAD: *value = t.observe_copy_thread; break;
     case VSF_OPT_PIPE_PRIORITY: *value = t.pipe_priority; break;
@@ -612,6 +673,7 @@
   }
   ctx->pipeline = on != 0;
   ctx->pyr_free_valid[0] = ctx->pyr_free_valid[1] = false;
+  ctx->cand_free_valid[0] = ctx->cand_free_valid[1] = false;
   ctx->fast_done_valid = false;
   return VSF_OK;
 }
diff --git a/vision_slam_frontend_amd/csrc/vsf_ctx.h b/vision_slam_frontend_amd/csrc/vsf_ctx.h
--- a/vision_slam_frontend_amd/csrc/vsf_ctx.h
+++ b/vision_slam_frontend_amd/csrc/vsf_ctx.h
@@ -69,6 +69,9 @@
   int pyr_flip = 0;
   vsfi::Event ev_pyr_done, ev_pyr_free[2], ev_fast_done;
   bool pyr_free_valid[2] = {false, false}, fast_done_valid = false;
+  int cand_flip = 0;
+  vsfi::Event ev_cand_free[2], ev_early_go, ev_early_done;
+  bool cand_free_valid[2] = {false, false};
   vsfi::Event ev_ingest_done;
   bool ingest_done_valid = false;
   hipEvent_t input_event = nullptr;
@@ -181,6 +184,8 @@
   DebugForm ob_debug_form;
   size_t ob_cmp_cap = 0;
   vsfi::DevBuf<uint8_t> pyr_alt;
+  vsfi::DevBuf<uint32_t> cand_alt;
+  vsfi::DevBuf<uint16_t> rowstart_alt;
   vsfi::Geometry orb, fast;
   vsfi::DevSet dorb, dfast;
   vsfi::DevBuf<int32_t> d_status;
diff --git a/vision_slam_frontend_amd/csrc/vsf_fast_split.h b/vision_slam_frontend_amd/csrc/vsf_fast_split.h
--- /dev/null
+++ b/vision_slam_frontend_amd/csrc/vsf_fast_split.h
@@ -0,0 +1,39 @@
+#ifndef VSF_FAST_SPLIT_H_
+#define VSF_FAST_SPLIT_H_
+
+#define VSF_FAST_SPLIT_BAND_COLS 248
+#define VSF_FAST_SPLIT_STRIP_ROWS 32
+
+inline int vsf_fast_cell_lanes(int fast_a0, int x_hi, int band) {
+  const int bx0 = fast_a0 + VSF_FAST_SPLIT_BAND_COLS * band;
+  const int end = x_hi < bx0 + VSF_FAST_SPLIT_BAND_COLS ? x_hi : bx0 + VSF_FAST_SPLIT_BAND_COLS;
+  return (end - bx0 + 3) / 4 + 2;
+}
+
+inline int vsf_fast_full_cells(int x_lo, int x_hi, int y_lo, int y_hi) {
+  if (x_hi <= x_lo || y_hi <= y_lo) return 0;
+  const int a0 = x_lo & ~3;
+  const int nbands = (x_hi - a0 + VSF_FAST_SPLIT_BAND_COLS - 1) / VSF_FAST_SPLIT_BAND_COLS;
+  const int nstrips = (y_hi - y_lo + VSF_FAST_SPLIT_STRIP_ROWS - 1) / VSF_FAST_SPLIT_STRIP_ROWS;
+  int full = 0;
+  for (int b = 0; b < nbands; b++) full += vsf_fast_cell_lanes(a0, x_hi, b) >= 64;
+  return full * nstrips;
+}
+
+template <class Level>
+inline int vsf_fast_split_levels(const Level* lv, int nlevels) {
+  int n = 0;
+  for (int l = 0; l < nlevels; l++)
+    if (vsf_fast_full_cells(lv[l].x_lo, lv[l].x_hi, lv[l].y_lo, lv[l].y_hi) > 0) n = l + 1;
+  return n;
+}
+
+template <class Level>
+inline int vsf_fast_n_early(const Level* lv, int nlevels, int early_levels) {
+  const int le = early_levels < nlevels ? early_levels : nlevels;
+  int n = 0;
+  for (int l = 0; l < le; l++) n += vsf_fast_full_cells(lv[l].x_lo, lv[l].x_hi, lv[l].y_lo, lv[l].y_hi);
+  return n;
+}
+
+#endif
diff --git a/vision_slam_frontend_amd/csrc/vsf_geometry.hip b/vision_slam_frontend_amd/csrc/vsf_geometry.hip
--- a/vision_slam_frontend_amd/csrc/vsf_geometry.hip
+++ b/vision_slam_frontend_amd/csrc/vsf_geometry.hip
@@ -186,8 +186,7 @@
     ncells += L.nstrips * L.nbands;
     for (int s = 0; s < L.nstrips; s++)
       for (int b = 0; b < L.nbands; b++) {
-        const int bx0 = L.fast_a0 + VSF_FAST_BAND_COLS * b;
-        const int lanes = (std::min(L.x_hi, bx0 + VSF_FAST_BAND_COLS) - bx0 + 3) / 4 + 2;
+        const int lanes = vsf_fast_cell_lanes(L.fast_a0, L.x_hi, b);
         const int rows = std::min(VSF_FAST_STRIP_ROWS, L.y_hi - (L.y_lo + VSF_FAST_STRIP_ROWS * s));
         if (lanes < 64)
           narrow.push_back(Narrow{rows, lanes, l, b, s});
@@ -205,6 +204,8 @@
   }
   G.g.cand_entries = std::max(cand, 1u);
   G.g.nunits = ncells;
+  G.g.fast_split_levels = vsf_fast_split_levels(G.levels.data(), nlevels);
+  if (vsf_fast_n_early(G.levels.data(), nlevels, nlevels) != (int)G.units.size()) return false;
   std::stable_sort(narrow.begin(), narrow.end(), [](const Narrow& a, const Narrow& b) {
     if (a.rows != b.rows) return a.rows > b.rows;
     if (a.lanes != b.lanes) return a.lanes > b.lanes;
diff --git a/vision_slam_frontend_amd/csrc/vsf_internal.h b/vision_slam_frontend_amd/csrc/vsf_internal.h
--- a/vision_slam_frontend_amd/csrc/vsf_internal.h
+++ b/vision_slam_frontend_amd/csrc/vsf_internal.h
@@ -8,6 +8,7 @@
 
 #include "../../include/vsf.h"
 #include "vsf_own.h"
+#include "vsf_fast_split.h"
 #include "vsf_resize.h"
 
 #define VSF_FAST_BAND_COLS 248
@@ -15,6 +16,8 @@
 #define VSF_FAST_PACK_WORDS (4 + 2 * VSF_FAST_PACK_SEGS)
 #define VSF_FAST_STRIP_ROWS 32
 #define VSF_FAST_RS_STRIDE (VSF_FAST_STRIP_ROWS + 2)
+static_assert(VSF_FAST_SPLIT_BAND_COLS == VSF_FAST_BAND_COLS && VSF_FAST_SPLIT_STRIP_ROWS == VSF_FAST_STRIP_ROWS,
+              "vsf_fast_split.h states the cell size for itself");
 #define VSF_BLUR_MMA_ROWS 26
 #define VSF_BLUR_MMA_STEPS 16
 #define VSF_BLUR_MMA_STEPS_SMALL 2
@@ -65,6 +68,7 @@
   uint32_t cand_entries;
   int nunits;
   int nwork_full, nwork_pack;
+  int fast_split_levels;
   int lvlkp_entries;
   uint64_t pyramid_pixels;
 };
@@ -75,6 +79,8 @@
   int pipe_priority = 0;
   int pipe_after_fast = 1;
   int select_big_class = 1;
+  int fast_early_levels = 12;
+  int fast_early_form = 0;
   int jpeg_serial = 0;
   int pyramid_few = 16;
   int pyramid_chain = 8;
@@ -141,10 +147,17 @@
 };
 void vsf_launch_bayer_bg_gray(const uint8_t* d_src, int n, int w, int h, size_t src_image_stride, int src_pitch,
                               uint8_t* d_dst, size_t dst_image_stride, int dst_pitch, hipStream_t s);
+struct VsfPyramidHook {
+  int level;
+  void (*fn)(void* arg, hipStream_t s);
+  void* arg;
+};
 void vsf_launch_pyramid(const VsfDev& d, const VsfGeom& g, const VsfLevel* h_levels, const VsfImages& im,
-                        hipStream_t s, const VsfSideStream* side);
+                        hipStream_t s, const VsfSideStream* side, const VsfPyramidHook* hook = nullptr);
+enum { VSF_FAST_ALL = 0, VSF_FAST_EARLY = 1, VSF_FAST_LATE = 2 };
 void vsf_launch_fast(const VsfDev& d, const VsfGeom& g, const VsfImages& im, int threshold, int nms, hipStream_t s,
-                     int resident_waves_per_simd = 0, int n_cus = 0, uint32_t* d_cell_counters = nullptr);
+                     int resident_waves_per_simd = 0, int n_cus = 0, uint32_t* d_cell_counters = nullptr,
+                     int part = VSF_FAST_ALL, int n_early = 0);
 void vsf_launch_select(const VsfDev& d, const VsfGeom& g, const VsfLevel* h_levels, const VsfImages& im,
                        hipStream_t s);
 void vsf_launch_retain_best_test(uint2* d_data, uint32_t* d_tables, int n, int n_points, int use_lds, int mode,
```

New measurement: 44850 (median of 6 runs). 1.04x the previous value.
